# microsoft/hivedscheduler

Hardware: AMD Instinct MI355X
Metric: scheduling p50 latency + VC-safety violations; RCCL bus-bw at 1/2/4/8-GPU cells (lower is better)
Workload: dtype fp32; 1 GPU; model=hived-sched-config4-fragmentation-stress, cluster=simulated 4-node x 8-MI355X, global_batch=64, seq_len=0, parallelism=single

## Files before the change

hivedscheduler_amd/core/algorithm.cpp:

```cpp
#include <cstdio>
#include <cstdlib>

#include "core.hpp"

namespace hived {

bool mapDebugRelease() {
  static int v = -1;
  if (v < 0) v = getenv("HIVED_DEBUG_MAP") ? 1 : 0;
  return v == 1;
}

namespace {
constexpr size_t kWaitReasonReserve = 128;

struct Victims {
  std::map<std::string, std::set<std::string>> byNode;
  std::set<Group*> overlappingPreemptors;
};

Victims collectPreemptionVictims(const Placement<PhysicalCell>& placement) {
  Victims v;
  for (auto& [leafNum, pods] : placement) {
    (void)leafNum;
    for (auto& pod : pods) {
      for (PhysicalCell* c : pod) {
        if (c == nullptr) continue;
        if ((c->state == CState::Used || c->state == CState::Reserving) &&
            c->usingGroup != nullptr) {
          for (auto& [ln, victims] : c->usingGroup->allocatedPods) {
            (void)ln;
            for (auto& p : victims) {
              if (p.present) v.byNode[p.node].insert(p.key);
            }
          }
        }
        if (c->state == CState::Reserving || c->state == CState::Reserved) {
          v.overlappingPreemptors.insert(c->reservingGroup);
        }
      }
    }
  }
  return v;
}

std::set<std::string> collectBadOrNonSuggestedNodes(const Placement<PhysicalCell>& placement,
                                                    const std::set<std::string>& suggestedNodes,
                                                    bool ignoreSuggestedNodes) {
  std::set<std::string> bad;
  for (auto& [leafNum, pods] : placement) {
    (void)leafNum;
    for (auto& pod : pods) {
      for (PhysicalCell* c : pod) {
        if (c == nullptr) continue;
        if (!c->healthy || (!ignoreSuggestedNodes && !suggestedNodes.count(c->nodes[0]))) {
          bad.insert(c->nodes[0]);
        }
      }
    }
  }
  return bad;
}

std::pair<PodPlacementInfo, std::string> retrieveMissingPodPlacement(Group* g, int leafCellNum,
                                                                     int podIndex) {
  for (auto& [ln, pods] : g->allocatedPods) {
    (void)ln;
    for (auto& p : pods) {
      if (!p.present) continue;
      for (auto& mbi : p.bindInfo.memberBindInfo) {
        if (!mbi.empty() && static_cast<int>(mbi[0].leafIndices.size()) == leafCellNum &&
            podIndex < static_cast<int>(mbi.size())) {
          return {mbi[podIndex], p.bindInfo.chain};
        }
      }
    }
  }
  throw HivedError::Internal("no allocated pod found in group " + g->name +
                             " when retrieving missing placement");
}

VirtualCell* retrieveVirtualCell(const Placement<PhysicalCell>& phys,
                                 const Placement<VirtualCell>& virt, PhysicalCell* target) {
  for (auto& [leafNum, pods] : phys) {
    auto vIt = virt.find(leafNum);
    if (vIt == virt.end()) continue;
    for (size_t podIdx = 0; podIdx < pods.size(); podIdx++) {
      for (size_t i = 0; i < pods[podIdx].size(); i++) {
        if (pods[podIdx][i] == target) return vIt->second[podIdx][i];
      }
    }
  }
  return nullptr;
}

int getNewPodIndex(const std::vector<AllocatedPod>& pods) {
  for (size_t i = 0; i < pods.size(); i++) {
    if (!pods[i].present) return static_cast<int>(i);
  }
  return -1;
}

int getAllocatedPodIndex(const BindInfo& info, int leafCellNum) {
  for (auto& mbi : info.memberBindInfo) {
    if (mbi.empty() || static_cast<int>(mbi[0].leafIndices.size()) != leafCellNum) continue;
    for (size_t podIndex = 0; podIndex < mbi.size(); podIndex++) {
      auto& pl = mbi[podIndex];
      if (pl.node == info.node && !info.isolation.empty() &&
          std::find(pl.leafIndices.begin(), pl.leafIndices.end(), info.isolation[0]) !=
              pl.leafIndices.end()) {
        return static_cast<int>(podIndex);
      }
    }
  }
  return -1;
}

bool allPodsReleased(const std::map<int, std::vector<AllocatedPod>>& allocatedPods) {
  for (auto& [ln, pods] : allocatedPods) {
    (void)ln;
    for (auto& p : pods) {
      if (p.present) return false;
    }
  }
  return true;
}

bool anyBoundUnder(PhysicalCell* c) {
  if (c->virt != nullptr) return true;
  for (Cell* ch : c->children) {
    if (anyBoundUnder(static_cast<PhysicalCell*>(ch))) return true;
  }
  return false;
}

std::unique_ptr<Group> newGroup(const PodSpec& s, GState state) {
  auto g = std::make_unique<Group>();
  g->name = s.groupName;
  g->vc = s.vc;
  g->lazyPreemptionEnable = s.lazyPreemptionEnable;
  g->ignoreK8sSuggestedNodes = s.ignoreK8sSuggestedNodes;
  g->gangReleaseEnable = s.gangReleaseEnable;
  g->priority = s.priority;
  g->state = state;
  g->totalPodNums = s.groupPodNums;
  for (auto& [leafNum, podNum] : s.groupPodNums) {
    g->allocatedPods[leafNum].resize(podNum);
    auto& phys = g->physPlacement[leafNum];
    phys.resize(podNum);
    for (auto& pod : phys) pod.assign(leafNum, nullptr);
    auto& virt = g->virtPlacement[leafNum];
    virt.resize(podNum);
    for (auto& pod : virt) pod.assign(leafNum, nullptr);
  }
  return g;
}

}


ScheduleResult HivedCore::schedule(const PodSpec& s, const std::string& podKey,
                                   const std::set<std::string>& suggestedNodes, Phase phase) {
  OpGuard opGuard(this);
  scheduleCount_++;
  Placement<PhysicalCell> phys;
  Placement<VirtualCell> virt;
  bool hasVirtual = true;
  std::map<std::string, std::set<std::string>> victims;
  std::string waitReason;
  waitReason.reserve(kWaitReasonReserve);
  int podIndex = 0;
  bool havePlacement = false;

  auto it = groups_.find(s.groupName);
  bool groupExists = it != groups_.end();
  bool mayHaveGroup = groupExists || phase == Phase::Preempting;
  if (groupExists) {
    havePlacement = schedulePodFromExistingGroup(it->second.get(), s, suggestedNodes, phase,
                                                 podKey, &phys, &hasVirtual, &virt, &victims,
                                                 &podIndex);
    groupExists = groups_.find(s.groupName) != groups_.end();
  }
  if (!groupExists) {
    schedulePodFromNewGroup(s, suggestedNodes, phase, podKey, &phys, &hasVirtual, &virt, &victims,
                            &waitReason);
    havePlacement = !phys.empty();
  }
  (void)havePlacement;
  Group* g = nullptr;
  if (mayHaveGroup) {
    if (auto git = groups_.find(s.groupName); git != groups_.end()) g = git->second.get();
  }
  return generateResult(phys, hasVirtual, virt, victims, std::move(waitReason), s.leafCellNumber,
                        podIndex, g, s.groupName);
}

ScheduleResult HivedCore::generateResult(const Placement<PhysicalCell>& phys, bool hasVirtual,
                                         const Placement<VirtualCell>& virt,
                                         const std::map<std::string, std::set<std::string>>& victims,
                                         std::string&& waitReason, int currentLeafNum,
                                         int podIndex, Group* group,
                                         const std::string& groupName) {
  ScheduleResult r;
  if (phys.empty()) {
    r.kind = ScheduleResult::Kind::Wait;
    if (waitReason.empty()) {
      r.waitReason = "waiting for resources";
    } else {
      r.waitReason = std::move(waitReason);
    }
    return r;
  }
  if (!victims.empty()) {
    r.kind = ScheduleResult::Kind::Preempt;
    auto it = victims.begin();
    std::advance(it, static_cast<long>(victimRng_() % victims.size()));
    r.victimNode = it->first;
    r.victimPodKeys.assign(it->second.begin(), it->second.end());
    return r;
  }
  r.kind = ScheduleResult::Kind::Bind;
  BindInfo& info = r.bindInfo;
  for (auto& [leafNum, pods] : phys) {
    std::vector<PodPlacementInfo> placements(pods.size());
    for (size_t pi = 0; pi < pods.size(); pi++) {
      auto& pl = placements[pi];
      pl.leafIndices.assign(leafNum, 0);
      pl.preassignedTypes.assign(leafNum, "");
      for (int li = 0; li < leafNum; li++) {
        PhysicalCell* c = pods[pi][li];
        if (c == nullptr) {
          if (group == nullptr || group->state == GState::Preempting) {
            throw HivedError::Internal("first pod in group " + groupName +
                                       " was allocated invalid resource");
          }
          auto [retrieved, chain] = retrieveMissingPodPlacement(group, leafNum, static_cast<int>(pi));
          pl = retrieved;
          if (info.chain.empty()) info.chain = chain;
          break;
        }
        if (pl.node.empty()) pl.node = c->nodes[0];
        pl.leafIndices[li] = c->leafIndices[0];
        if (hasVirtual) {
          auto vIt = virt.find(leafNum);
          if (vIt != virt.end() && pi < vIt->second.size() &&
              li < static_cast<int>(vIt->second[pi].size()) && vIt->second[pi][li] != nullptr) {
            VirtualCell* v = vIt->second[pi][li];
            pl.preassignedTypes[li] = cellTypes_[v->chain][v->preassigned->level];
          }
        }
      }
    }
    if (leafNum == currentLeafNum) {
      if (podIndex >= static_cast<int>(placements.size())) {
        throw HivedError::BadRequest("pod index " + std::to_string(podIndex) +
                                     " out of range in group " + groupName);
      }
      info.node = placements[podIndex].node;
      info.isolation = placements[podIndex].leafIndices;
      PhysicalCell* first = pods[podIndex].empty() ? nullptr : pods[podIndex][0];
      if (first != nullptr) info.chain = first->chain;
    }
    info.memberBindInfo.push_back(std::move(placements));
  }
  return r;
}


bool HivedCore::schedulePodFromExistingGroup(
    Group* g, const PodSpec& s, const std::set<std::string>& suggestedNodes, Phase phase,
    const std::string& podKey, Placement<PhysicalCell>* phys, bool* hasVirtual,
    Placement<VirtualCell>* virt, std::map<std::string, std::set<std::string>>* victims,
    int* podIndex) {
  std::set<std::string> badNodes =
      collectBadOrNonSuggestedNodes(g->physPlacement, suggestedNodes, g->ignoreK8sSuggestedNodes);
  if (g->state == GState::Allocated) {
    *phys = g->physPlacement;
    *hasVirtual = g->hasVirtualPlacement;
    *virt = g->virtPlacement;
    auto it = g->allocatedPods.find(s.leafCellNumber);
    int idx = (it == g->allocatedPods.end()) ? -1 : getNewPodIndex(it->second);
    if (idx == -1) {
      throw HivedError::BadRequest("Requesting more pods than the configured number for " +
                                   std::to_string(s.leafCellNumber) + " leaf cells in group " +
                                   s.groupName);
    }
    *podIndex = idx;
    return true;
  }
  if (phase == Phase::Preempting && !badNodes.empty()) {
    deletePreemptingGroup(g, podKey);
    return false;
  }
  *phys = g->physPlacement;
  *hasVirtual = g->hasVirtualPlacement;
  *virt = g->virtPlacement;
  Victims v = collectPreemptionVictims(g->physPlacement);
  *victims = std::move(v.byNode);
  g->preemptingPods.insert(podKey);
  return true;
}

void HivedCore::schedulePodFromNewGroup(const PodSpec& s,
                                        const std::set<std::string>& suggestedNodes, Phase phase,
                                        const std::string& podKey, Placement<PhysicalCell>* phys,
                                        bool* hasVirtual, Placement<VirtualCell>* virt,
                                        std::map<std::string, std::set<std::string>>* victims,
                                        std::string* waitReason) {
  if (!scheduleNewAffinityGroup(s, suggestedNodes, podKey, phys, hasVirtual, virt, waitReason)) {
    phys->clear();
    return;
  }
  Victims v = collectPreemptionVictims(*phys);
  *victims = std::move(v.byNode);
  if (phase == Phase::Preempting) {
    for (Group* preemptor : v.overlappingPreemptors) {
      deletePreemptingGroup(preemptor, podKey);
    }
    if (!victims->empty()) {
      createPreemptingGroup(s, *phys, *virt, podKey);
    }
  }
}

bool HivedCore::scheduleNewAffinityGroup(const PodSpec& s,
                                         const std::set<std::string>& suggestedNodes,
                                         const std::string& podKey, Placement<PhysicalCell>* phys,
                                         bool* hasVirtual, Placement<VirtualCell>* virt,
                                         std::string* failedReason) {
  SchedulingRequest sr(s);
  sr.suggestedNodes = &suggestedNodes;
  sr.ignoreSuggestedNodes = s.ignoreK8sSuggestedNodes;
  sr.hbmBytes = s.hbmBytesPerCell;
  validateSchedulingRequest(sr, podKey);
  if (!sr.pinnedCellId.empty()) {
    sr.chain = &pinnedPhysical_[s.vc][s.pinnedCellId]->chain;
    auto it = sr.vcScheduler->pinnedSchedulers.find(sr.pinnedCellId);
    sr.topo = it == sr.vcScheduler->pinnedSchedulers.end() ? nullptr : &it->second;
    return handleSchedulingRequest(sr, phys, hasVirtual, virt, failedReason);
  }
  if (!s.leafCellType.empty()) {
    auto it = cellChains_.find(s.leafCellType);
    if (it == cellChains_.end()) {
      throw HivedError::BadRequest("[" + podKey + "]: Pod requesting leaf cell type " +
                                   s.leafCellType + " which the whole cluster does not have");
    }
    return scheduleForLeafCellType(sr, s.leafCellType, it->second, podKey, true, phys, hasVirtual,
                                   virt, failedReason);
  }
  for (auto& [leafType, chains] : cellChains_) {
    if (scheduleForLeafCellType(sr, leafType, chains, podKey, false, phys, hasVirtual, virt,
                                failedReason)) {
      return true;
    }
  }
  return false;
}

bool HivedCore::scheduleForLeafCellType(SchedulingRequest& sr, const std::string& leafCellType,
                                        const std::vector<std::string>& chains,
                                        const std::string& podKey, bool typeSpecified,
                                        Placement<PhysicalCell>* phys, bool* hasVirtual,
                                        Placement<VirtualCell>* virt, std::string* failedReason) {
  bool vcHasType = false;
  for (const std::string& chain : chains) {
    if (sr.priority < kMinGuaranteedPriority) {
      sr.topo = &opportunisticSchedulers_.at(chain);
    } else {
      auto it = sr.vcScheduler->nonPinnedSchedulers.find(chain);
      if (it == sr.vcScheduler->nonPinnedSchedulers.end()) continue;
      sr.topo = &it->second;
    }
    vcHasType = true;
    sr.chain = &chain;
    if (handleSchedulingRequest(sr, phys, hasVirtual, virt, failedReason)) return true;
  }
  if (typeSpecified && sr.priority >= kMinGuaranteedPriority && !vcHasType) {
    throw HivedError::BadRequest("[" + podKey + "]: Pod requesting leaf cell type " + leafCellType +
                                 " which VC " + sr.vc + " does not have");
  }
  return false;
}

void HivedCore::validateSchedulingRequest(SchedulingRequest& sr, const std::string& podKey) {
  std::string message;
  auto vcIt = vcSchedulers_.find(sr.vc);
  if (vcIt == vcSchedulers_.end()) {
    message = "VC " + sr.vc + " does not exist!";
  } else {
    sr.vcScheduler = &vcIt->second;
    if (!sr.pinnedCellId.empty()) {
      if (!sr.vcScheduler->pinned.count(sr.pinnedCellId)) {
        message = "VC " + sr.vc + " does not have pinned cell " + sr.pinnedCellId;
      } else if (sr.priority == kOpportunisticPriority) {
        message = "opportunistic pod not supported to use pinned cell " + sr.pinnedCellId;
      }
    }
  }
  if (!message.empty()) throw HivedError::BadRequest("[" + podKey + "]: " + message);
}

bool HivedCore::handleSchedulingRequest(SchedulingRequest& sr, Placement<PhysicalCell>* phys,
                                        bool* hasVirtual, Placement<VirtualCell>* virt,
                                        std::string* failedReason) {
  if (sr.priority >= kMinGuaranteedPriority) {
    *hasVirtual = true;
    return scheduleGuaranteedGroup(sr, phys, virt, failedReason);
  }
  *hasVirtual = false;
  virt->clear();
  return scheduleOpportunisticGroup(sr, phys, failedReason);
}

bool HivedCore::scheduleGuaranteedGroup(SchedulingRequest& sr, Placement<PhysicalCell>* phys,
                                        Placement<VirtualCell>* virt, std::string* failedReason) {
  struct RestoreSteering {
    SchedulingRequest& sr;
    bool honorLinksOnly;
    const CleanShapeWorld* cleanWorld;
    ~RestoreSteering() {
      sr.honorLinksOnly = honorLinksOnly;
      sr.cleanWorld = cleanWorld;
    }
  } restoreSteering{sr, sr.honorLinksOnly, sr.cleanWorld};

  const ChainCellList& fullCells = fullCellList_[*sr.chain];
  const bool badLinks = chainHasBadLinks(fullCells);

  auto attemptOnce = [&](bool honorOnly) -> bool {
    sr.honorLinksOnly = honorOnly;
    if (!sr.vcScheduler->schedule(sr, virt, failedReason)) return false;
    if (mapDebugRelease()) {
      for (auto& [ln, pods] : *virt) {
        for (auto& pod : pods) {
          fprintf(stderr, "[virt ln=%d honorOnly=%d]", ln, (int)honorOnly);
          for (auto* v : pod) fprintf(stderr, " %s", v->address.c_str());
          fprintf(stderr, "\n");
        }
      }
    }

    CellBindings bindings;
    auto lazyPreempted = tryLazyPreempt(*virt, sr.groupName);

    MapScratch& ms = mapScratch_;
    ms.reset();
    std::vector<BindingVertex*>& preassigned = ms.preassigned;
    SmallPtrMap<VirtualCell, BindingVertex*, 32> vertexMap;
    std::vector<VirtualCell*>& path = ms.path;
    for (auto& [leafNum, pods] : *virt) {
      (void)leafNum;
      for (auto& pod : pods) {
        for (VirtualCell* leaf : pod) {
          if (leaf->phys != nullptr) {
            bindings[leaf] = leaf->phys;
            continue;
          }
          path.clear();
          for (Cell* c = leaf; c != nullptr; c = c->parent) {
            auto* vc = static_cast<VirtualCell*>(c);
            if (vc->phys != nullptr || vertexMap.count(vc)) break;
            path.push_back(vc);
          }
          if (path.empty()) continue;
          VirtualCell* pathRoot = path.back();
          BindingVertex* rootPtr = ms.newVertex(pathRoot);
          vertexMap[pathRoot] = rootPtr;
          if (pathRoot->parent == nullptr) {
            preassigned.push_back(rootPtr);
          } else if (static_cast<VirtualCell*>(pathRoot->parent)->phys != nullptr) {
            bool buddyExists = false;
            for (size_t gi = 0; gi < ms.nonPreassignedUsed; gi++) {
              auto& grp = ms.nonPreassigned[gi];
              if (grp[0]->cell->parent == pathRoot->parent) {
                grp.push_back(rootPtr);
                buddyExists = true;
                break;
              }
            }
            if (!buddyExists) ms.newNonPreassignedGroup().push_back(rootPtr);
          } else {
            vertexMap.at(static_cast<VirtualCell*>(pathRoot->parent))->children.push_back(rootPtr);
          }
          for (int i = static_cast<int>(path.size()) - 2; i >= 0; i--) {
            BindingVertex* childVertex = ms.newVertex(path[i]);
            vertexMap[path[i]] = childVertex;
            vertexMap.at(static_cast<VirtualCell*>(path[i]->parent))->children.push_back(childVertex);
          }
        }
      }
    }

    const bool mayRetry = !honorOnly && (sr.cleanWorld != nullptr || badLinks);
    CellBindings seedBindings;
    if (mayRetry) seedBindings = bindings;
    bool firstTry = true;
    auto tryMap = [&](bool honorLinks) {
      if (!firstTry) bindings = seedBindings;
      firstTry = false;
      ms.freeList = freeCellList_[*sr.chain];
      ms.freeCellNum = allVCFreeCellNum_[*sr.chain];
      return mapVirtualPlacementToPhysical(preassigned, ms.nonPreassigned, ms.nonPreassignedUsed,
                                           ms.freeList, ms.freeCellNum, *sr.suggestedNodes,
                                           sr.ignoreSuggestedNodes, bindings, sr.hbmBytes,
                                           honorLinks, sr.cleanWorld);
    };
    bool mapped;
    if (honorOnly) {
      mapped = tryMap(true);
    } else if (sr.cleanWorld != nullptr || badLinks) {
      mapped = tryMap(true) || tryMap(false);
    } else {
      mapped = tryMap(false);
    }
    if (mapped) {
      phys->clear();
      for (auto& [leafNum, pods] : *virt) {
        for (auto& pod : pods) {
          std::vector<PhysicalCell*> cells;
          cells.reserve(pod.size());
          for (VirtualCell* v : pod) cells.push_back(bindings.at(v));
          (*phys)[leafNum].push_back(std::move(cells));
        }
      }
      return true;
    }
    for (auto& [groupName, placement] : lazyPreempted) {
      revertLazyPreempt(groups_.at(groupName).get(), placement);
    }
    return false;
  };

  int gangLeaves = 0;
  for (auto& [ln, pn] : sr.podLeafCellNums) gangLeaves += ln * pn;
  if (badLinks && gangLeaves >= 2) {
    const std::set<std::string>* filter =
        sr.ignoreSuggestedNodes ? nullptr : sr.suggestedNodes;
    auto tryWorlds = [&](int tier) {
      std::vector<CleanShapeWorld> computed;
      const std::vector<CleanShapeWorld>* worldsPtr;
      if (filter == nullptr) {
        WorldCacheEntry& entry = worldCache_[{*sr.chain, tier}];
        if (entry.epoch != gWorldEpochCounter) {
          entry.worlds = computeCleanShapeWorlds(fullCells, nullptr, 4, tier);
          entry.epoch = gWorldEpochCounter;
        }
        worldsPtr = &entry.worlds;
      } else {
        computed = computeCleanShapeWorlds(fullCells, filter, 4, tier);
        worldsPtr = &computed;
      }
      for (const auto& w : *worldsPtr) {
        sr.cleanWorld = &w;
        if (mapDebugRelease()) {
          fprintf(stderr, "[world] chain=%s tier=%d excl=%zu:", sr.chain->c_str(), tier,
                  w.excluded.size());
          for (auto& [l, v] : w.caps) fprintf(stderr, " L%d=%d", l, v);
          fprintf(stderr, "\n");
        }
        if (attemptOnce(true)) return true;
      }
      return false;
    };
    if (tryWorlds(kOpportunisticPriority)) return true;
    if (sr.priority > kOpportunisticPriority && tryWorlds(sr.priority)) return true;
    sr.cleanWorld = nullptr;
  }
  if (attemptOnce(false)) return true;
  failedReason->assign("Mapping the virtual placement would need to use at least one ")
      .append(sr.ignoreSuggestedNodes ? "bad" : "bad or non-suggested")
      .append(" node");
  return false;
}

bool HivedCore::chainHasBadLinks(const ChainCellList& ccl) {
  for (Cell* c : ccl.at(ccl.top())) {
    if (static_cast<PhysicalCell*>(c)->badLinksUnder > 0) return true;
  }
  return false;
}

std::map<std::string, Placement<VirtualCell>> HivedCore::tryLazyPreempt(
    const Placement<VirtualCell>& p, const std::string& groupName) {
  std::map<std::string, Placement<VirtualCell>> preempted;
  for (auto& [leafNum, pods] : p) {
    (void)leafNum;
    for (auto& pod : pods) {
      for (VirtualCell* leaf : pod) {
        if (PhysicalCell* pc = leaf->phys) {
          if (pc->state == CState::Used && pc->usingGroup->lazyPreemptionEnable &&
              !preempted.count(pc->usingGroup->name)) {
            preempted[pc->usingGroup->name] = lazyPreemptGroup(pc->usingGroup, groupName);
          }
        }
      }
    }
  }
  return preempted;
}

bool HivedCore::scheduleOpportunisticGroup(const SchedulingRequest& sr,
                                           Placement<PhysicalCell>* phys,
                                           std::string* failedReason) {
  Placement<Cell> generic;
  if (!sr.topo->Schedule(sr.podLeafCellNums, kOpportunisticPriority, *sr.suggestedNodes,
                         sr.ignoreSuggestedNodes, &generic, failedReason, sr.hbmBytes)) {
    failedReason->append(" when scheduling in physical cluster");
    return false;
  }
  phys->clear();
  for (auto& [leafNum, pods] : generic) {
    for (auto& pod : pods) {
      std::vector<PhysicalCell*> cells;
      cells.reserve(pod.size());
      for (Cell* c : pod) cells.push_back(static_cast<PhysicalCell*>(c));
      (*phys)[leafNum].push_back(std::move(cells));
    }
  }
  return true;
}


void HivedCore::deleteUnallocatedPod(const PodSpec& s, const std::string& podKey) {
  OpGuard opGuard(this);
  auto it = groups_.find(s.groupName);
  if (it == groups_.end() || it->second->state != GState::Preempting) return;
  Group* g = it->second.get();
  g->preemptingPods.erase(podKey);
  if (g->preemptingPods.empty()) {
    deletePreemptingGroup(g, podKey);
  }
}

void HivedCore::addAllocatedPod(const PodSpec& s, const BindInfo& info, const std::string& podKey) {
  OpGuard opGuard(this);
  int podIndex = 0;
  bool releasable = true;
  Group* g = nullptr;
  auto it = groups_.find(s.groupName);
  if (it != groups_.end()) {
    g = it->second.get();
    if (g->state == GState::Preempting) allocatePreemptingGroup(g, podKey);
    podIndex = getAllocatedPodIndex(info, s.leafCellNumber);
    if (podIndex == -1) return;
  } else {
    g = createAllocatedGroup(s, info, podKey);
    podIndex = getAllocatedPodIndex(info, s.leafCellNumber);
    if (podIndex == -1) {
      podIndex = 0;
      releasable = false;
    }
  }
  setPodSlot(g, s.leafCellNumber, podIndex, releasable, podKey, info);
}

void HivedCore::deleteAllocatedPod(const PodSpec& s, const BindInfo& info,
                                   const std::string& podKey) {
  OpGuard opGuard(this);
  auto it = groups_.find(s.groupName);
  if (it == groups_.end()) return;
  Group* g = it->second.get();
  int podIndex = getAllocatedPodIndex(info, s.leafCellNumber);
  if (podIndex == -1) return;
  clearPodSlot(g, s.leafCellNumber, podIndex);
  if (allPodsReleased(g->allocatedPods)) {
    deleteAllocatedGroup(g, podKey);
  }
}

bool HivedCore::deleteAllocatedPodByKey(const std::string& podKey) {
  auto it = podIndex_.find(podKey);
  if (it == podIndex_.end()) return false;
  const PodSlotRef ref = it->second;
  OpGuard opGuard(this);
  if (!ref.releasable) return true;
  podIndex_.erase(it);
  ref.group->allocatedPods[ref.leafCellNum][ref.podIndex] = AllocatedPod{};
  if (allPodsReleased(ref.group->allocatedPods)) {
    deleteAllocatedGroup(ref.group, podKey);
  }
  return true;
}

void HivedCore::setPodSlot(Group* g, int leafCellNum, int podIndex, bool releasable,
                           const std::string& podKey, const BindInfo& info) {
  auto& slots = g->allocatedPods[leafCellNum];
  if (podIndex >= static_cast<int>(slots.size())) slots.resize(podIndex + 1);
  AllocatedPod& slot = slots[podIndex];
  if (slot.present && slot.key != podKey) clearPodSlot(g, leafCellNum, podIndex);
  slot.present = true;
  slot.key = podKey;
  slot.node = info.node;
  slot.bindInfo = info;
  podIndex_[podKey] = PodSlotRef{g, leafCellNum, podIndex, releasable};
}

void HivedCore::clearPodSlot(Group* g, int leafCellNum, int podIndex) {
  auto& slots = g->allocatedPods[leafCellNum];
  if (podIndex >= static_cast<int>(slots.size())) return;
  AllocatedPod& slot = slots[podIndex];
  if (slot.present) {
    auto it = podIndex_.find(slot.key);
    if (it != podIndex_.end() && it->second.group == g &&
        it->second.leafCellNum == leafCellNum && it->second.podIndex == podIndex) {
      podIndex_.erase(it);
    }
  }
  slot = AllocatedPod{};
}

void HivedCore::eraseGroup(Group* g) {
  for (auto& [leafNum, pods] : g->allocatedPods) {
    for (size_t i = 0; i < pods.size(); i++) {
      if (pods[i].present) clearPodSlot(g, leafNum, static_cast<int>(i));
    }
  }
  groups_.erase(g->name);
}


Group* HivedCore::createAllocatedGroup(const PodSpec& s, const BindInfo& info,
                                       const std::string& podKey) {
  auto group = newGroup(s, GState::Allocated);
  Group* g = group.get();
  groups_[s.groupName] = std::move(group);
  bool shouldLazyPreempt = false;
  for (auto& mbi : info.memberBindInfo) {
    if (mbi.empty()) continue;
    int leafCellNumber = static_cast<int>(mbi[0].leafIndices.size());
    if (!g->physPlacement.count(leafCellNumber)) {
      g->physPlacement[leafCellNumber].assign(mbi.size(),
                                              std::vector<PhysicalCell*>(leafCellNumber, nullptr));
      g->virtPlacement[leafCellNumber].assign(mbi.size(),
                                              std::vector<VirtualCell*>(leafCellNumber, nullptr));
      g->allocatedPods[leafCellNumber].resize(mbi.size());
    }
    for (size_t podIndex = 0; podIndex < mbi.size(); podIndex++) {
      for (size_t li = 0; li < mbi[podIndex].leafIndices.size(); li++) {
        bool lazyPreempt = false;
        bool isOpportunistic = false;
        auto [p, v] = findAllocatedLeafCell(static_cast<int>(li), mbi[podIndex], info.chain, s, g,
                                            podKey, &lazyPreempt, &isOpportunistic);
        if (p == nullptr) {
          continue;
        }
        g->physPlacement[leafCellNumber][podIndex][li] = p;
        if (isOpportunistic) {
          g->hasVirtualPlacement = false;
        } else if (v != nullptr) {
          g->virtPlacement[leafCellNumber][podIndex][li] = v;
          if (inFreeCellList(p) && v->preassigned->priority > kFreePriority) {
            lazyPreemptCell(v->preassigned, g->name);
          }
        } else {
          shouldLazyPreempt = shouldLazyPreempt || lazyPreempt;
        }
        if (p->reservingGroup != nullptr && p->reservingGroup != g) {
          deletePreemptingGroup(p->reservingGroup, podKey);
        }
        auto [safetyOk, reason] =
            allocateLeafCell(p, g->virtPlacement[leafCellNumber][podIndex][li], s.priority, g->vc);
        p->usingGroup = g;
        setCellState(p, CState::Used);
        if (!safetyOk) {
          shouldLazyPreempt = true;
        }
        (void)reason;
      }
    }
  }
  if (shouldLazyPreempt) {
    lazyPreemptGroup(g, g->name);
  }
  return g;
}

void HivedCore::deleteAllocatedGroup(Group* g, const std::string& podKey) {
  (void)podKey;
  for (auto& [leafNum, pods] : g->physPlacement) {
    (void)leafNum;
    for (auto& pod : pods) {
      for (PhysicalCell* c : pod) {
        if (c == nullptr) continue;
        c->usingGroup = nullptr;
        if (c->state == CState::Used) {
          releaseLeafCell(c, g->vc);
          setCellState(c, CState::Free);
        } else {
          setCellState(c, CState::Reserved);
        }
      }
    }
  }
  eraseGroup(g);
}

void HivedCore::createPreemptingGroup(const PodSpec& s, const Placement<PhysicalCell>& phys,
                                      const Placement<VirtualCell>& virt,
                                      const std::string& podKey) {
  auto group = newGroup(s, GState::Preempting);
  Group* g = group.get();
  g->physPlacement = phys;
  g->virtPlacement = virt;
  for (auto& [leafNum, pods] : phys) {
    auto vIt = virt.find(leafNum);
    for (size_t pi = 0; pi < pods.size(); pi++) {
      for (size_t li = 0; li < pods[pi].size(); li++) {
        PhysicalCell* pc = pods[pi][li];
        VirtualCell* vc = vIt->second[pi][li];
        if (pc->state == CState::Used) {
          Group* usingGroup = pc->usingGroup;
          releaseLeafCell(pc, usingGroup->vc);
          usingGroup->state = GState::BeingPreempted;
        }
        allocateLeafCell(pc, vc, s.priority, g->vc);
        pc->reservingGroup = g;
        if (pc->state == CState::Used) {
          setCellState(pc, CState::Reserving);
        } else {
          setCellState(pc, CState::Reserved);
        }
      }
    }
  }
  g->preemptingPods.insert(podKey);
  groups_[s.groupName] = std::move(group);
}

void HivedCore::deletePreemptingGroup(Group* g, const std::string& podKey) {
  (void)podKey;
  for (auto& [leafNum, pods] : g->physPlacement) {
    (void)leafNum;
    for (auto& pod : pods) {
      for (PhysicalCell* pc : pod) {
        releaseLeafCell(pc, g->vc);
        pc->reservingGroup = nullptr;
        if (pc->state == CState::Reserving) {
          setCellState(pc, CState::Used);
          Group* beingPreempted = pc->usingGroup;
          VirtualCell* vc = nullptr;
          if (beingPreempted->hasVirtualPlacement) {
            vc = retrieveVirtualCell(beingPreempted->physPlacement, beingPreempted->virtPlacement,
                                     pc);
          }
          allocateLeafCell(pc, vc, beingPreempted->priority, beingPreempted->vc);
        } else {
          setCellState(pc, CState::Free);
        }
      }
    }
  }
  for (auto& [name, other] : groups_) {
    (void)name;
    if (other->state == GState::BeingPreempted) {
      bool stillPreempted = false;
      for (auto& [ln, pods] : other->physPlacement) {
        (void)ln;
        for (auto& pod : pods) {
          for (PhysicalCell* c : pod) {
            if (c != nullptr && (c->state == CState::Reserving || c->state == CState::Reserved)) {
              stillPreempted = true;
            }
          }
        }
      }
      if (!stillPreempted) other->state = GState::Allocated;
    }
  }
  eraseGroup(g);
}

void HivedCore::allocatePreemptingGroup(Group* g, const std::string& podKey) {
  (void)podKey;
  for (auto& [leafNum, pods] : g->physPlacement) {
    (void)leafNum;
    for (auto& pod : pods) {
      for (PhysicalCell* pc : pod) {
        pc->reservingGroup = nullptr;
        pc->usingGroup = g;
        setCellState(pc, CState::Used);
      }
    }
  }
  g->state = GState::Allocated;
  g->preemptingPods.clear();
}

Placement<VirtualCell> HivedCore::lazyPreemptGroup(Group* victim, const std::string& preemptor) {
  if (victim->hasVirtualPlacement) {
    for (auto& [leafNum, pods] : victim->virtPlacement) {
      (void)leafNum;
      for (auto& pod : pods) {
        for (VirtualCell* v : pod) {
          if (v != nullptr && v->phys != nullptr) {
            PhysicalCell* p = v->phys;
            releaseLeafCell(p, victim->vc);
            allocateLeafCell(p, nullptr, kOpportunisticPriority, victim->vc);
          }
        }
      }
    }
  }
  Placement<VirtualCell> original = victim->virtPlacement;
  victim->virtPlacement.clear();
  victim->hasVirtualPlacement = false;
  victim->lazyStatus = LazyPreemptionStatus{preemptor, ""};
  return original;
}

void HivedCore::lazyPreemptCell(VirtualCell* c, const std::string& preemptor) {
  if (c->level == kLowestLevel && c->phys != nullptr && c->phys->state == CState::Used &&
      c->phys->usingGroup != nullptr) {
    lazyPreemptGroup(c->phys->usingGroup, preemptor);
  }
  for (Cell* child : c->children) {
    lazyPreemptCell(static_cast<VirtualCell*>(child), preemptor);
  }
}

void HivedCore::revertLazyPreempt(Group* g, const Placement<VirtualCell>& virt) {
  for (auto& [leafNum, pods] : g->physPlacement) {
    auto vIt = virt.find(leafNum);
    if (vIt == virt.end()) continue;
    for (size_t pi = 0; pi < pods.size(); pi++) {
      for (size_t li = 0; li < pods[pi].size(); li++) {
        PhysicalCell* p = pods[pi][li];
        if (p == nullptr) continue;
        VirtualCell* v = vIt->second[pi][li];
        releaseLeafCell(p, g->vc);
        allocateLeafCell(p, v, g->priority, g->vc);
      }
    }
  }
  g->virtPlacement = virt;
  g->hasVirtualPlacement = true;
  g->lazyStatus.reset();
}


std::pair<PhysicalCell*, VirtualCell*> HivedCore::findAllocatedLeafCell(
    int index, const PodPlacementInfo& placement, const std::string& chain, const PodSpec& s,
    Group* group, const std::string& podKey, bool* lazyPreempt, bool* isOpportunistic) {
  (void)podKey;
  *lazyPreempt = false;
  *isOpportunistic = false;
  int leafIndex = placement.leafIndices[index];
  PhysicalCell* p = nullptr;
  int matches = 0;
  if (auto nodeIt = nodeLeafCellsStorage_.find(placement.node);
      nodeIt != nodeLeafCellsStorage_.end()) {
    for (PhysicalCell* leaf : nodeIt->second) {
      if (leaf->leafIndices[0] == leafIndex) {
        p = leaf;
        matches++;
      }
    }
  }
  if (matches > 1) p = findPhysicalLeafCell(fullCellList_, chain, placement.node, leafIndex);
  if (p == nullptr) return {nullptr, nullptr};
  if (placement.preassignedTypes.empty()) {
    *lazyPreempt = true;
    return {p, nullptr};
  }
  if (!group->hasVirtualPlacement) {
    return {p, nullptr};
  }
  const std::string& preassignedType =
      index < static_cast<int>(placement.preassignedTypes.size()) ? placement.preassignedTypes[index]
                                                                  : std::string();
  if (preassignedType.empty()) {
    *isOpportunistic = true;
    return {p, nullptr};
  }
  int preassignedLevel = -1;
  auto typesIt = cellTypes_.find(p->chain);
  if (typesIt != cellTypes_.end()) {
    for (auto& [l, t] : typesIt->second) {
      if (t == preassignedType) preassignedLevel = l;
    }
  }
  if (preassignedLevel > 0) {
    PhysicalCell* pre = p;
    while (pre->parent != nullptr && pre->level < preassignedLevel) {
      pre = static_cast<PhysicalCell*>(pre->parent);
    }
    for (PhysicalCell* a = static_cast<PhysicalCell*>(pre->parent); a != nullptr;
         a = static_cast<PhysicalCell*>(a->parent)) {
      if (a->virt != nullptr) {
        *lazyPreempt = true;
        return {p, nullptr};
      }
    }
    if (pre->virt == nullptr) {
      for (Cell* ch : pre->children) {
        if (anyBoundUnder(static_cast<PhysicalCell*>(ch))) {
          *lazyPreempt = true;
          return {p, nullptr};
        }
      }
    }
  }
  VirtualCell* v = nullptr;
  std::string message;
  if (preassignedLevel < 0) {
    message = "preassigned cell type " + preassignedType + " not found in chain " + p->chain;
  } else if (!vcSchedulers_.count(s.vc)) {
    message = "VC " + s.vc + " not found";
  } else {
    IntraVCScheduler& vcs = vcSchedulers_[s.vc];
    const ChainCellList* vccl = nullptr;
    if (!s.pinnedCellId.empty()) {
      auto it = vcs.pinned.find(s.pinnedCellId);
      if (it != vcs.pinned.end()) vccl = &it->second;
    } else {
      auto it = vcs.nonPinnedPreassigned.find(p->chain);
      if (it != vcs.nonPinnedPreassigned.end()) vccl = &it->second;
    }
    if (vccl == nullptr) {
      message = "VC " + s.vc + " has no cell for chain " + p->chain;
    } else {
      v = mapPhysicalCellToVirtual(p, *vccl, preassignedLevel, s.priority, &message);
    }
  }
  if (v == nullptr) {
    *lazyPreempt = true;
    return {p, nullptr};
  }
  if (v->vc != s.vc) {
    *lazyPreempt = true;
    return {p, nullptr};
  }
  return {p, v};
}

std::pair<bool, std::string> HivedCore::allocateLeafCell(PhysicalCell* p, VirtualCell* v,
                                                         int priority, const std::string& vc) {
  bool safetyOk = true;
  std::string reason;
  if (v != nullptr) {
    setCellPriority(v, priority);
    updateUsedLeafCellNumAtPriority(v, priority, true);
    setCellPriority(p, priority);
    updateUsedLeafCellNumAtPriority(p, priority, true);
    VirtualCell* pac = v->preassigned;
    if (pac->phys != nullptr && pac->phys->virt == pac &&
        pac->phys->priority < kMinGuaranteedPriority &&
        vcDoomedBadCells_[vc][p->chain].contains(pac->phys, pac->phys->level)) {
      PhysicalCell* anc = p;
      while (anc->parent != nullptr && anc != pac->phys && anc->level < pac->phys->level) {
        anc = static_cast<PhysicalCell*>(anc->parent);
      }
      if (anc != pac->phys) {
        PhysicalCell* doomed = pac->phys;
        pac->phys = nullptr;
        doomed->virt = nullptr;
        vcDoomedBadCells_[vc][p->chain].remove(doomed, doomed->level);
        allVCDoomedBadCellNum_[p->chain][doomed->level]--;
        releasePreassignedCell(doomed, vc, true);
      }
    }
    bool preassignedNewlyBound = pac->phys == nullptr;
    bool preassignedProducible = false;
    if (preassignedNewlyBound) {
      PhysicalCell* anc = p;
      while (anc->parent != nullptr && anc->level < pac->level) {
        anc = static_cast<PhysicalCell*>(anc->parent);
      }
      auto& fl = freeCellList_[p->chain];
      for (PhysicalCell* a = anc; a != nullptr && a->virt == nullptr;
           a = static_cast<PhysicalCell*>(a->parent)) {
        if (a->level <= fl.top() && fl.contains(a, a->level)) {
          preassignedProducible = true;
          break;
        }
      }
    }
    if (p->virt == nullptr) {
      bindCell(p, v);
    }
    if (preassignedNewlyBound && preassignedProducible) {
      std::tie(safetyOk, reason) = allocatePreassignedCell(pac->phys, vc, false);
    }
  } else {
    setCellPriority(p, kOpportunisticPriority);
    updateUsedLeafCellNumAtPriority(p, kOpportunisticPriority, true);
    p->otVC = vc;
  }
  return {safetyOk, reason};
}

void HivedCore::releaseLeafCell(PhysicalCell* p, const std::string& vc) {
  (void)vc;
  if (!p->otVC.empty() || p->virt == nullptr) {
    p->otVC.clear();
  } else {
    VirtualCell* v = p->virt;
    const std::string& owner = v->vc;
    updateUsedLeafCellNumAtPriority(v, v->priority, false);
    setCellPriority(v, kFreePriority);
    PhysicalCell* preassignedPhysical = v->preassigned->phys;
    if (p->healthy) {
      unbindCell(p);
    }
    if (preassignedPhysical != nullptr && !preassignedPhysical->pinned &&
        v->preassigned->priority < kMinGuaranteedPriority &&
        !vcDoomedBadCells_[owner][preassignedPhysical->chain].contains(
            preassignedPhysical, preassignedPhysical->level)) {
      releasePreassignedCell(preassignedPhysical, owner, false);
    } else if (mapDebugRelease()) {
      fprintf(stderr, "[rel] keep preassigned %s: phys=%d pinned=%d prio=%d doomed=%d (leaf %s)\n",
              v->preassigned->address.c_str(), preassignedPhysical != nullptr,
              preassignedPhysical != nullptr && preassignedPhysical->pinned,
              v->preassigned->priority,
              preassignedPhysical != nullptr &&
                  vcDoomedBadCells_[owner][preassignedPhysical->chain].contains(
                      preassignedPhysical, preassignedPhysical->level),
              p->address.c_str());
    }
  }
  updateUsedLeafCellNumAtPriority(p, p->priority, false);
  setCellPriority(p, kFreePriority);
}

}
```

hivedscheduler_amd/core/bindings.cpp:

```cpp
#include <pybind11/pybind11.h>
#include <pybind11/stl.h>

#include <climits>
#include <cstring>
#include <functional>
#include <mutex>

#include "core.hpp"

namespace py = pybind11;
using namespace hived;

namespace {

std::string dstr(const py::dict& d, const char* key, const std::string& def = "") {
  if (!d.contains(key)) return def;
  py::object v = d[key];
  if (v.is_none()) return def;
  return py::cast<std::string>(py::str(v));
}
long long dint(const py::dict& d, const char* key, long long def = 0) {
  if (!d.contains(key)) return def;
  py::object v = d[key];
  if (v.is_none()) return def;
// ... 130 lines not shown
  HIVED_NAME(leafCellNumber);
  HIVED_NAME(gangReleaseEnable);
  HIVED_NAME(lazyPreemptionEnable);
  HIVED_NAME(ignoreK8sSuggestedNodes);
  HIVED_NAME(hbmBytesPerCell);
  HIVED_NAME(affinityGroup);
  HIVED_NAME(name);
  HIVED_NAME(members);
  HIVED_NAME(podNumber);
  HIVED_NAME(node);
  HIVED_NAME(cellChain);
  HIVED_NAME(leafCellIsolation);
  HIVED_NAME(affinityGroupBindInfo);
  HIVED_NAME(podPlacements);
  HIVED_NAME(physicalNode);
  HIVED_NAME(physicalLeafCellIndices);
  HIVED_NAME(preassignedCellTypes);
  HIVED_NAME(kind);
  HIVED_NAME(bind);
  HIVED_NAME(preempt);
  HIVED_NAME(wait);
  HIVED_NAME(bindInfo);
  HIVED_NAME(victimNode);
  HIVED_NAME(victimPodKeys);
  HIVED_NAME(reason);
  HIVED_NAME(pod_spec);
  HIVED_NAME(spec);
  HIVED_NAME(pod_key);
  HIVED_NAME(suggested_nodes);
  HIVED_NAME(phase);
  HIVED_NAME(commit);
  HIVED_NAME(validate);
  HIVED_NAME(Filtering);
  HIVED_NAME(Preempting);
  HIVED_NAME(code);
#undef HIVED_NAME
}

struct ApiTypes {
  PyObject* PodSchedulingSpec;
  PyObject* AffinityGroupSpec;
  PyObject* AffinityGroupMemberSpec;
  PyObject* PodBindInfo;
  PyObject* AffinityGroupMemberBindInfo;
  PyObject* PodPlacementInfo;
  PyObject* WebServerError;
  PyObject* emptyTuple;
  PyObject* one;
};
ApiTypes T{};

void initApiTypes() {
  py::module_ types = py::module_::import("hivedscheduler_amd.api.types");
#define HIVED_TYPE(x) T.x = py::object(types.attr(#x)).release().ptr()
  HIVED_TYPE(PodSchedulingSpec);
  HIVED_TYPE(AffinityGroupSpec);
  HIVED_TYPE(AffinityGroupMemberSpec);
  HIVED_TYPE(PodBindInfo);
  HIVED_TYPE(AffinityGroupMemberBindInfo);
  HIVED_TYPE(PodPlacementInfo);
  HIVED_TYPE(WebServerError);
#undef HIVED_TYPE
  T.emptyTuple = PyTuple_New(0);
  T.one = PyLong_FromLong(1);
  if (T.emptyTuple == nullptr || T.one == nullptr) throw py::error_already_set();
}

class Record {
 public:
  explicit Record(py::handle rec) : rec_(rec.ptr()) {
    if (PyDict_Check(rec_)) {
      dict_ = rec_;
      wire_ = true;
      return;
    }
    PyObject* tp = reinterpret_cast<PyObject*>(Py_TYPE(rec_));
    if (tp == T.PodSchedulingSpec || tp == T.AffinityGroupMemberSpec ||
        tp == T.AffinityGroupSpec) {
      dict_ = ownedDict_ = PyObject_GenericGetDict(rec_, nullptr);
      if (dict_ == nullptr) PyErr_Clear();
    }
  }
  Record(const Record&) = delete;
  Record& operator=(const Record&) = delete;
  ~Record() { Py_XDECREF(ownedDict_); }
  py::handle object() const { return rec_; }

 private:
  friend class Field;
  PyObject* rec_;
  PyObject* dict_ = nullptr;
  PyObject* ownedDict_ = nullptr;
  bool wire_ = false;
};

class Field {
 public:
  Field(py::handle rec, PyObject* name) {
    if (PyDict_Check(rec.ptr())) {
      p_ = PyDict_GetItemWithError(rec.ptr(), name);
      if (p_ == nullptr && PyErr_Occurred()) throw py::error_already_set();
    } else {
      p_ = PyObject_GetAttr(rec.ptr(), name);
      if (p_ == nullptr) throw py::error_already_set();
      owned_ = true;
    }
  }
  Field(const Record& rec, PyObject* name) {
    if (rec.dict_ != nullptr) {
      p_ = PyDict_GetItemWithError(rec.dict_, name);
      if (p_ == nullptr && PyErr_Occurred()) throw py::error_already_set();
      if (rec.wire_) return;
      if (p_ != nullptr) {
        Py_INCREF(p_);
        owned_ = true;
        return;
      }
    }
    p_ = PyObject_GetAttr(rec.rec_, name);
    if (p_ == nullptr) throw py::error_already_set();
    owned_ = true;
  }
  Field(const Field&) = delete;
  Field& operator=(const Field&) = delete;
  ~Field() {
    if (owned_) Py_DECREF(p_);
  }
  explicit operator bool() const { return p_ != nullptr && p_ != Py_None; }
  py::handle get() const { return p_; }

 private:
  PyObject* p_ = nullptr;
  bool owned_ = false;
};

std::string toStdString(py::handle v) {
  if (PyUnicode_Check(v.ptr())) {
    Py_ssize_t n = 0;
    const char* s = PyUnicode_AsUTF8AndSize(v.ptr(), &n);
    if (s == nullptr) throw py::error_already_set();
    return std::string(s, static_cast<size_t>(n));
  }
  return py::cast<std::string>(py::str(v));
}
long long toLongLong(py::handle v) {
  if (PyLong_CheckExact(v.ptr())) {
    int overflow = 0;
    long long x = PyLong_AsLongLongAndOverflow(v.ptr(), &overflow);
    if (overflow == 0) {
      if (x == -1 && PyErr_Occurred()) throw py::error_already_set();
      return x;
    }
  }
  return py::cast<long long>(v);
}
int toInt(py::handle v) {
  if (PyLong_CheckExact(v.ptr())) {
    int overflow = 0;
    long x = PyLong_AsLongAndOverflow(v.ptr(), &overflow);
    if (overflow == 0 && x >= INT_MIN && x <= INT_MAX) {
      if (x == -1 && PyErr_Occurred()) throw py::error_already_set();
      return static_cast<int>(x);
    }
  }
  return py::cast<int>(v);
}
bool toBool(py::handle v) {
  if (v.ptr() == Py_True) return true;
  if (v.ptr() == Py_False) return false;
  return py::cast<bool>(v);
}

template <class Rec>
std::string fstr(const Rec& rec, PyObject* name) {
  Field f(rec, name);
  return f ? toStdString(f.get()) : std::string();
}
template <class Rec>
long long fint(const Rec& rec, PyObject* name) {
  Field f(rec, name);
  return f ? toLongLong(f.get()) : 0;
}
template <class Rec>
bool fbool(const Rec& rec, PyObject* name, bool def) {
  Field f(rec, name);
  return f ? toBool(f.get()) : def;
}

class Items {
 public:
  explicit Items(py::handle v) : seq_(PySequence_Fast(v.ptr(), "expected a list")) {
    if (seq_ == nullptr) throw py::error_already_set();
  }
  Items(const Items&) = delete;
  Items& operator=(const Items&) = delete;
  ~Items() { Py_DECREF(seq_); }
  Py_ssize_t size() const { return PySequence_Fast_GET_SIZE(seq_); }
  py::handle operator[](Py_ssize_t i) const { return PySequence_Fast_GET_ITEM(seq_, i); }

 private:
  PyObject* seq_;
};

PodSpec parsePodSpec(py::handle spec) {
  Record d(spec);
  PodSpec s;
  s.vc = fstr(d, N.virtualCluster);
  s.priority = static_cast<int>(fint(d, N.priority));
  s.pinnedCellId = fstr(d, N.pinnedCellId);
  s.leafCellType = fstr(d, N.leafCellType);
  s.leafCellNumber = static_cast<int>(fint(d, N.leafCellNumber));
  s.gangReleaseEnable = fbool(d, N.gangReleaseEnable, false);
  s.lazyPreemptionEnable = fbool(d, N.lazyPreemptionEnable, false);
  s.ignoreK8sSuggestedNodes = fbool(d, N.ignoreK8sSuggestedNodes, true);
  s.hbmBytesPerCell = fint(d, N.hbmBytesPerCell);
  if (s.hbmBytesPerCell < 0) {
    throw HivedError::BadRequest("hbmBytesPerCell must be non-negative");
  }
  if (Field ag{d, N.affinityGroup}) {
    Record group(ag.get());
    s.groupName = fstr(group, N.name);
    if (Field members{group, N.members}) {
      Items ms(members.get());
      for (Py_ssize_t i = 0; i < ms.size(); i++) {
        Record member(ms[i]);
        s.groupPodNums[static_cast<int>(fint(member, N.leafCellNumber))] +=
            static_cast<int>(fint(member, N.podNumber));
      }
    }
  }
  if (s.groupPodNums.empty() && s.leafCellNumber > 0) {
    s.groupPodNums[s.leafCellNumber] = 1;
  }
  return s;
}

void parseIntList(py::handle rec, PyObject* name, std::vector<int>* out) {
  if (Field f{rec, name}) {
    Items items(f.get());
    out->reserve(static_cast<size_t>(items.size()));
    for (Py_ssize_t i = 0; i < items.size(); i++) out->push_back(toInt(items[i]));
  }
}

BindInfo parseBindInfo(py::handle d) {
  BindInfo info;
  info.node = fstr(d, N.node);
  info.chain = fstr(d, N.cellChain);
  parseIntList(d, N.leafCellIsolation, &info.isolation);
  if (Field mbis{d, N.affinityGroupBindInfo}) {
    Items mbiItems(mbis.get());
    info.memberBindInfo.reserve(static_cast<size_t>(mbiItems.size()));
    for (Py_ssize_t m = 0; m < mbiItems.size(); m++) {
      std::vector<PodPlacementInfo> placements;
      if (Field pls{mbiItems[m], N.podPlacements}) {
        Items plItems(pls.get());
        placements.reserve(static_cast<size_t>(plItems.size()));
        for (Py_ssize_t p = 0; p < plItems.size(); p++) {
          py::handle plD = plItems[p];
          PodPlacementInfo pl;
          pl.node = fstr(plD, N.physicalNode);
          parseIntList(plD, N.physicalLeafCellIndices, &pl.leafIndices);
          if (Field types{plD, N.preassignedCellTypes}) {
            Items ts(types.get());
            pl.preassignedTypes.reserve(static_cast<size_t>(ts.size()));
            for (Py_ssize_t t = 0; t < ts.size(); t++) {
              pl.preassignedTypes.push_back(ts[t].is_none() ? std::string() : toStdString(ts[t]));
            }
          }
          placements.push_back(std::move(pl));
        }
      }
      info.memberBindInfo.push_back(std::move(placements));
    }
  }
  return info;
}

py::object pyStr(const std::string& s) {
  PyObject* o = PyUnicode_FromStringAndSize(s.data(), static_cast<Py_ssize_t>(s.size()));
  if (o == nullptr) throw py::error_already_set();
  return py::reinterpret_steal<py::object>(o);
}
py::object pyIntList(const std::vector<int>& v) {
  py::list l(v.size());
  for (size_t i = 0; i < v.size(); i++) {
    PyObject* o = PyLong_FromLong(v[i]);
    if (o == nullptr) throw py::error_already_set();
    PyList_SET_ITEM(l.ptr(), static_cast<Py_ssize_t>(i), o);
  }
  return std::move(l);
}
py::object pyStrList(const std::vector<std::string>& v) {
  py::list l(v.size());
  for (size_t i = 0; i < v.size(); i++) {
    PyList_SET_ITEM(l.ptr(), static_cast<Py_ssize_t>(i), pyStr(v[i]).release().ptr());
  }
  return std::move(l);
}
void setItem(py::dict& d, PyObject* key, py::handle value) {
  if (PyDict_SetItem(d.ptr(), key, value.ptr()) != 0) throw py::error_already_set();
}

py::dict bindInfoToDict(const BindInfo& info) {
  py::dict d;
  setItem(d, N.node, pyStr(info.node));
  setItem(d, N.leafCellIsolation, pyIntList(info.isolation));
  setItem(d, N.cellChain, pyStr(info.chain));
  py::list mbis(info.memberBindInfo.size());
  for (size_t m = 0; m < info.memberBindInfo.size(); m++) {
    auto& mbi = info.memberBindInfo[m];
    py::list placements(mbi.size());
    for (size_t p = 0; p < mbi.size(); p++) {
      auto& pl = mbi[p];
      py::dict pd;
      setItem(pd, N.physicalNode, pyStr(pl.node));
      setItem(pd, N.physicalLeafCellIndices, pyIntList(pl.leafIndices));
      setItem(pd, N.preassignedCellTypes, pyStrList(pl.preassignedTypes));
      PyList_SET_ITEM(placements.ptr(), static_cast<Py_ssize_t>(p), pd.release().ptr());
    }
    py::dict md;
    setItem(md, N.podPlacements, placements);
    PyList_SET_ITEM(mbis.ptr(), static_cast<Py_ssize_t>(m), md.release().ptr());
  }
  setItem(d, N.affinityGroupBindInfo, mbis);
  return d;
}

bool isNodeNameCollection(py::handle v) {
  PyObject* o = v.ptr();
  if (PySequence_Check(o) != 0) return !PyUnicode_Check(o) && !PyBytes_Check(o);
  if (PyGen_Check(o) != 0 || PyAnySet_Check(o) != 0) return true;
  if (PyType_Check(o)) return false;
  const char* tp = Py_TYPE(o)->tp_name;
  for (const char* ok : {"dict_keys", "dict_values", "dict_items", "map", "zip"}) {
    if (std::strcmp(tp, ok) == 0) return true;
  }
  return false;
}

std::set<std::string> toNodeNameSet(py::handle v) {
  std::set<std::string> out;
  Items items(v);
  for (Py_ssize_t i = 0; i < items.size(); i++) {
    py::handle item = items[i];
    if (!PyUnicode_Check(item.ptr()) && !PyBytes_Check(item.ptr())) {
      throw py::type_error("suggested_nodes must contain node names (str)");
    }
    out.insert(py::cast<std::string>(item));
  }
  return out;
}


py::object newInstance(PyObject* cls) {
  PyTypeObject* tp = reinterpret_cast<PyTypeObject*>(cls);
  PyObject* o = tp->tp_new(tp, T.emptyTuple, nullptr);
  if (o == nullptr) throw py::error_already_set();
  return py::reinterpret_steal<py::object>(o);
}
void setAttr(py::handle o, PyObject* name, py::handle value) {
  if (PyObject_SetAttr(o.ptr(), name, value.ptr()) != 0) throw py::error_already_set();
}

py::object defaultAffinityGroup(py::handle podKey, py::handle leafCellNumber) {
  py::object member = newInstance(T.AffinityGroupMemberSpec);
  setAttr(member, N.podNumber, T.one);
  setAttr(member, N.leafCellNumber, leafCellNumber);
  py::list members(1);
  PyList_SET_ITEM(members.ptr(), 0, member.release().ptr());
  py::object group = newInstance(T.AffinityGroupSpec);
  setAttr(group, N.name, podKey);
  setAttr(group, N.members, members);
  return group;
}

PodSpec parseValidatedPodSpec(py::handle spec, py::handle podKey, const std::string& key) {
  if (PyDict_Check(spec.ptr())) {
    throw py::type_error("schedule_pod validates a PodSchedulingSpec object, not a dict");
  }
  Record d(spec);
  PodSpec s;
  Field leaf(d, N.leafCellNumber);
  bool defaulted = false;
  {
    Field ag(d, N.affinityGroup);
    if (!ag) {
      setAttr(spec, N.affinityGroup, defaultAffinityGroup(podKey, leaf.get()));
      defaulted = true;
    }
  }
  s.vc = fstr(d, N.virtualCluster);
  if (s.vc.empty()) throw HivedError::BadRequest("VirtualCluster is empty");
  long long priority = fint(d, N.priority);
  if (priority < kOpportunisticPriority) {
    throw HivedError::BadRequest("Priority is less than " + std::to_string(kOpportunisticPriority));
  }
  if (priority > kMaxGuaranteedPriority) {
    throw HivedError::BadRequest("Priority is greater than " +
                                 std::to_string(kMaxGuaranteedPriority));
  }
  s.priority = static_cast<int>(priority);
  long long leafNum = leaf ? toLongLong(leaf.get()) : 0;
  if (leafNum <= 0) throw HivedError::BadRequest("LeafCellNumber is non-positive");
  s.leafCellNumber = static_cast<int>(leafNum);
  if (defaulted) {
    s.groupName = key;
    s.groupPodNums[s.leafCellNumber] = 1;
  } else {
    Field ag(d, N.affinityGroup);
    Record group(ag.get());
    s.groupName = fstr(group, N.name);
    if (s.groupName.empty()) throw HivedError::BadRequest("AffinityGroup.Name is empty");
    bool podInGroup = false;
    if (Field members{group, N.members}) {
      Items ms(members.get());
      for (Py_ssize_t i = 0; i < ms.size(); i++) {
        Record member(ms[i]);
        long long podNumber = fint(member, N.podNumber);
        if (podNumber <= 0) {
          throw HivedError::BadRequest("AffinityGroup.Members has non-positive PodNumber");
        }
        long long memberLeafNum = fint(member, N.leafCellNumber);
        if (memberLeafNum <= 0) {
          throw HivedError::BadRequest("AffinityGroup.Members has non-positive LeafCellNumber");
        }
        if (memberLeafNum == leafNum) podInGroup = true;
        s.groupPodNums[static_cast<int>(memberLeafNum)] += static_cast<int>(podNumber);
      }
    }
    if (!podInGroup) {
      throw HivedError::BadRequest("AffinityGroup.Members does not contain current Pod");
    }
  }
  s.pinnedCellId = fstr(d, N.pinnedCellId);
  s.leafCellType = fstr(d, N.leafCellType);
  s.gangReleaseEnable = fbool(d, N.gangReleaseEnable, false);
  s.lazyPreemptionEnable = fbool(d, N.lazyPreemptionEnable, false);
  s.ignoreK8sSuggestedNodes = fbool(d, N.ignoreK8sSuggestedNodes, true);
  s.hbmBytesPerCell = fint(d, N.hbmBytesPerCell);
  if (s.hbmBytesPerCell < 0) {
    throw HivedError::BadRequest("hbmBytesPerCell must be non-negative");
  }
  return s;
}

py::object bindInfoToObject(const BindInfo& info) {
  py::list mbis(info.memberBindInfo.size());
  for (size_t m = 0; m < info.memberBindInfo.size(); m++) {
    auto& mbi = info.memberBindInfo[m];
    py::list placements(mbi.size());
    for (size_t p = 0; p < mbi.size(); p++) {
      auto& pl = mbi[p];
      py::object po = newInstance(T.PodPlacementInfo);
      setAttr(po, N.physicalNode, pyStr(pl.node));
      setAttr(po, N.physicalLeafCellIndices, pyIntList(pl.leafIndices));
      setAttr(po, N.preassignedCellTypes, pyStrList(pl.preassignedTypes));
      PyList_SET_ITEM(placements.ptr(), static_cast<Py_ssize_t>(p), po.release().ptr());
    }
    py::object mo = newInstance(T.AffinityGroupMemberBindInfo);
    setAttr(mo, N.podPlacements, placements);
    PyList_SET_ITEM(mbis.ptr(), static_cast<Py_ssize_t>(m), mo.release().ptr());
  }
  py::object o = newInstance(T.PodBindInfo);
  setAttr(o, N.node, pyStr(info.node));
  setAttr(o, N.leafCellIsolation, pyIntList(info.isolation));
  setAttr(o, N.cellChain, pyStr(info.chain));
  setAttr(o, N.affinityGroupBindInfo, mbis);
  return o;
}

struct PyScheduleResult {
  PyObject_HEAD
  PyObject* bindInfo;
  PyObject* victimNode;
  PyObject* victimPodKeys;
  PyObject* waitReason;
  hived::ScheduleResult r;
};

void resultDealloc(PyObject* self) {
  auto* o = reinterpret_cast<PyScheduleResult*>(self);
  Py_XDECREF(o->bindInfo);
  Py_XDECREF(o->victimNode);
  Py_XDECREF(o->victimPodKeys);
  Py_XDECREF(o->waitReason);
  o->r.~ScheduleResult();
  Py_TYPE(self)->tp_free(self);
}

template <class Make>
PyObject* cachedAttr(PyObject** slot, Make make) {
  if (*slot == nullptr) {
    try {
      *slot = make().release().ptr();
    } catch (py::error_already_set& e) {
      e.restore();
      return nullptr;
    } catch (const std::exception& e) {
      PyErr_SetString(PyExc_RuntimeError, e.what());
      return nullptr;
    }
  }
  Py_INCREF(*slot);
  return *slot;
}

PyObject* resultKind(PyObject* self, void*) {
  PyObject* k = nullptr;
  switch (reinterpret_cast<PyScheduleResult*>(self)->r.kind) {
    case hived::ScheduleResult::Kind::Bind: k = N.bind; break;
    case hived::ScheduleResult::Kind::Preempt: k = N.preempt; break;
    case hived::ScheduleResult::Kind::Wait: k = N.wait; break;
  }
  Py_INCREF(k);
  return k;
}
PyObject* resultBindInfo(PyObject* self, void*) {
  auto* o = reinterpret_cast<PyScheduleResult*>(self);
  if (o->r.kind != hived::ScheduleResult::Kind::Bind) Py_RETURN_NONE;
  return cachedAttr(&o->bindInfo, [o] { return bindInfoToObject(o->r.bindInfo); });
}
PyObject* resultVictimNode(PyObject* self, void*) {
  auto* o = reinterpret_cast<PyScheduleResult*>(self);
  return cachedAttr(&o->victimNode, [o] { return pyStr(o->r.victimNode); });
}
PyObject* resultVictimPodKeys(PyObject* self, void*) {
  auto* o = reinterpret_cast<PyScheduleResult*>(self);
  return cachedAttr(&o->victimPodKeys, [o] { return pyStrList(o->r.victimPodKeys); });
}
PyObject* resultWaitReason(PyObject* self, void*) {
  auto* o = reinterpret_cast<PyScheduleResult*>(self);
  return cachedAttr(&o->waitReason, [o] { return pyStr(o->r.waitReason); });
}

PyObject* resultRepr(PyObject* self) {
  auto* o = reinterpret_cast<PyScheduleResult*>(self);
  switch (o->r.kind) {
    case hived::ScheduleResult::Kind::Bind: {
      PyObject* info = resultBindInfo(self, nullptr);
      if (info == nullptr) return nullptr;
      PyObject* node = PyObject_GetAttr(info, N.node);
      PyObject* cells = PyObject_GetAttr(info, N.leafCellIsolation);
      PyObject* out = (node != nullptr && cells != nullptr)
                          ? PyUnicode_FromFormat("ScheduleResult(bind node=%S cells=%S)", node, cells)
                          : nullptr;
      Py_XDECREF(node);
      Py_XDECREF(cells);
      Py_DECREF(info);
      return out;
    }
    case hived::ScheduleResult::Kind::Preempt: {
      PyObject* keys = resultVictimPodKeys(self, nullptr);
      if (keys == nullptr) return nullptr;
      PyObject* out = PyUnicode_FromFormat("ScheduleResult(preempt victims=%S)", keys);
      Py_DECREF(keys);
      return out;
    }
    case hived::ScheduleResult::Kind::Wait:
      break;
  }
  PyObject* reason = resultWaitReason(self, nullptr);
  if (reason == nullptr) return nullptr;
  PyObject* out = PyUnicode_FromFormat("ScheduleResult(wait reason=%R)", reason);
  Py_DECREF(reason);
  return out;
}

PyGetSetDef resultGetSet[] = {
    {"kind", resultKind, nullptr, "\"bind\", \"preempt\" or \"wait\"", nullptr},
    {"bind_info", resultBindInfo, nullptr, "PodBindInfo of a bind decision, else None", nullptr},
    {"victim_node", resultVictimNode, nullptr, "node whose pods a preempt decision evicts", nullptr},
    {"victim_pod_keys", resultVictimPodKeys, nullptr, "pod keys a preempt decision evicts", nullptr},
    {"wait_reason", resultWaitReason, nullptr, "why a wait decision waits", nullptr},
    {nullptr, nullptr, nullptr, nullptr, nullptr},
};

PyTypeObject ResultType = {PyVarObject_HEAD_INIT(nullptr, 0)};

void initResultType(py::module_& m) {
  ResultType.tp_name = "hivedscheduler_amd.hivedcore.ScheduleResult";
  ResultType.tp_doc = "One of bind / preempt / wait.";
  ResultType.tp_basicsize = sizeof(PyScheduleResult);
  ResultType.tp_flags = Py_TPFLAGS_DEFAULT;
  ResultType.tp_dealloc = resultDealloc;
  ResultType.tp_repr = resultRepr;
  ResultType.tp_getset = resultGetSet;
  if (PyType_Ready(&ResultType) != 0) throw py::error_already_set();
  m.add_object("ScheduleResult", reinterpret_cast<PyObject*>(&ResultType));
}

py::object makeResult(hived::ScheduleResult&& r) {
  PyScheduleResult* o = PyObject_New(PyScheduleResult, &ResultType);
  if (o == nullptr) throw py::error_already_set();
  o->bindInfo = o->victimNode = o->victimPodKeys = o->waitReason = nullptr;
  new (&o->r) hived::ScheduleResult(std::move(r));
  return py::reinterpret_steal<py::object>(reinterpret_cast<PyObject*>(o));
}

py::dict physicalCellStatus(PhysicalCell* c, bool withChildren = true) {
  py::dict d;
  d["cellType"] = c->typeName;
  d["cellAddress"] = c->address;
  d["isNodeLevel"] = c->isNodeLevel;
  d["cellState"] = to_string(c->state);
  d["cellHealthiness"] = c->healthy ? "Healthy" : "Bad";
  d["cellPriority"] = c->priority;
  if (!c->otVC.empty()) d["vc"] = c->otVC;
  if (c->virt != nullptr) {
    d["vc"] = c->virt->vc;
    d["virtualCell"] = c->virt->address;
  }
  if (c->level == kLowestLevel) {
    d["physicalNode"] = c->nodes.empty() ? "" : c->nodes[0];
    d["leafCellIndex"] = c->leafIndices.empty() ? -1 : c->leafIndices[0];
    d["hbmBytes"] = c->hbmBytes;
  } else if (c->badLinksUnder > 0) {
    d["badXgmiLinksUnder"] = c->badLinksUnder;
  }
  if (withChildren && !c->children.empty()) {
    py::list children;
    for (Cell* child : c->children) {
      children.append(physicalCellStatus(static_cast<PhysicalCell*>(child)));
    }
    d["cellChildren"] = children;
  }
  return d;
}

py::dict virtualCellStatus(VirtualCell* c, bool withChildren = true) {
  py::dict d;
  d["cellType"] = c->typeName;
  d["cellAddress"] = c->address;
  CState state = c->phys != nullptr ? c->phys->state
                                    : (c->priority > kFreePriority ? CState::Used : CState::Free);
  d["cellState"] = to_string(state);
  d["cellHealthiness"] = (c->phys == nullptr || c->phys->healthy) ? "Healthy" : "Bad";
  d["cellPriority"] = c->priority;
  if (c->phys != nullptr) d["physicalCell"] = c->phys->address;
  if (withChildren && !c->children.empty()) {
    py::list children;
    for (Cell* child : c->children) {
      children.append(virtualCellStatus(static_cast<VirtualCell*>(child)));
    }
    d["cellChildren"] = children;
  }
  return d;
}

py::dict groupToDict(const Group* g) {
  py::dict d;
  d["name"] = g->name;
  d["vc"] = g->vc;
  d["priority"] = g->priority;
  d["state"] = to_string(g->state);
  if (g->lazyStatus.has_value()) {
    py::dict lp;
    lp["preemptor"] = g->lazyStatus->preemptor;
    lp["preemptionTime"] = g->lazyStatus->preemptionTime;
    d["lazyPreemptionStatus"] = lp;
  } else {
    d["lazyPreemptionStatus"] = py::none();
  }
  py::dict physD;
  for (auto& [leafNum, pods] : g->physPlacement) {
    (void)leafNum;
    for (auto& pod : pods) {
      for (PhysicalCell* c : pod) {
        if (c == nullptr) continue;
        std::string node = c->nodes.empty() ? "" : c->nodes[0];
        if (!physD.contains(py::str(node))) physD[py::str(node)] = py::list();
        py::cast<py::list>(physD[py::str(node)]).append(c->leafIndices[0]);
      }
    }
  }
  d["physicalPlacement"] = physD;
  py::dict virtD;
  if (g->hasVirtualPlacement) {
    for (auto& [leafNum, pods] : g->virtPlacement) {
      (void)leafNum;
      for (auto& pod : pods) {
        for (VirtualCell* v : pod) {
          if (v == nullptr) continue;
          std::string pre = v->preassigned->address;
          if (!virtD.contains(py::str(pre))) virtD[py::str(pre)] = py::list();
          py::cast<py::list>(virtD[py::str(pre)]).append(v->address);
        }
      }
    }
  }
  d["virtualPlacement"] = virtD;
  py::list allocated;
  for (auto& [ln, pods] : g->allocatedPods) {
    (void)ln;
    for (auto& p : pods) {
      if (p.present) allocated.append(p.key);
    }
  }
  d["allocatedPods"] = allocated;
  py::list preempting;
  for (auto& k : g->preemptingPods) preempting.append(k);
  d["preemptingPods"] = preempting;
  return d;
}

#if defined(Py_GIL_DISABLED) || defined(HIVED_CORE_MUTEX)
using CoreMutex = std::mutex;
using CoreSection = std::lock_guard<std::mutex>;
#else
struct CoreMutex {};
struct CoreSection {
  explicit CoreSection(CoreMutex&) {}
};
#endif

class PyHivedCore {
 public:
  explicit PyHivedCore(const py::dict& spec) : core_(parseClusterSpec(spec)) {
    for (auto& node : core_.allNodes()) {
      nodeNames_.push_back(pyStr(node));
      allNodeSet_.insert(node);
    }
  }

  void setNodeHealthy(const std::string& node, bool healthy) {
    CoreSection section(coreMutex_);
    core_.setNodeHealthy(node, healthy);
  }
  void setLeafCellHealthy(const std::string& node, int leafIndex, bool healthy) {
    CoreSection section(coreMutex_);
    core_.setLeafCellHealthy(node, leafIndex, healthy);
  }
  void setXgmiLinkHealthy(const std::string& node, int a, int b, bool healthy, double gbps) {
    CoreSection section(coreMutex_);
    core_.setXgmiLinkHealthy(node, a, b, healthy, gbps);
  }
  py::list xgmiLinks(const std::string& node) const {
    py::list out;
    for (auto& [a, b, gbps, healthy] : core_.xgmiLinks(node)) {
      py::dict d;
      d["a"] = a;
      d["b"] = b;
      d["gbps"] = gbps;
      d["healthy"] = healthy;
      out.append(d);
    }
    return out;
  }
  py::list allNodes() const {
    py::list out(nodeNames_.size());
    for (size_t i = 0; i < nodeNames_.size(); i++) {
      PyList_SET_ITEM(out.ptr(), static_cast<Py_ssize_t>(i), py::object(nodeNames_[i]).release().ptr());
    }
    return out;
  }
  std::vector<std::string> badNodes() const {
    auto s = core_.badNodes();
    return {s.begin(), s.end()};
  }

  py::dict schedule(py::handle spec, const std::string& podKey, py::handle suggestedNodes,
                    const std::string& phase) {
    if (!isNodeNameCollection(suggestedNodes)) {
      throw py::type_error("suggested_nodes must be a sequence of node names, not " +
                           std::string(Py_TYPE(suggestedNodes.ptr())->tp_name));
    }
    PodSpec s = parsePodSpec(spec);
    bool needSuggested = !s.ignoreK8sSuggestedNodes;
    if (!needSuggested) {
      CoreSection section(coreMutex_);
      auto it = core_.groups().find(s.groupName);
      needSuggested = it != core_.groups().end() && !it->second->ignoreK8sSuggestedNodes;
    }
    std::set<std::string> suggested;
    if (needSuggested) suggested = toNodeNameSet(suggestedNodes);
    Phase ph = (phase == "Preempting") ? Phase::Preempting : Phase::Filtering;
    ScheduleResult r = [&] {
      CoreSection section(coreMutex_);
      return core_.schedule(s, podKey, suggested, ph);
    }();
    py::dict d;
    switch (r.kind) {
      case ScheduleResult::Kind::Bind:
        setItem(d, N.kind, N.bind);
        setItem(d, N.bindInfo, bindInfoToDict(r.bindInfo));
        break;
      case ScheduleResult::Kind::Preempt:
        setItem(d, N.kind, N.preempt);
        setItem(d, N.victimNode, pyStr(r.victimNode));
        setItem(d, N.victimPodKeys, pyStrList(r.victimPodKeys));
        break;
      case ScheduleResult::Kind::Wait:
        setItem(d, N.kind, N.wait);
        setItem(d, N.reason, pyStr(r.waitReason));
        break;
    }
    return d;
  }

  py::object schedulePod(py::handle spec, py::handle podKey, py::handle suggestedNodes,
                         py::handle phase, bool commit, bool validate) {
    if (!PyUnicode_Check(podKey.ptr())) throw py::type_error("pod_key must be a str");
    Phase ph = Phase::Filtering;
    if (phase.ptr() != nullptr && phase.ptr() != N.Filtering) {
      if (!PyUnicode_Check(phase.ptr())) throw py::type_error("phase must be a str");
      if (phase.ptr() == N.Preempting ||
          PyUnicode_CompareWithASCIIString(phase.ptr(), "Preempting") == 0) {
        ph = Phase::Preempting;
      }
    }
    if (!suggestedNodes.is_none() && !isNodeNameCollection(suggestedNodes)) {
      throw py::type_error("suggested_nodes must be a sequence of node names, not " +
                           std::string(Py_TYPE(suggestedNodes.ptr())->tp_name));
    }
    std::string key = toStdString(podKey);
    PodSpec s = validate ? parseValidatedPodSpec(spec, podKey, key) : parsePodSpec(spec);
    bool needSuggested = !s.ignoreK8sSuggestedNodes;
    if (!needSuggested) {
      CoreSection section(coreMutex_);
      auto it = core_.groups().find(s.groupName);
      needSuggested = it != core_.groups().end() && !it->second->ignoreK8sSuggestedNodes;
    }
    std::set<std::string> given;
    const std::set<std::string>* suggested = &given;
    if (needSuggested) {
      if (suggestedNodes.is_none()) {
        suggested = &allNodeSet_;
      } else {
        given = toNodeNameSet(suggestedNodes);
      }
    }
    hived::ScheduleResult r = [&] {
      CoreSection section(coreMutex_);
      hived::ScheduleResult decided = core_.schedule(s, key, *suggested, ph);
      if (commit && decided.kind == hived::ScheduleResult::Kind::Bind) {
        core_.addAllocatedPod(s, decided.bindInfo, key);
      }
      return decided;
    }();
    return makeResult(std::move(r));
  }

  void deleteUnallocatedPod(py::handle spec, const std::string& podKey) {
    PodSpec s = parsePodSpec(spec);
    CoreSection section(coreMutex_);
    core_.deleteUnallocatedPod(s, podKey);
  }
  void addAllocatedPod(py::handle spec, py::handle bindInfo, const std::string& podKey) {
    PodSpec s = parsePodSpec(spec);
    BindInfo info = parseBindInfo(bindInfo);
    CoreSection section(coreMutex_);
    core_.addAllocatedPod(s, info, podKey);
  }
  void deleteAllocatedPod(py::handle spec, py::handle bindInfo, const std::string& podKey) {
    PodSpec s = parsePodSpec(spec);
    BindInfo info = parseBindInfo(bindInfo);
    CoreSection section(coreMutex_);
    core_.deleteAllocatedPod(s, info, podKey);
  }

  bool deleteAllocatedPodByKey(py::handle podKey) {
    if (!PyUnicode_Check(podKey.ptr())) throw py::type_error("pod_key must be a str");
    Py_ssize_t n = 0;
    const char* utf8 = PyUnicode_AsUTF8AndSize(podKey.ptr(), &n);
    if (utf8 == nullptr) throw py::error_already_set();
    CoreSection section(coreMutex_);
    releaseKey_.assign(utf8, static_cast<size_t>(n));
    return core_.deleteAllocatedPodByKey(releaseKey_);
  }

  py::list getAllAffinityGroups() const {
    py::list out;
    for (auto& [name, g] : core_.groups()) {
      (void)name;
      out.append(groupToDict(g.get()));
    }
    return out;
  }

  py::dict getAffinityGroup(const std::string& name) const {
    auto it = core_.groups().find(name);
    if (it == core_.groups().end()) {
      throw HivedError::BadRequest("Affinity group " + name +
                                   " does not exist since it is not allocated or preempting");
    }
    return groupToDict(it->second.get());
  }

  py::dict getClusterStatus() {
    py::dict d;
    d["physicalCluster"] = getPhysicalClusterStatus();
    d["virtualClusters"] = getAllVirtualClustersStatus();
    return d;
  }

  py::list getPhysicalClusterStatus() {
    py::list out;
    for (auto& [chain, ccl] : core_.fullCellList_) {
      (void)chain;
      int top = ccl.top();
      for (Cell* c : ccl.at(top)) {
        out.append(physicalCellStatus(static_cast<PhysicalCell*>(c)));
      }
    }
    return out;
  }

  py::dict getAllVirtualClustersStatus() {
    py::dict out;
    for (auto& [vcName, vcs] : core_.vcSchedulers_) {
      out[py::str(vcName)] = getVirtualClusterStatus(vcName);
    }
    return out;
  }

  py::list getVirtualClusterStatus(const std::string& vcName) {
    auto it = core_.vcSchedulers_.find(vcName);
    if (it == core_.vcSchedulers_.end()) {
      throw HivedError::NotFound("VC " + vcName + " not found");
    }
    py::list out;
    for (auto& [chain, ccl] : it->second.nonPinnedPreassigned) {
      (void)chain;
      for (int l = 1; l <= ccl.top(); l++) {
        for (Cell* c : ccl.at(l)) {
          out.append(virtualCellStatus(static_cast<VirtualCell*>(c)));
        }
      }
    }
    for (auto& [pid, ccl] : it->second.pinned) {
      (void)pid;
      int top = ccl.top();
      for (Cell* c : ccl.at(top)) {
        out.append(virtualCellStatus(static_cast<VirtualCell*>(c)));
      }
    }
    for (auto& [chain, ccl] : core_.fullCellList_) {
      (void)chain;
      for (Cell* c : ccl.at(kLowestLevel)) {
        auto* pc = static_cast<PhysicalCell*>(c);
        if (pc->otVC == vcName) {
          py::dict d;
          d["cellType"] = pc->typeName;
          d["cellAddress"] = pc->address + "-opp";
          d["cellState"] = to_string(CState::Used);
          d["cellHealthiness"] = pc->healthy ? "Healthy" : "Bad";
          d["cellPriority"] = kOpportunisticPriority;
          d["physicalCell"] = pc->address;
          out.append(d);
        }
      }
    }
    return out;
  }

  long long scheduleCount() const { return core_.scheduleCount_; }
  void checkInvariants() const { hived::checkInvariants(core_); }

  py::dict debugCounters() const {
    py::dict d;
    for (auto& [chain, perLevel] : core_.totalLeftCellNum_) {
      py::dict cd;
      for (auto& [level, left] : perLevel) {
        py::dict ld;
        ld["totalLeft"] = left;
        int avf = 0;
        auto ai = core_.allVCFreeCellNum_.find(chain);
        if (ai != core_.allVCFreeCellNum_.end()) {
          auto li = ai->second.find(level);
          if (li != ai->second.end()) avf = li->second;
        }
        ld["allVCFree"] = avf;
        py::dict vd;
        for (auto& [vcn, perChain] : core_.vcFreeCellNum_) {
          auto ci = perChain.find(chain);
          if (ci == perChain.end()) continue;
          auto li = ci->second.find(level);
          if (li != ci->second.end() && li->second != 0) vd[py::str(vcn)] = li->second;
        }
        ld["vcFree"] = vd;
        auto fi = core_.freeCellList_.find(chain);
        if (fi != core_.freeCellList_.end() && level <= fi->second.top()) {
          py::list fl;
          for (auto* fc : fi->second.at(level)) fl.append(fc->address);
          ld["freeList"] = fl;
        }
        auto di = core_.allVCDoomedBadCellNum_.find(chain);
        if (di != core_.allVCDoomedBadCellNum_.end()) {
          auto li2 = di->second.find(level);
          if (li2 != di->second.end() && li2->second != 0) ld["doomed"] = li2->second;
        }
        auto bi = core_.badFreeCells_.find(chain);
        if (bi != core_.badFreeCells_.end() && level <= bi->second.top()) {
          ld["badFree"] = static_cast<int>(bi->second.at(level).size());
        }
        cd[py::int_(level)] = ld;
      }
      d[py::str(chain)] = cd;
    }
    return d;
  }

 private:
  HivedCore core_;
  std::vector<py::object> nodeNames_;
  std::set<std::string> allNodeSet_;
  CoreMutex coreMutex_;
  std::string releaseKey_;
};


PyObject* gCoreError = nullptr;
PyTypeObject* gCoreType = nullptr;

PyObject* newCoreError(const HivedError& e) {
  PyObject* text = PyUnicode_FromString(e.what());
  if (text == nullptr) return nullptr;
  PyObject* inst = PyObject_CallFunctionObjArgs(gCoreError, text, nullptr);
  Py_DECREF(text);
  if (inst == nullptr) return nullptr;
  PyObject* code = PyLong_FromLong(e.code);
  if (code == nullptr || PyObject_SetAttr(inst, N.code, code) != 0) {
    Py_XDECREF(code);
    Py_DECREF(inst);
    return nullptr;
  }
  Py_DECREF(code);
  return inst;
}

void setCoreError(const HivedError& e, bool asWebServerError) {
  PyObject* inst = newCoreError(e);
  if (inst == nullptr) return;
  if (!asWebServerError) {
    PyErr_SetObject(gCoreError, inst);
    Py_DECREF(inst);
    return;
  }
  PyObject* web = PyObject_CallFunction(T.WebServerError, "is", e.code, e.what());
  if (web == nullptr) {
    Py_DECREF(inst);
    return;
  }
  Py_INCREF(inst);
  PyException_SetCause(web, inst);
  PyException_SetContext(web, inst);
  PyErr_SetObject(T.WebServerError, web);
  Py_DECREF(web);
}

bool toFlag(PyObject* o, const char* name) {
  if (o == Py_True) return true;
  if (o == Py_False || o == Py_None) return false;
  PyNumberMethods* num = Py_TYPE(o)->tp_as_number;
  if (num != nullptr && num->nb_bool != nullptr) {
    int r = num->nb_bool(o);
    if (r < 0) throw py::error_already_set();
    return r != 0;
  }
  throw py::type_error(std::string(name) + " must be a bool");
}

PyHivedCore* coreOf(PyObject* self) {
  if (Py_TYPE(self) == gCoreType) {
    auto* inst = reinterpret_cast<py::detail::instance*>(self);
    if (inst->simple_layout && inst->simple_value_holder[0] != nullptr) {
      return static_cast<PyHivedCore*>(inst->simple_value_holder[0]);
    }
  }
  return py::cast<PyHivedCore*>(py::handle(self));
}

void setErrorFromCurrentException(bool facade) {
  try {
    throw;
  } catch (py::error_already_set& e) {
    e.restore();
  } catch (const py::builtin_exception& e) {
    e.set_error();
  } catch (const HivedError& e) {
    setCoreError(e, facade);
  } catch (const std::bad_alloc&) {
    PyErr_NoMemory();
  } catch (const std::out_of_range& e) {
    PyErr_SetString(PyExc_IndexError, e.what());
  } catch (const std::exception& e) {
    PyErr_SetString(PyExc_RuntimeError, e.what());
  }
}

constexpr int kSchedulePodArgs = 6;

PyObject* schedulePodCall(PyObject* self, PyObject* const* args, Py_ssize_t nargs,
                          PyObject* kwnames, bool facade) {
  const char* fn = facade ? "schedule_validated_pod" : "schedule_pod";
  const int maxArgs = facade ? kSchedulePodArgs - 1 : kSchedulePodArgs;
  PyObject* const names[kSchedulePodArgs] = {facade ? N.spec : N.pod_spec, N.pod_key,
                                             N.suggested_nodes,            N.phase,
                                             N.commit,                     N.validate};
  PyObject* a[kSchedulePodArgs] = {nullptr, nullptr, nullptr, nullptr, nullptr, nullptr};
  Py_ssize_t nkw = kwnames == nullptr ? 0 : PyTuple_GET_SIZE(kwnames);
  if (nargs + nkw > maxArgs) {
    PyErr_Format(PyExc_TypeError, "%s() takes at most %d arguments (%zd given)", fn, maxArgs,
                 nargs + nkw);
    return nullptr;
  }
  for (Py_ssize_t i = 0; i < nargs; i++) a[i] = args[i];
  for (Py_ssize_t k = 0; k < nkw; k++) {
    PyObject* name = PyTuple_GET_ITEM(kwnames, k);
    int idx = -1;
    for (int j = 0; j < maxArgs; j++) {
      if (name == names[j]) {
        idx = j;
        break;
      }
    }
    for (int j = 0; idx < 0 && j < maxArgs; j++) {
      int eq = PyObject_RichCompareBool(name, names[j], Py_EQ);
      if (eq < 0) return nullptr;
      if (eq) idx = j;
    }
    if (idx < 0) {
      PyErr_Format(PyExc_TypeError, "%s() got an unexpected keyword argument '%U'", fn, name);
      return nullptr;
    }
    if (a[idx] != nullptr) {
      PyErr_Format(PyExc_TypeError, "%s() got multiple values for argument '%U'", fn, name);
      return nullptr;
    }
    a[idx] = args[nargs + k];
  }
  for (int j = 0; j < 2; j++) {
    if (a[j] == nullptr) {
      PyErr_Format(PyExc_TypeError, "%s() missing required argument '%U' (pos %d)", fn, names[j],
                   j + 1);
      return nullptr;
    }
  }
  try {
    bool commit = a[4] != nullptr && toFlag(a[4], "commit");
    bool validate = a[5] == nullptr || toFlag(a[5], "validate");
    return coreOf(self)
        ->schedulePod(a[0], a[1], a[2] != nullptr ? a[2] : Py_None, a[3], commit, validate)
        .release()
        .ptr();
  } catch (...) {
    setErrorFromCurrentException(facade);
  }
  return nullptr;
}

PyObject* deleteByKeyCall(PyObject* self, PyObject* const* args, Py_ssize_t nargs,
                          PyObject* kwnames, bool facade) {
  const char* fn = facade ? "delete_validated_pod_by_key" : "delete_allocated_pod_by_key";
  Py_ssize_t nkw = kwnames == nullptr ? 0 : PyTuple_GET_SIZE(kwnames);
  if (nargs + nkw != 1) {
    PyErr_Format(PyExc_TypeError, "%s() takes exactly one argument 'pod_key' (%zd given)", fn,
                 nargs + nkw);
    return nullptr;
  }
  if (nkw == 1) {
    PyObject* name = PyTuple_GET_ITEM(kwnames, 0);
    int eq = name == N.pod_key ? 1 : PyObject_RichCompareBool(name, N.pod_key, Py_EQ);
    if (eq < 0) return nullptr;
    if (eq == 0) {
      PyErr_Format(PyExc_TypeError, "%s() got an unexpected keyword argument '%U'", fn, name);
      return nullptr;
    }
  }
  try {
    if (coreOf(self)->deleteAllocatedPodByKey(args[0])) Py_RETURN_TRUE;
    Py_RETURN_FALSE;
  } catch (...) {
    setErrorFromCurrentException(facade);
  }
  return nullptr;
}

PyObject* schedulePodEntry(PyObject* self, PyObject* const* args, Py_ssize_t nargs,
                           PyObject* kwnames) {
  return schedulePodCall(self, args, nargs, kwnames, false);
}
PyObject* scheduleValidatedPodEntry(PyObject* self, PyObject* const* args, Py_ssize_t nargs,
                                    PyObject* kwnames) {
  return schedulePodCall(self, args, nargs, kwnames, true);
}

PyObject* deleteByKeyEntry(PyObject* self, PyObject* const* args, Py_ssize_t nargs,
                           PyObject* kwnames) {
  return deleteByKeyCall(self, args, nargs, kwnames, false);
}
PyObject* deleteValidatedByKeyEntry(PyObject* self, PyObject* const* args, Py_ssize_t nargs,
                                    PyObject* kwnames) {
  return deleteByKeyCall(self, args, nargs, kwnames, true);
}

using FastCallWithKeywords = PyObject* (*)(PyObject*, PyObject* const*, Py_ssize_t, PyObject*);
PyCFunction asCFunction(FastCallWithKeywords f) {
  return reinterpret_cast<PyCFunction>(reinterpret_cast<void (*)()>(f));
}

PyMethodDef directMethods[] = {
    {"schedule_pod", asCFunction(schedulePodEntry), METH_FASTCALL | METH_KEYWORDS,
     "schedule_pod($self, /, pod_spec, pod_key, suggested_nodes=None, phase='Filtering', "
     "commit=False, validate=True)\n--\n\n"
     "One filter decision in one call: validate and default the request, decide,\n"
     "commit a bind decision, return the native ScheduleResult. Raises CoreError."},
    {"schedule_validated_pod", asCFunction(scheduleValidatedPodEntry),
     METH_FASTCALL | METH_KEYWORDS,
     "schedule_validated_pod($self, /, spec, pod_key, suggested_nodes=None, "
     "phase='Filtering', commit=False)\n--\n\n"
     "schedule_pod with validate=True whose core errors leave as\n"
     "WebServerError(code, text) with the CoreError as __cause__."},
    {"delete_allocated_pod_by_key", asCFunction(deleteByKeyEntry), METH_FASTCALL | METH_KEYWORDS,
     "delete_allocated_pod_by_key($self, /, pod_key)\n--\n\n"
     "Release the allocated pod the core holds under pod_key, as\n"
     "delete_allocated_pod does for the spec and bind info it was added with.\n"
     "False, and nothing changed, if the core holds no such pod. Raises CoreError."},
    {"delete_validated_pod_by_key", asCFunction(deleteValidatedByKeyEntry),
     METH_FASTCALL | METH_KEYWORDS,
     "delete_validated_pod_by_key($self, /, pod_key)\n--\n\n"
     "delete_allocated_pod_by_key whose core errors leave as\n"
     "WebServerError(code, text) with the CoreError as __cause__."},
};

void addDirectMethods(py::handle cls) {
  gCoreType = reinterpret_cast<PyTypeObject*>(cls.ptr());
  for (PyMethodDef& def : directMethods) {
    PyObject* descr = PyDescr_NewMethod(gCoreType, &def);
    if (descr == nullptr) throw py::error_already_set();
    int rc = PyObject_SetAttrString(cls.ptr(), def.ml_name, descr);
    Py_DECREF(descr);
    if (rc != 0) throw py::error_already_set();
  }
}

}

PYBIND11_MODULE(hivedcore, m) {
  m.doc() = "MI355X-native gang scheduler core (C++)";
  initNames();
  initApiTypes();
  initResultType(m);

  static py::exception<HivedError> exc(m, "CoreError");
  gCoreError = exc.ptr();
  py::register_exception_translator([](std::exception_ptr p) {
    try {
      if (p) std::rethrow_exception(p);
    } catch (const HivedError& e) {
      py::object pyExc = exc;
      py::object inst = pyExc(e.what());
      inst.attr("code") = e.code;
      PyErr_SetObject(pyExc.ptr(), inst.ptr());
    }
  });

  py::class_<PyHivedCore> coreClass(m, "HivedCore");
  coreClass
      .def(py::init<const py::dict&>(), py::arg("spec"))
      .def("set_node_healthy", &PyHivedCore::setNodeHealthy, py::arg("node"), py::arg("healthy"))
      .def("set_xgmi_link_healthy", &PyHivedCore::setXgmiLinkHealthy, py::arg("node"),
           py::arg("a"), py::arg("b"), py::arg("healthy"), py::arg("gbps") = 0.0)
      .def("xgmi_links", &PyHivedCore::xgmiLinks, py::arg("node"))
      .def("set_leaf_cell_healthy", &PyHivedCore::setLeafCellHealthy, py::arg("node"),
           py::arg("leaf_index"), py::arg("healthy"))
      .def("all_nodes", &PyHivedCore::allNodes)
      .def("bad_nodes", &PyHivedCore::badNodes)
      .def("schedule", &PyHivedCore::schedule, py::arg("pod_spec"), py::arg("pod_key"),
           py::arg("suggested_nodes"), py::arg("phase"))
      .def("delete_unallocated_pod", &PyHivedCore::deleteUnallocatedPod, py::arg("pod_spec"),
           py::arg("pod_key"))
      .def("add_allocated_pod", &PyHivedCore::addAllocatedPod, py::arg("pod_spec"),
           py::arg("bind_info"), py::arg("pod_key"))
      .def("delete_allocated_pod", &PyHivedCore::deleteAllocatedPod, py::arg("pod_spec"),
           py::arg("bind_info"), py::arg("pod_key"))
      .def("get_all_affinity_groups", &PyHivedCore::getAllAffinityGroups)
      .def("get_affinity_group", &PyHivedCore::getAffinityGroup, py::arg("name"))
      .def("get_cluster_status", &PyHivedCore::getClusterStatus)
      .def("get_physical_cluster_status", &PyHivedCore::getPhysicalClusterStatus)
      .def("get_all_virtual_clusters_status", &PyHivedCore::getAllVirtualClustersStatus)
      .def("get_virtual_cluster_status", &PyHivedCore::getVirtualClusterStatus, py::arg("vc"))
      .def("schedule_count", &PyHivedCore::scheduleCount)
      .def("check_invariants", &PyHivedCore::checkInvariants)
      .def("debug_counters", &PyHivedCore::debugCounters);
  addDirectMethods(coreClass);
}
```

hivedscheduler_amd/core/config4_alloc_main.cpp:

```cpp
#include <cstdio>
#include <cstdlib>
#include <map>
#include <new>
#include <string>
#include <vector>

#include "config4_stream.hpp"
#include "core.hpp"

namespace {
long gAllocations = 0;
}

void* operator new(std::size_t n) {
  gAllocations++;
  if (void* p = std::malloc(n ? n : 1)) return p;
  throw std::bad_alloc();
}
void* operator new[](std::size_t n) { return operator new(n); }
void* operator new(std::size_t n, const std::nothrow_t&) noexcept {
  gAllocations++;
  return std::malloc(n ? n : 1);
}
void* operator new[](std::size_t n, const std::nothrow_t& t) noexcept { return operator new(n, t); }
void operator delete(void* p) noexcept { std::free(p); }
void operator delete[](void* p) noexcept { std::free(p); }
void operator delete(void* p, std::size_t) noexcept { std::free(p); }
void operator delete[](void* p, std::size_t) noexcept { std::free(p); }

using namespace hived;
using namespace config4;

namespace {

struct Tally {
  long n = 0, total = 0, lo = -1, hi = 0;
  void add(long a) {
    n++;
    total += a;
    if (lo < 0 || a < lo) lo = a;
    if (a > hi) hi = a;
  }
};

bool endsWith(const std::string& s, const char* tail) {
  std::string t(tail);
  return s.size() >= t.size() && s.compare(s.size() - t.size(), t.size(), t) == 0;
}

}

int main(int argc, char** argv) {
  int steps = argc > 1 ? atoi(argv[1]) : 20;
  int warmup = argc > 2 ? atoi(argv[2]) : 5;

  HivedCore core(makeSpec());
  for (auto& n : core.allNodes()) core.setNodeHealthy(n, true);

  std::vector<PodSpec> specs(kNumRequests);
  std::vector<std::string> keys(kNumRequests);
  for (int i = 0; i < kNumRequests; i++) {
    keys[i] = "bench/p" + std::to_string(i);
    PodSpec& s = specs[i];
    s.vc = kRequests[i].vc;
    s.priority = kRequests[i].priority;
    s.leafCellNumber = kRequests[i].cells;
    s.groupName = keys[i];
    s.groupPodNums[s.leafCellNumber] = 1;
  }
  const std::set<std::string> suggested;

  std::map<std::string, Tally> tallies;
  for (int step = 0; step < warmup + steps; step++) {
    std::vector<std::pair<int, BindInfo>> bound;
    for (int i = 0; i < kNumRequests; i++) {
      long before = gAllocations;
      ScheduleResult r = core.schedule(specs[i], keys[i], suggested, Phase::Filtering);
      long during = gAllocations - before;
      std::string what;
      switch (r.kind) {
        case ScheduleResult::Kind::Bind:
          what = "bind";
          {
            long beforeAdd = gAllocations;
            core.addAllocatedPod(specs[i], r.bindInfo, keys[i]);
            long add = gAllocations - beforeAdd;
            if (step >= warmup) {
              tallies["commit (addAllocatedPod)"].add(add);
              tallies["bind + commit"].add(during + add);
            }
          }
          bound.emplace_back(i, std::move(r.bindInfo));
          break;
        case ScheduleResult::Kind::Preempt:
          what = "preempt";
          break;
        case ScheduleResult::Kind::Wait:
          what = "wait: " + r.waitReason;
          if (!endsWith(r.waitReason, "physical cluster")) {
            what += kRequests[i].priority >= 0 ? " [guaranteed]" : " [opportunistic]";
          }
          break;
      }
      if (step >= warmup) tallies[what].add(during);
    }
#ifdef CONFIG4_NO_RELEASE_BY_KEY
    const bool byKey = false;
#else
    const bool byKey = step % 2 == 1;
#endif
    for (auto& [i, info] : bound) {
      long before = gAllocations;
#ifndef CONFIG4_NO_RELEASE_BY_KEY
      if (byKey) {
        if (!core.deleteAllocatedPodByKey(keys[i])) {
          fprintf(stderr, "unknown key %s\n", keys[i].c_str());
          return 1;
        }
      } else
#endif
        core.deleteAllocatedPod(specs[i], info, keys[i]);
      if (step >= warmup) {
        tallies[byKey ? "release (deleteAllocatedPodByKey)" : "release (deleteAllocatedPod)"].add(
            gAllocations - before);
      }
    }
#ifndef CONFIG4_NO_RELEASE_BY_KEY
    for (auto& [i, info] : bound) {
      (void)info;
      if (core.deleteAllocatedPodByKey(keys[i])) {
        fprintf(stderr, "key %s known after its release\n", keys[i].c_str());
        return 1;
      }
    }
#endif
  }
  checkInvariants(core);

  printf("config4 heap allocations per core call: steps=%d warmup=%d\n", steps, warmup);
  for (auto& [what, t] : tallies) {
    printf("  n=%-5ld min=%-3ld max=%-3ld mean=%6.2f  %s\n", t.n, t.lo, t.hi,
           static_cast<double>(t.total) / static_cast<double>(t.n), what.c_str());
  }
  return 0;
}
```

hivedscheduler_amd/core/config4_bench_main.cpp:

```cpp
#include <algorithm>
#include <chrono>
#include <cstdio>
#include <cstdlib>
#include <string>
#include <vector>

#include "config4_stream.hpp"
#include "core.hpp"

using namespace hived;
using namespace config4;

namespace {

using Clock = std::chrono::steady_clock;
double usSince(Clock::time_point t0) {
  return std::chrono::duration<double, std::micro>(Clock::now() - t0).count();
}

struct Samples {
  std::vector<double> us;
  void report(const char* what) {
    if (us.empty()) {
      printf("  %-22s n=0\n", what);
      return;
    }
    std::sort(us.begin(), us.end());
    printf("  %-22s n=%-6zu p50=%7.2fus p99=%7.2fus\n", what, us.size(), us[us.size() / 2],
           us[std::min(us.size() - 1, static_cast<size_t>(us.size() * 0.99))]);
  }
};

}

int main(int argc, char** argv) {
  int steps = argc > 1 ? atoi(argv[1]) : 200;
  int warmup = argc > 2 ? atoi(argv[2]) : 5;

  HivedCore core(makeSpec());
  for (auto& n : core.allNodes()) core.setNodeHealthy(n, true);

  std::vector<PodSpec> specs(kNumRequests);
  std::vector<std::string> keys(kNumRequests);
  for (int i = 0; i < kNumRequests; i++) {
    keys[i] = "bench/p" + std::to_string(i);
    PodSpec& s = specs[i];
    s.vc = kRequests[i].vc;
    s.priority = kRequests[i].priority;
    s.leafCellNumber = kRequests[i].cells;
    s.groupName = keys[i];
    s.groupPodNums[s.leafCellNumber] = 1;
  }
  const std::set<std::string> suggested;

  Samples all, waitS, preemptS, bindS, addS, delS, delKeyS;
  std::vector<double> stepMs;
  long binds = 0, waits = 0, preempts = 0;
  for (int step = 0; step < warmup + steps; step++) {
    bool timed = step >= warmup;
    std::vector<std::pair<int, BindInfo>> bound;
    auto ts = Clock::now();
    for (int i = 0; i < kNumRequests; i++) {
      auto t0 = Clock::now();
      ScheduleResult r = core.schedule(specs[i], keys[i], suggested, Phase::Filtering);
      double us = usSince(t0);
      double addUs = 0;
      if (r.kind == ScheduleResult::Kind::Bind) {
        auto t1 = Clock::now();
        core.addAllocatedPod(specs[i], r.bindInfo, keys[i]);
        addUs = usSince(t1);
        bound.emplace_back(i, std::move(r.bindInfo));
      }
      if (!timed) continue;
      all.us.push_back(us + addUs);
      switch (r.kind) {
        case ScheduleResult::Kind::Bind:
          bindS.us.push_back(us);
          addS.us.push_back(addUs);
          binds++;
          break;
        case ScheduleResult::Kind::Preempt:
          preemptS.us.push_back(us);
          preempts++;
          break;
        case ScheduleResult::Kind::Wait:
          waitS.us.push_back(us);
          waits++;
          break;
      }
    }
#ifdef CONFIG4_NO_RELEASE_BY_KEY
    const bool byKey = false;
#else
    const bool byKey = step % 2 == 1;
#endif
    for (auto& [i, info] : bound) {
      auto t0 = Clock::now();
#ifndef CONFIG4_NO_RELEASE_BY_KEY
      if (byKey) {
        if (!core.deleteAllocatedPodByKey(keys[i])) {
          fprintf(stderr, "unknown key %s\n", keys[i].c_str());
          return 1;
        }
      } else
#endif
        core.deleteAllocatedPod(specs[i], info, keys[i]);
      double us = usSince(t0);
      if (timed) (byKey ? delKeyS : delS).us.push_back(us);
    }
    if (timed) stepMs.push_back(usSince(ts) / 1e3);
  }
  checkInvariants(core);

  int n = std::max(1, steps);
  printf("config4 core-only: steps=%d warmup=%d per step: binds=%ld waits=%ld preempts=%ld\n", steps,
         warmup, binds / n, waits / n, preempts / n);
  all.report("decision (+commit)");
  waitS.report("schedule -> wait");
  preemptS.report("schedule -> preempt");
  bindS.report("schedule -> bind");
  addS.report("addAllocatedPod");
  delS.report("deleteAllocatedPod");
  delKeyS.report("deleteAllocatedPodByKey");
  std::sort(stepMs.begin(), stepMs.end());
  if (!stepMs.empty()) printf("  ms_per_step p50=%.4f\n", stepMs[stepMs.size() / 2]);
  return 0;
}
```

hivedscheduler_amd/core/core.hpp:

```cpp
#pragma once

#include <algorithm>
#include <cstddef>
#include <map>
#include <memory>
#include <optional>
#include <random>
#include <set>
#include <stdexcept>
#include <string>
#include <unordered_map>
#include <unordered_set>
#include <vector>

namespace hived {

constexpr int kMaxGuaranteedPriority = 1000;
constexpr int kMinGuaranteedPriority = 0;
constexpr int kOpportunisticPriority = -1;
constexpr int kFreePriority = -2;
constexpr int kLowestLevel = 1;
constexpr int kHighestLevel = 100;

enum class CState { Free, Used, Reserving, Reserved };
enum class GState { Allocated, Preempting, BeingPreempted };

const char* to_string(CState s);
const char* to_string(GState s);

struct HivedError : std::runtime_error {
  int code;
  HivedError(int code_, const std::string& msg) : std::runtime_error(msg), code(code_) {}
  static HivedError BadRequest(const std::string& msg) { return HivedError(400, msg); }
  static HivedError NotFound(const std::string& msg) { return HivedError(404, msg); }
  static HivedError Internal(const std::string& msg) { return HivedError(500, msg); }
};

template <class K, size_t N = 16>
class SmallPtrSet {
 public:
  bool empty() const { return n_ == 0 && big_.empty(); }
  size_t count(K* k) const {
    if (!big_.empty()) return big_.count(k);
    for (size_t i = 0; i < n_; i++) {
      if (inl_[i] == k) return 1;
    }
    return 0;
  }
  void insert(K* k) {
    if (count(k)) return;
    if (big_.empty() && n_ < N) {
      inl_[n_++] = k;
      return;
    }
    for (size_t i = 0; i < n_; i++) big_.insert(inl_[i]);
    n_ = 0;
    big_.insert(k);
  }
  void erase(K* k) {
    if (!big_.empty()) {
      big_.erase(k);
      return;
    }
    for (size_t i = 0; i < n_; i++) {
      if (inl_[i] == k) {
        inl_[i] = inl_[--n_];
        return;
      }
    }
  }

 private:
  K* inl_[N];
  size_t n_ = 0;
  std::unordered_set<K*> big_;
};

template <class K, class V, size_t N = 32>
class SmallPtrMap {
 public:
  bool empty() const { return n_ == 0 && big_.empty(); }
  V* find(K* k) {
    if (!big_.empty()) {
      auto it = big_.find(k);
      return it == big_.end() ? nullptr : &it->second;
    }
    for (size_t i = 0; i < n_; i++) {
      if (inl_[i].first == k) return &inl_[i].second;
    }
    return nullptr;
  }
  const V* find(K* k) const { return const_cast<SmallPtrMap*>(this)->find(k); }
  size_t count(K* k) const { return find(k) != nullptr ? 1 : 0; }
  V& at(K* k) {
    V* v = find(k);
    if (v == nullptr) throw std::out_of_range("SmallPtrMap::at");
    return *v;
  }
  V& operator[](K* k) {
    if (V* v = find(k)) return *v;
    if (big_.empty() && n_ < N) {
      inl_[n_] = {k, V{}};
      return inl_[n_++].second;
    }
    for (size_t i = 0; i < n_; i++) big_.emplace(inl_[i].first, inl_[i].second);
    n_ = 0;
    return big_[k];
  }
  void erase(K* k) {
    if (!big_.empty()) {
      big_.erase(k);
      return;
    }
    for (size_t i = 0; i < n_; i++) {
      if (inl_[i].first == k) {
        inl_[i] = inl_[--n_];
        return;
      }
    }
  }
  void clear() {
    n_ = 0;
    big_.clear();
  }
  template <class F>
  void forEach(F f) const {
    for (size_t i = 0; i < n_; i++) f(inl_[i].first, inl_[i].second);
    for (auto& [k, v] : big_) f(k, v);
  }

 private:
  std::pair<K*, V> inl_[N];
  size_t n_ = 0;
  std::unordered_map<K*, V> big_;
};

template <class T, size_t N = 16>
class SmallBuf {
 public:
  explicit SmallBuf(size_t n, const T& init = T{}) : n_(n) {
    if (n > N) {
      heap_.assign(n, init);
      p_ = heap_.data();
    } else {
      p_ = inl_;
      for (size_t i = 0; i < n; i++) inl_[i] = init;
    }
  }
  SmallBuf(const SmallBuf&) = delete;
  SmallBuf& operator=(const SmallBuf&) = delete;
  T& operator[](size_t i) { return p_[i]; }
  const T& operator[](size_t i) const { return p_[i]; }
  T* begin() { return p_; }
  T* end() { return p_ + n_; }
  size_t size() const { return n_; }

 private:
  T inl_[N];
  std::vector<T> heap_;
  T* p_;
  size_t n_;
};

template <class It, class Less>
void stableSortSmall(It first, It last, Less less) {
  if (last - first > 16) {
    std::stable_sort(first, last, less);
    return;
  }
  for (It i = first == last ? last : first + 1; i != last; ++i) {
    auto moving = *i;
    It j = i;
    for (; j != first && less(moving, *(j - 1)); --j) *j = *(j - 1);
    *j = moving;
  }
}

struct Group;
struct PhysicalCell;
struct VirtualCell;

struct Cell {
  std::string chain;
  int level = 0;
  int totalLeaf = 0;
  std::string address;
  std::string typeName;
  bool atOrAboveNode = false;
  bool isNodeLevel = false;
  Cell* parent = nullptr;
  std::vector<Cell*> children;
  int priority = kFreePriority;
  bool healthy = true;
  std::map<int, int> usedLeafAtPriority;
  int freeLeavesUnder = 0;

  virtual ~Cell() = default;
  virtual bool isPhysical() const = 0;
  int usedAt(int p) const {
    auto it = usedLeafAtPriority.find(p);
    return it == usedLeafAtPriority.end() ? 0 : it->second;
  }
};

struct PhysicalCell : Cell {
  std::vector<std::string> nodes;
  std::vector<int> leafIndices;
  CState state = CState::Free;
  bool split = false;
  bool pinned = false;
  std::string pinnedId;
  VirtualCell* virt = nullptr;
  Group* usingGroup = nullptr;
  Group* reservingGroup = nullptr;
  std::string otVC;
  long long hbmBytes = 0;
  int badLinksUnder = 0;
  std::vector<PhysicalCell*> badLinkPeers;
  bool isPhysical() const override { return true; }
};

struct XgmiLink {
  PhysicalCell* a = nullptr;
  PhysicalCell* b = nullptr;
  double gbps = 0.0;
  bool healthy = true;
};

struct VirtualCell : Cell {
  std::string vc;
  VirtualCell* preassigned = nullptr;
  PhysicalCell* phys = nullptr;
  std::string pinnedId;
  bool isPhysical() const override { return false; }
};

struct ChainCellList {
  std::vector<std::vector<Cell*>> byLevel;
  int top() const { return static_cast<int>(byLevel.size()) - 1; }
  void init(int topLevel) { byLevel.assign(topLevel + 1, {}); }
  std::vector<Cell*>& at(int l) { return byLevel[l]; }
  const std::vector<Cell*>& at(int l) const { return byLevel[l]; }
  bool contains(Cell* c, int l) const {
    if (l < 0 || l >= static_cast<int>(byLevel.size())) return false;
    auto& v = byLevel[l];
    return std::find(v.begin(), v.end(), c) != v.end();
  }
  void remove(Cell* c, int l) {
    auto& v = byLevel[l];
    auto it = std::find(v.begin(), v.end(), c);
    if (it == v.end()) throw HivedError::Internal("cell not found in list when removing: " + c->address);
    *it = v.back();
    v.pop_back();
  }
  void add(Cell* c, int l) { byLevel[l].push_back(c); }
  ChainCellList shallowCopy() const { return *this; }
};

struct PodPlacementInfo {
  std::string node;
  std::vector<int> leafIndices;
  std::vector<std::string> preassignedTypes;
};
struct BindInfo {
  std::string node;
  std::vector<int> isolation;
  std::string chain;
  std::vector<std::vector<PodPlacementInfo>> memberBindInfo;
};

struct AllocatedPod {
  bool present = false;
  std::string key;
  std::string node;
  BindInfo bindInfo;
};

struct LazyPreemptionStatus {
  std::string preemptor;
  std::string preemptionTime;
};

struct Group {
  std::string name;
  std::string vc;
  bool lazyPreemptionEnable = false;
  bool ignoreK8sSuggestedNodes = true;
  bool gangReleaseEnable = false;
  int priority = 0;
  GState state = GState::Allocated;
  std::map<int, int> totalPodNums;
  std::map<int, std::vector<AllocatedPod>> allocatedPods;
  std::map<int, std::vector<std::vector<PhysicalCell*>>> physPlacement;
  bool hasVirtualPlacement = true;
  std::map<int, std::vector<std::vector<VirtualCell*>>> virtPlacement;
  std::set<std::string> preemptingPods;
  std::optional<LazyPreemptionStatus> lazyStatus;
};

struct CellTypeSpec {
  std::string child;
  int childCount = 0;
  bool isNode = false;
};
struct PhysCellSpec {
  std::string type;
  std::string address;
  std::string pinnedId;
  std::vector<PhysCellSpec> children;
  long long hbmBytes = 0;
  std::vector<std::tuple<int, int, double, bool>> xgmiLinks;
};
struct VirtCellSpec {
  std::string typePath;
  int number = 0;
};
struct VCSpec {
  std::vector<VirtCellSpec> virtualCells;
  std::vector<std::string> pinnedIds;
};
struct ClusterSpec {
  std::map<std::string, CellTypeSpec> cellTypes;
  std::vector<PhysCellSpec> physicalCells;
  std::map<std::string, VCSpec> virtualClusters;
};

struct PodSpec {
  std::string vc;
  int priority = 0;
  std::string pinnedCellId;
  std::string leafCellType;
  int leafCellNumber = 0;
  bool gangReleaseEnable = false;
  bool lazyPreemptionEnable = false;
  bool ignoreK8sSuggestedNodes = true;
  std::string groupName;
  std::map<int, int> groupPodNums;
  long long hbmBytesPerCell = 0;
};

enum class Phase { Filtering, Preempting };

struct ScheduleResult {
  enum class Kind { Bind, Preempt, Wait } kind = Kind::Wait;
  BindInfo bindInfo;
  std::string victimNode;
  std::vector<std::string> victimPodKeys;
  std::string waitReason;
};

template <class CellT>
using Placement = std::map<int, std::vector<std::vector<CellT*>>>;

struct CleanShapeWorld {
  int priority = kOpportunisticPriority;
  std::map<int, int> caps;
  std::unordered_set<PhysicalCell*> excluded;
  std::map<int, std::vector<PhysicalCell*>> physByLevel;
};

class TopoScheduler;
struct IntraVCScheduler;

struct SchedulingRequest {
  explicit SchedulingRequest(const PodSpec& s)
      : vc(s.vc),
        pinnedCellId(s.pinnedCellId),
        groupName(s.groupName),
        podLeafCellNums(s.groupPodNums),
        priority(s.priority) {}
  const std::string& vc;
  const std::string& pinnedCellId;
  const std::string& groupName;
  const std::map<int, int>& podLeafCellNums;
  const std::string* chain = nullptr;
  IntraVCScheduler* vcScheduler = nullptr;
  const TopoScheduler* topo = nullptr;
  int priority = 0;
  const std::set<std::string>* suggestedNodes = nullptr;
  bool ignoreSuggestedNodes = true;
  long long hbmBytes = 0;
  const CleanShapeWorld* cleanWorld = nullptr;
  bool honorLinksOnly = false;
};

class TopoScheduler {
 public:
  TopoScheduler() = default;
  TopoScheduler(const ChainCellList& ccl, std::map<int, int> levelLeafNum, bool crossPriorityPack);

  bool Schedule(const std::map<int, int>& podLeafCellNums, int priority,
                const std::set<std::string>& suggestedNodes, bool ignoreSuggestedNodes,
                Placement<Cell>* out, std::string* failedReason,
                long long minHbmBytes = 0,
                const CleanShapeWorld* cleanWorld = nullptr, bool honorOnly = false) const;

 private:
  struct NodeView {
    Cell* c = nullptr;
    int freeAtPriority = 0;
    int usedSamePriority = 0;
    int usedHigherPriority = 0;
    bool healthy = true;
    bool suggested = true;
  };
  bool tryScheduleAtPriority(const std::vector<int>& sortedLeafNums, int priority,
                             const std::set<std::string>& suggestedNodes, bool ignoreSuggestedNodes,
                             long long minHbmBytes, bool honorLinks,
                             const CleanShapeWorld* cleanWorld, Placement<Cell>* out,
                             std::string* failedReason) const;

  std::vector<Cell*> viewCells_;
  std::map<int, int> levelLeafNum_;
  bool crossPriorityPack_ = false;
  struct Scratch {
    std::vector<NodeView> view;
    std::vector<int> sortedLeafNums;
    std::vector<int> pickedNodeIndices;
  };
  mutable Scratch scratch_;
};

struct IntraVCScheduler {
  std::map<std::string, ChainCellList> nonPinnedFull;
  std::map<std::string, ChainCellList> nonPinnedPreassigned;
  std::map<std::string, ChainCellList> pinned;
  std::map<std::string, TopoScheduler> nonPinnedSchedulers;
  std::map<std::string, TopoScheduler> pinnedSchedulers;

  bool schedule(const SchedulingRequest& sr, Placement<VirtualCell>* out, std::string* failedReason) const;
};

struct BindingVertex {
  VirtualCell* cell = nullptr;
  std::vector<BindingVertex*> children;
};

using CellBindings = SmallPtrMap<VirtualCell, PhysicalCell*, 32>;

class HivedCore {
 public:
  explicit HivedCore(const ClusterSpec& spec);
  ~HivedCore();

  void setNodeHealthy(const std::string& node, bool healthy);
  void setLeafCellHealthy(const std::string& node, int leafIndex, bool healthy);
  void setXgmiLinkHealthy(const std::string& node, int a, int b, bool healthy,
                          double gbps = 0.0);
  std::vector<std::tuple<int, int, double, bool>> xgmiLinks(const std::string& node) const;
  std::vector<std::string> allNodes() const;
  std::set<std::string> badNodes() const { return badNodes_; }

  ScheduleResult schedule(const PodSpec& s, const std::string& podKey,
                          const std::set<std::string>& suggestedNodes, Phase phase);
  void deleteUnallocatedPod(const PodSpec& s, const std::string& podKey);
  void addAllocatedPod(const PodSpec& s, const BindInfo& info, const std::string& podKey);
  void deleteAllocatedPod(const PodSpec& s, const BindInfo& info, const std::string& podKey);
  bool deleteAllocatedPodByKey(const std::string& podKey);

  const std::map<std::string, std::unique_ptr<Group>>& groups() const { return groups_; }
  const std::map<std::string, ChainCellList>& fullCellList() const { return fullCellList_; }
  const std::map<std::string, ChainCellList>& freeCellList() const { return freeCellList_; }
  const std::map<std::string, IntraVCScheduler>& vcSchedulers() const { return vcSchedulers_; }
  std::vector<std::string> chains() const;
  std::map<int, std::string> chainLevelTypes(const std::string& chain) const;

 private:
  friend struct BuildContext;

  void buildFromSpec(const ClusterSpec& spec);
  void initCellNums();
  void initPinnedCells();
  void initBadNodes();

  void setBadCell(PhysicalCell* c);
  void setHealthyCell(PhysicalCell* c);
  void addBadFreeCell(PhysicalCell* c);
  void removeBadFreeCell(PhysicalCell* c);
  bool doomAllocationIsSafe(PhysicalCell* pc);
  void tryBindDoomedBadCell(const std::string& chain, int level);
  void tryUnbindDoomedBadCell(const std::string& chain, int level);
  void doBindDoomedBadCell(const std::string& chain, int level);
  void doUnbindDoomedBadCell(const std::string& chain, int level);
  void drainDoomChecks();

  class OpGuard {
   public:
    explicit OpGuard(HivedCore* c)
        : c_(c), outer_(!c->inOperation_), exceptionsAtEntry_(std::uncaught_exceptions()) {
      c_->inOperation_ = true;
    }
    ~OpGuard() noexcept(false) {
      if (!outer_) return;
      c_->inOperation_ = false;
      if (std::uncaught_exceptions() == exceptionsAtEntry_) c_->drainDoomChecks();
    }

   private:
    HivedCore* c_;
    bool outer_;
    int exceptionsAtEntry_;
  };

  ScheduleResult generateResult(const Placement<PhysicalCell>& phys, bool hasVirtual,
                                const Placement<VirtualCell>& virt,
                                const std::map<std::string, std::set<std::string>>& victims,
                                std::string&& waitReason, int currentLeafNum, int podIndex,
                                Group* group, const std::string& groupName);
  bool schedulePodFromExistingGroup(Group* g, const PodSpec& s,
                                    const std::set<std::string>& suggestedNodes, Phase phase,
                                    const std::string& podKey, Placement<PhysicalCell>* phys,
                                    bool* hasVirtual, Placement<VirtualCell>* virt,
                                    std::map<std::string, std::set<std::string>>* victims,
                                    int* podIndex);
  void schedulePodFromNewGroup(const PodSpec& s, const std::set<std::string>& suggestedNodes,
                               Phase phase, const std::string& podKey,
                               Placement<PhysicalCell>* phys, bool* hasVirtual,
                               Placement<VirtualCell>* virt,
                               std::map<std::string, std::set<std::string>>* victims,
                               std::string* waitReason);
  bool scheduleNewAffinityGroup(const PodSpec& s, const std::set<std::string>& suggestedNodes,
                                const std::string& podKey, Placement<PhysicalCell>* phys,
                                bool* hasVirtual, Placement<VirtualCell>* virt,
                                std::string* failedReason);
  bool scheduleForLeafCellType(SchedulingRequest& sr, const std::string& leafCellType,
                               const std::vector<std::string>& chains,
                               const std::string& podKey, bool typeSpecified,
                               Placement<PhysicalCell>* phys, bool* hasVirtual,
                               Placement<VirtualCell>* virt, std::string* failedReason);
  bool handleSchedulingRequest(SchedulingRequest& sr, Placement<PhysicalCell>* phys,
                               bool* hasVirtual, Placement<VirtualCell>* virt,
                               std::string* failedReason);
  bool scheduleGuaranteedGroup(SchedulingRequest& sr, Placement<PhysicalCell>* phys,
                               Placement<VirtualCell>* virt, std::string* failedReason);
  static bool chainHasBadLinks(const ChainCellList& fullCells);
  bool scheduleOpportunisticGroup(const SchedulingRequest& sr, Placement<PhysicalCell>* phys,
                                  std::string* failedReason);
  void validateSchedulingRequest(SchedulingRequest& sr, const std::string& podKey);

  std::map<std::string, Placement<VirtualCell>> tryLazyPreempt(const Placement<VirtualCell>& p,
                                                               const std::string& groupName);

  void setPodSlot(Group* g, int leafCellNum, int podIndex, bool releasable,
                  const std::string& podKey, const BindInfo& info);
  void clearPodSlot(Group* g, int leafCellNum, int podIndex);
  void eraseGroup(Group* g);

  Group* createAllocatedGroup(const PodSpec& s, const BindInfo& info, const std::string& podKey);
  void deleteAllocatedGroup(Group* g, const std::string& podKey);
  void createPreemptingGroup(const PodSpec& s, const Placement<PhysicalCell>& phys,
                             const Placement<VirtualCell>& virt, const std::string& podKey);
  void deletePreemptingGroup(Group* g, const std::string& podKey);
  void allocatePreemptingGroup(Group* g, const std::string& podKey);
  Placement<VirtualCell> lazyPreemptGroup(Group* victim, const std::string& preemptor);
  void lazyPreemptCell(VirtualCell* c, const std::string& preemptor);
  void revertLazyPreempt(Group* g, const Placement<VirtualCell>& virt);

  std::pair<PhysicalCell*, VirtualCell*> findAllocatedLeafCell(
      int index, const PodPlacementInfo& placement, const std::string& chain, const PodSpec& s,
      Group* group, const std::string& podKey, bool* lazyPreempt, bool* isOpportunistic);
  std::pair<bool, std::string> allocateLeafCell(PhysicalCell* p, VirtualCell* v, int priority,
                                                const std::string& vc);
  void releaseLeafCell(PhysicalCell* p, const std::string& vc);
  std::pair<bool, std::string> allocatePreassignedCell(PhysicalCell* c, const std::string& vc,
                                                       bool doomedBad);
  void releasePreassignedCell(PhysicalCell* c, const std::string& vc, bool doomedBad);
  void allocateBadCell(PhysicalCell* c);
  void releaseBadCell(PhysicalCell* c);
  int removeCellFromFreeList(PhysicalCell* c);
  int addCellToFreeList(PhysicalCell* c);

  bool mapVirtualPlacementToPhysical(const std::vector<BindingVertex*>& preassigned,
                                     const std::vector<std::vector<BindingVertex*>>& nonPreassigned,
                                     size_t nonPreassignedCount, ChainCellList& freeList,
                                     std::map<int, int>& freeCellNum,
                                     const std::set<std::string>& suggestedNodes,
                                     bool ignoreSuggestedNodes, CellBindings& bindings,
                                     long long minHbmBytes = 0, bool honorLinks = false,
                                     const CleanShapeWorld* world = nullptr);

  struct MapScratch {
    std::vector<std::unique_ptr<BindingVertex>> vertexPool;
    size_t verticesUsed = 0;
    std::vector<BindingVertex*> preassigned;
    std::vector<std::vector<BindingVertex*>> nonPreassigned;
    size_t nonPreassignedUsed = 0;
    std::vector<VirtualCell*> path;
    ChainCellList freeList;
    std::map<int, int> freeCellNum;
    void reset() {
      verticesUsed = 0;
      preassigned.clear();
      nonPreassignedUsed = 0;
    }
    BindingVertex* newVertex(VirtualCell* cell) {
      if (verticesUsed == vertexPool.size()) vertexPool.push_back(std::make_unique<BindingVertex>());
      BindingVertex* v = vertexPool[verticesUsed++].get();
      v->cell = cell;
      v->children.clear();
      return v;
    }
    std::vector<BindingVertex*>& newNonPreassignedGroup() {
      if (nonPreassignedUsed == nonPreassigned.size()) nonPreassigned.emplace_back();
      std::vector<BindingVertex*>& g = nonPreassigned[nonPreassignedUsed++];
      g.clear();
      return g;
    }
  };
  MapScratch mapScratch_;

 public:
  std::map<std::string, ChainCellList> fullCellList_;
  std::map<std::string, ChainCellList> freeCellList_;
  bool inOperation_ = false;
  std::vector<std::pair<std::string, int>> pendingDoomChecks_;
  std::map<std::string, IntraVCScheduler> vcSchedulers_;
  std::map<std::string, TopoScheduler> opportunisticSchedulers_;
  std::map<std::string, std::unique_ptr<Group>> groups_;
  struct PodSlotRef {
    Group* group = nullptr;
    int leafCellNum = 0;
    int podIndex = 0;
    bool releasable = true;
  };
  std::unordered_map<std::string, PodSlotRef> podIndex_;

  std::map<std::string, std::map<std::string, std::map<int, int>>> vcFreeCellNum_;
  std::map<std::string, std::map<int, int>> allVCFreeCellNum_;
  std::map<std::string, std::map<int, int>> totalLeftCellNum_;

  std::map<std::string, ChainCellList> badFreeCells_;
  std::map<std::string, std::map<std::string, ChainCellList>> vcDoomedBadCells_;
  std::map<std::string, std::map<int, int>> allVCDoomedBadCellNum_;

  std::set<std::string> badNodes_;
  std::set<PhysicalCell*> badLeafMarks_;
  std::map<std::string, std::map<std::pair<int, int>, XgmiLink>> xgmiLinks_;
  std::map<std::string, std::vector<std::string>> cellChains_;
  std::map<std::string, std::map<int, std::string>> cellTypes_;
  std::map<std::string, std::map<int, int>> leafCellNums_;
  std::map<std::string, std::map<std::string, PhysicalCell*>> pinnedPhysical_;

  std::minstd_rand victimRng_{12345};
  std::vector<std::unique_ptr<Cell>> cellStore_;
  std::map<std::string, std::vector<PhysicalCell*>> nodeLeafCellsStorage_;
  long long scheduleCount_ = 0;
  struct WorldCacheEntry {
    unsigned long long epoch = 0;
    std::vector<CleanShapeWorld> worlds;
  };
  std::map<std::pair<std::string, int>, WorldCacheEntry> worldCache_;
};

extern unsigned long long gWorldEpochCounter;
void setCellPriority(Cell* c, int p);
void updateUsedLeafCellNumAtPriority(Cell* c, int p, bool increase);
void bindCell(PhysicalCell* pc, VirtualCell* vc);
void unbindCell(PhysicalCell* c);
VirtualCell* getUnboundVirtualCell(const std::vector<Cell*>& cl);
VirtualCell* getLowestPriorityVirtualCell(const std::vector<Cell*>& cl, int p);
VirtualCell* mapPhysicalCellToVirtual(PhysicalCell* c, const ChainCellList& vccl,
                                      int preassignedLevel, int p, std::string* message);
bool inFreeCellList(PhysicalCell* c);
void setCellState(PhysicalCell* c, CState s);
PhysicalCell* findPhysicalLeafCell(std::map<std::string, ChainCellList>& fullCellList,
                                   const std::string& chain, const std::string& node,
                                   int leafIndex);
Cell* ancestorNoHigherThanNode(Cell* c);
std::vector<CleanShapeWorld> computeCleanShapeWorlds(
    const ChainCellList& ccl, const std::set<std::string>* suggestedNodes,
    size_t maxWorlds = 4, int priority = kOpportunisticPriority);
void checkInvariants(const HivedCore& core);

}
```

hivedscheduler_amd/core/debug.cpp:

```cpp
#include <sstream>

#include "core.hpp"

namespace hived {

namespace {

void fail(const std::string& what) { throw HivedError::Internal("invariant violated: " + what); }

int countFreeListSubtree(const ChainCellList& freeList, int level) {
  int count = 0;
  for (int l = level; l <= freeList.top(); l++) {
    int mult = 1;
    bool ok = true;
    for (Cell* c : freeList.at(l)) {
      Cell* probe = c;
      mult = 1;
      while (probe->level > level) {
        mult *= static_cast<int>(probe->children.size());
        probe = probe->children[0];
      }
      if (ok) count += mult;
    }
  }
  return count;
}

}

void checkInvariants(const HivedCore& core) {
  for (auto& [chain, ccl] : core.fullCellList_) {
    for (int l = ccl.top(); l >= kLowestLevel; l--) {
      for (Cell* cc : ccl.at(l)) {
        auto* c = static_cast<PhysicalCell*>(cc);
        if (!c->children.empty()) {
          int maxPrio = kFreePriority;
          bool allHealthy = true;
          bool anyUsed = false;
          std::map<int, int> usedSum;
          for (Cell* childC : c->children) {
            auto* child = static_cast<PhysicalCell*>(childC);
            maxPrio = std::max(maxPrio, child->priority);
            allHealthy = allHealthy && child->healthy;
            anyUsed = anyUsed || (child->state == CState::Used);
            for (auto& [p, n] : child->usedLeafAtPriority) usedSum[p] += n;
          }
          if (c->priority != maxPrio) {
            fail("priority roll-up at " + c->address + ": " + std::to_string(c->priority) +
                 " != max(children) " + std::to_string(maxPrio));
          }
          int freeSum = 0;
          for (Cell* childC : c->children) freeSum += childC->freeLeavesUnder;
          if (c->freeLeavesUnder != freeSum) {
            fail("freeLeavesUnder roll-up at " + c->address + ": " +
                 std::to_string(c->freeLeavesUnder) + " != sum(children) " +
                 std::to_string(freeSum));
          }
          if (c->healthy != allHealthy) fail("healthiness roll-up at " + c->address);
          if (anyUsed && c->state != CState::Used) fail("state roll-up (Used) at " + c->address);
          if (usedSum != c->usedLeafAtPriority) fail("usedLeafAtPriority roll-up at " + c->address);
        } else if (c->freeLeavesUnder != (c->priority == kFreePriority ? 1 : 0)) {
          fail("leaf freeLeavesUnder at " + c->address);
        }
        if (c->virt != nullptr && c->virt->phys != c) fail("asymmetric binding at " + c->address);
      }
    }
  }
  {
    std::unordered_map<const Cell*, int> expect;
    for (auto& [node, links] : core.xgmiLinks_) {
      (void)node;
      for (auto& [key, l] : links) {
        (void)key;
        if (l.healthy) continue;
        auto hasPeer = [](PhysicalCell* from, PhysicalCell* to) {
          return std::find(from->badLinkPeers.begin(), from->badLinkPeers.end(), to) !=
                 from->badLinkPeers.end();
        };
        if (!hasPeer(l.a, l.b) || !hasPeer(l.b, l.a)) {
          fail("bad xGMI link " + l.a->address + "<->" + l.b->address +
               " not mirrored in badLinkPeers");
        }
        Cell* x = l.a;
        Cell* y = l.b;
        while (x != y && x != nullptr && y != nullptr) {
          x = x->parent;
          y = y->parent;
        }
        for (Cell* c = x; c != nullptr; c = c->parent) expect[c]++;
      }
    }
    for (auto& [chain, ccl] : core.fullCellList_) {
      (void)chain;
      for (int l = ccl.top(); l >= kLowestLevel; l--) {
        for (Cell* cc : ccl.at(l)) {
          auto* c = static_cast<PhysicalCell*>(cc);
          int want = expect.count(c) ? expect[c] : 0;
          if (c->badLinksUnder != want) {
            fail("badLinksUnder roll-up at " + c->address + ": " +
                 std::to_string(c->badLinksUnder) + " != " + std::to_string(want));
          }
        }
      }
    }
  }
  for (auto& [chain, freeList] : core.freeCellList_) {
    for (int l = freeList.top(); l >= kLowestLevel; l--) {
      for (Cell* cc : freeList.at(l)) {
        auto* c = static_cast<PhysicalCell*>(cc);
        if (c->virt != nullptr) fail("free cell " + c->address + " is bound");
        if (c->split) fail("free cell " + c->address + " is split");
        if (c->parent != nullptr && !static_cast<PhysicalCell*>(c->parent)->split) {
          fail("free cell " + c->address + " has unsplit parent (should be merged)");
        }
        if (c->priority >= kMinGuaranteedPriority) {
          fail("free cell " + c->address + " has guaranteed priority " +
               std::to_string(c->priority));
        }
      }
    }
    auto tlIt = core.totalLeftCellNum_.find(chain);
    if (tlIt != core.totalLeftCellNum_.end()) {
      for (auto& [level, left] : tlIt->second) {
        int actual = countFreeListSubtree(freeList, level);
        if (actual != left) {
          std::ostringstream os;
          os << "totalLeftCellNum mismatch at chain " << chain << " level " << level
             << ": accounted " << left << ", free list yields " << actual;
          fail(os.str());
        }
      }
    }
  }
  for (auto& [chain, perLevel] : core.allVCFreeCellNum_) {
    auto tlIt = core.totalLeftCellNum_.find(chain);
    if (tlIt == core.totalLeftCellNum_.end()) continue;
    for (auto& [level, vcFree] : perLevel) {
      auto it = tlIt->second.find(level);
      int left = it == tlIt->second.end() ? 0 : it->second;
      if (left < vcFree) {
        std::ostringstream os;
        os << "VC safety broken at chain " << chain << " level " << level << ": " << left
           << " left < " << vcFree << " free in all VCs";
        fail(os.str());
      }
    }
  }
  std::map<std::string, std::map<int, int>> sum;
  for (auto& [vc, perChain] : core.vcFreeCellNum_) {
    (void)vc;
    for (auto& [chain, perLevel] : perChain) {
      for (auto& [level, n] : perLevel) sum[chain][level] += n;
    }
  }
  for (auto& [chain, perLevel] : core.allVCFreeCellNum_) {
    for (auto& [level, n] : perLevel) {
      int s = sum.count(chain) && sum[chain].count(level) ? sum[chain][level] : 0;
      if (s != n) {
        fail("allVCFreeCellNum mismatch at " + chain + " level " + std::to_string(level));
      }
    }
  }
  for (auto& [vcName, perChain] : core.vcDoomedBadCells_) {
    for (auto& [chain, ccl] : perChain) {
      for (int l = 1; l <= ccl.top(); l++) {
        for (Cell* cc : ccl.at(l)) {
          auto* pc = static_cast<PhysicalCell*>(cc);
          if (pc->virt == nullptr) {
            fail("doomed bad cell " + pc->address + " (VC " + vcName + ", chain " + chain +
                 ") has no binding");
          }
          if (pc->virt->phys != pc) fail("doomed bad cell " + pc->address + " binding asymmetric");
        }
      }
    }
  }
  for (auto& [vcName, vcs] : core.vcSchedulers_) {
    (void)vcName;
    for (auto& [chain, ccl] : vcs.nonPinnedFull) {
      (void)chain;
      for (int l = ccl.top(); l >= kLowestLevel; l--) {
        for (Cell* cc : ccl.at(l)) {
          auto* v = static_cast<VirtualCell*>(cc);
          if (v->phys != nullptr && v->phys->virt != v) {
            fail("asymmetric virtual binding at " + v->address);
          }
          if (!v->children.empty()) {
            int maxPrio = kFreePriority;
            int freeSum = 0;
            for (Cell* child : v->children) {
              maxPrio = std::max(maxPrio, child->priority);
              freeSum += child->freeLeavesUnder;
            }
            if (v->priority != maxPrio) fail("virtual priority roll-up at " + v->address);
            if (v->freeLeavesUnder != freeSum) {
              fail("virtual freeLeavesUnder roll-up at " + v->address);
            }
          } else if (v->freeLeavesUnder != (v->priority == kFreePriority ? 1 : 0)) {
            fail("virtual leaf freeLeavesUnder at " + v->address);
          }
        }
      }
    }
  }
  for (auto& [name, g] : core.groups_) {
    (void)name;
    for (auto& [leafNum, pods] : g->physPlacement) {
      (void)leafNum;
      for (auto& pod : pods) {
        for (PhysicalCell* c : pod) {
          if (c == nullptr) continue;
          if (g->state == GState::Allocated && c->state == CState::Used &&
              c->usingGroup != g.get() && c->usingGroup != nullptr) {
          }
          if (g->state == GState::Preempting &&
              (c->state == CState::Reserving || c->state == CState::Reserved) &&
              c->reservingGroup != g.get()) {
            fail("reserved cell " + c->address + " does not reference its preemptor");
          }
        }
      }
    }
  }
}

}
```

hivedscheduler_amd/core/sched_bench_main.cpp:

```cpp
#include <algorithm>
#include <chrono>
#include <cstdio>
#include <cstdlib>
#include <random>
#include <vector>

#include "core.hpp"

using namespace hived;

static ClusterSpec makeSpec(int nodes) {
  ClusterSpec spec;
  spec.cellTypes["MI355X"] = {"", 0, false};
  spec.cellTypes["MI355X-PAIR"] = {"MI355X", 2, false};
  spec.cellTypes["MI355X-QUAD"] = {"MI355X-PAIR", 2, false};
  CellTypeSpec node;
  node.child = "MI355X-QUAD";
  node.childCount = 2;
  node.isNode = true;
  spec.cellTypes["MI355X-NODE"] = node;
  for (int i = 0; i < nodes; i++) {
    PhysCellSpec n;
    n.type = "MI355X-NODE";
    n.address = "node" + std::to_string(i + 1);
    int g = 0;
    for (int q = 0; q < 2; q++) {
      PhysCellSpec quad;
      for (int p = 0; p < 2; p++) {
        PhysCellSpec pair;
        for (int l = 0; l < 2; l++) {
          PhysCellSpec leaf;
          leaf.address = std::to_string(g++);
          pair.children.push_back(leaf);
        }
        quad.children.push_back(pair);
      }
      n.children.push_back(quad);
    }
    spec.physicalCells.push_back(n);
  }
  VCSpec vc1, vc2;
  VirtCellSpec v;
  v.typePath = "MI355X-NODE";
  v.number = nodes / 2;
  vc1.virtualCells.push_back(v);
  v.number = nodes - nodes / 2;
  vc2.virtualCells.push_back(v);
  spec.virtualClusters["VC1"] = vc1;
  spec.virtualClusters["VC2"] = vc2;
  return spec;
}

int main(int argc, char** argv) {
  int nodes = argc > 1 ? atoi(argv[1]) : 128;
  int nreq = argc > 2 ? atoi(argv[2]) : 2000;
  int badLinks = argc > 3 ? atoi(argv[3]) : 0;
  auto tb0 = std::chrono::steady_clock::now();
  HivedCore core(makeSpec(nodes));
  for (int i = 0; i < nodes; i++) core.setNodeHealthy("node" + std::to_string(i + 1), true);
  {
    std::mt19937 lrng(7);
    for (int i = 0; i < badLinks; i++) {
      int n = (int)(lrng() % nodes) + 1;
      int a = (int)(lrng() % 8), b = (int)(lrng() % 8);
      if (a == b) b = (a + 1) % 8;
      core.setXgmiLinkHealthy("node" + std::to_string(n), a, b, false, 12.0);
    }
  }
  auto tb1 = std::chrono::steady_clock::now();

  std::mt19937 rng(0);
  std::set<std::string> suggested;
  std::vector<double> lat;
  lat.reserve(nreq);
  struct LivePod {
    PodSpec spec;
    BindInfo info;
    std::string key;
  };
  std::vector<LivePod> live;
  int cells[] = {1, 2, 4};
  for (int i = 0; i < nreq; i++) {
    PodSpec s;
    s.vc = (rng() % 2) ? "VC1" : "VC2";
    s.priority = (int)(rng() % 2);
    s.leafCellNumber = cells[rng() % 3];
    s.groupName = "g" + std::to_string(i);
    s.groupPodNums[s.leafCellNumber] = 1;
    std::string key = "ns/p" + std::to_string(i);
    auto t0 = std::chrono::steady_clock::now();
    ScheduleResult r = core.schedule(s, key, suggested, Phase::Filtering);
    if (r.kind == ScheduleResult::Kind::Bind) {
      core.addAllocatedPod(s, r.bindInfo, key);
    }
    auto t1 = std::chrono::steady_clock::now();
    lat.push_back(std::chrono::duration<double, std::micro>(t1 - t0).count());
    if (r.kind == ScheduleResult::Kind::Bind) {
      live.push_back({s, r.bindInfo, key});
    }
    if ((int)live.size() > nodes * 4) {
      core.deleteAllocatedPod(live.front().spec, live.front().info, live.front().key);
      live.erase(live.begin());
    }
  }
  std::sort(lat.begin(), lat.end());
  printf("nodes=%d reqs=%d badLinks=%d build=%.1fms p50=%.1fus p90=%.1fus p99=%.1fus\n", nodes, nreq,
         badLinks,
         std::chrono::duration<double, std::milli>(tb1 - tb0).count(), lat[lat.size() / 2],
         lat[(size_t)(lat.size() * 0.90)], lat[(size_t)(lat.size() * 0.99)]);
  return 0;
}
```

hivedscheduler_amd/core/topo_sched.cpp:

```cpp
#include <climits>
#include <functional>

#include "core.hpp"

namespace hived {

TopoScheduler::TopoScheduler(const ChainCellList& ccl, std::map<int, int> levelLeafNum,
                             bool crossPriorityPack)
    : levelLeafNum_(std::move(levelLeafNum)), crossPriorityPack_(crossPriorityPack) {
  int top = ccl.top();
  int nodeLevel = top;
  for (int l = 1; l <= top; l++) {
    if (!ccl.at(l).empty() && ccl.at(l)[0]->atOrAboveNode) {
      nodeLevel = l;
      break;
    }
  }
  std::unordered_set<Cell*> seen;
  for (int l = std::min(nodeLevel, top); l >= 1; l--) {
    for (Cell* c : ccl.at(l)) {
      Cell* v = ancestorNoHigherThanNode(c);
      if (seen.insert(v).second) viewCells_.push_back(v);
    }
  }
// ... 261 lines not shown
  for (Cell* c : toExclude) s.excluded.insert(c);
}

int bestLCALevel(Cell* c, int q, int p, const PickSession& s) {
  auto [t, f] = availLeaves(c, p, s);
  (void)f;
  if (t < q) return INT_MAX;
  int best = c->level;
  for (Cell* child : c->children) {
    int b = bestLCALevel(child, q, p, s);
    if (b < best) best = b;
  }
  return best;
}

void pickLeaves(Cell* cell, int q, int p, PickSession& s, std::vector<Cell*>& out) {
  if (cell->level == kLowestLevel) {
    s.taken.insert(cell);
    out.push_back(cell);
    return;
  }
  int n = static_cast<int>(cell->children.size());
  SmallBuf<std::pair<int, int>, 8> av(n);
  for (int i = 0; i < n; i++) av[i] = availLeaves(cell->children[i], p, s);

  int best = -1, bestLca = INT_MAX;
  for (int i = 0; i < n; i++) {
    if (av[i].first >= q) {
      int lca = bestLCALevel(cell->children[i], q, p, s);
      if (best < 0) {
        best = i;
        bestLca = lca;
        continue;
      }
      int needPreempt = std::max(0, q - av[i].second);
      int bestPreempt = std::max(0, q - av[best].second);
      int linkKey = badLinksUnderOf(cell->children[i]);
      int bestLinkKey = badLinksUnderOf(cell->children[best]);
      if (q == 1) {
        linkKey = -linkKey;
        bestLinkKey = -bestLinkKey;
      }
      if (lca < bestLca ||
          (lca == bestLca &&
           (needPreempt < bestPreempt ||
            (needPreempt == bestPreempt &&
             (linkKey < bestLinkKey ||
              (linkKey == bestLinkKey && av[i].first < av[best].first)))))) {
        best = i;
        bestLca = lca;
      }
    }
  }
  if (best >= 0) {
    pickLeaves(cell->children[best], q, p, s, out);
    return;
  }
  SmallBuf<int, 8> order(n);
  for (int i = 0; i < n; i++) order[i] = i;
  stableSortSmall(order.begin(), order.end(),
                  [&](int a, int b) { return av[a].first > av[b].first; });
  int remaining = q;
  for (int idx : order) {
    if (remaining == 0) break;
    int t = std::min(remaining, av[idx].first);
    if (t > 0) {
      pickLeaves(cell->children[idx], t, p, s, out);
      remaining -= t;
    }
  }
  if (remaining != 0) throw HivedError::Internal("pickLeaves underflow in " + cell->address);
}

struct WorldPair {
  Cell* child;
  PhysicalCell* hint;
  int avail;
};

bool matchWorldChildren(Cell* cell, PhysicalCell* hint, int p, const PickSession& s,
                        std::vector<WorldPair>& pairs) {
  std::vector<Cell*> unboundChildren;
  std::vector<PhysicalCell*> freeHints;
  for (Cell* childC : cell->children) {
    auto* vc = static_cast<VirtualCell*>(childC);
    if (vc->phys != nullptr) {
      pairs.push_back({vc, vc->phys, 0});
    } else {
      unboundChildren.push_back(vc);
    }
  }
  for (Cell* hc : hint->children) {
    auto* ph = static_cast<PhysicalCell*>(hc);
    if (ph->virt == nullptr) freeHints.push_back(ph);
  }
  if (freeHints.size() < unboundChildren.size()) return false;
  std::stable_sort(freeHints.begin(), freeHints.end(), [&](PhysicalCell* a, PhysicalCell* b) {
    return physFreeInWorld(a, s) > physFreeInWorld(b, s);
  });
  std::stable_sort(unboundChildren.begin(), unboundChildren.end(), [&](Cell* a, Cell* b) {
    return availLeaves(a, p, s).first > availLeaves(b, p, s).first;
  });
  for (size_t i = 0; i < unboundChildren.size(); i++) {
    pairs.push_back({unboundChildren[i], freeHints[i], 0});
  }
  return true;
}

int availWorld(Cell* cell, PhysicalCell* hint, int p, const PickSession& s) {
  if (cell->level == kLowestLevel) {
    auto [t, f] = availLeaves(cell, p, s);
    (void)f;
    return std::min(t, physFreeInWorld(hint, s));
  }
  std::vector<WorldPair> pairs;
  if (!matchWorldChildren(cell, hint, p, s, pairs)) return 0;
  int total = 0;
  for (auto& pr : pairs) total += availWorld(pr.child, pr.hint, p, s);
  return total;
}

bool pickLeavesWorld(Cell* cell, PhysicalCell* hint, int q, int p, PickSession& s,
                     std::vector<Cell*>& out) {
  if (cell->level == kLowestLevel) {
    if (availWorld(cell, hint, p, s) < 1) return false;
    s.taken.insert(cell);
    s.physTaken.insert(hint);
    s.hintTaken[cell] = hint;
    out.push_back(cell);
    return true;
  }
  std::vector<WorldPair> pairs;
  if (!matchWorldChildren(cell, hint, p, s, pairs)) return false;
  int total = 0;
  for (auto& pr : pairs) {
    pr.avail = availWorld(pr.child, pr.hint, p, s);
    total += pr.avail;
  }
  if (total < q) return false;
  int best = -1;
  for (size_t i = 0; i < pairs.size(); i++) {
    if (pairs[i].avail >= q && (best < 0 || pairs[i].avail < pairs[best].avail)) {
      best = static_cast<int>(i);
    }
  }
  if (best >= 0) {
    return pickLeavesWorld(pairs[best].child, pairs[best].hint, q, p, s, out);
  }
  std::stable_sort(pairs.begin(), pairs.end(), [](const WorldPair& a, const WorldPair& b) {
    return a.avail > b.avail;
  });
  int remaining = q;
  size_t outStart = out.size();
  for (auto& pr : pairs) {
    if (remaining == 0) break;
    int t = std::min(remaining, pr.avail);
    if (t > 0) {
      if (!pickLeavesWorld(pr.child, pr.hint, t, p, s, out)) {
        for (size_t i = outStart; i < out.size(); i++) {
          s.taken.erase(out[i]);
          auto it = s.hintTaken.find(out[i]);
          if (it != s.hintTaken.end()) {
            s.physTaken.erase(it->second);
            s.hintTaken.erase(it);
          }
        }
        out.resize(outStart);
        return false;
      }
      remaining -= t;
    }
  }
  if (remaining != 0) {
    for (size_t i = outStart; i < out.size(); i++) {
      s.taken.erase(out[i]);
      auto it = s.hintTaken.find(out[i]);
      if (it != s.hintTaken.end()) {
        s.physTaken.erase(it->second);
        s.hintTaken.erase(it);
      }
    }
    out.resize(outStart);
    return false;
  }
  return true;
}

std::vector<PhysicalCell*> resolveWorldHints(Cell* cell, int q, const PickSession& s) {
  auto* vc = static_cast<VirtualCell*>(cell);
  if (vc->phys != nullptr) return {vc->phys};
  PhysicalCell* region = nullptr;
  for (Cell* a = cell->parent; a != nullptr; a = a->parent) {
    PhysicalCell* ap = static_cast<VirtualCell*>(a)->phys;
    if (ap != nullptr) {
      region = ap;
      break;
    }
  }
  std::vector<PhysicalCell*> candidates;
  auto consider = [&](PhysicalCell* ph) {
    if (ph->virt != nullptr) return;
    if (physFreeInWorld(ph, s) >= q) candidates.push_back(ph);
  };
  if (region != nullptr) {
    std::function<void(PhysicalCell*)> walk = [&](PhysicalCell* ph) {
      if (ph->level == cell->level) {
        consider(ph);
        return;
      }
      for (Cell* c : ph->children) walk(static_cast<PhysicalCell*>(c));
    };
    walk(region);
  } else {
    auto it = s.world->physByLevel.find(cell->level);
    if (it != s.world->physByLevel.end()) {
      for (PhysicalCell* ph : it->second) consider(ph);
    }
  }
  std::stable_sort(candidates.begin(), candidates.end(),
                   [&](PhysicalCell* a, PhysicalCell* b) {
                     return physFreeInWorld(a, s) < physFreeInWorld(b, s);
                   });
  return candidates;
}

std::tuple<bool, bool> healthyAndSuggested(Cell* c, const std::set<std::string>& suggestedNodes,
                                           bool ignoreSuggestedNodes) {
  PhysicalCell* pc = physOf(c);
  if (pc == nullptr) return {true, true};
  bool suggested =
      ignoreSuggestedNodes || (!pc->nodes.empty() && suggestedNodes.count(pc->nodes[0]) > 0);
  return {pc->healthy, suggested};
}

}

std::vector<CleanShapeWorld> computeCleanShapeWorlds(
    const ChainCellList& ccl, const std::set<std::string>* suggestedNodes, size_t maxWorlds,
    int priority) {
  PickSession base;
  base.suggestedFilter = suggestedNodes;
  int top = ccl.top();
  std::vector<std::vector<std::vector<Cell*>>> perCell;
  for (Cell* c : ccl.at(top)) {
    auto variants = enumerateCleanExclusionVariants(c, base, maxWorlds, priority);
    if (!variants.empty()) perCell.push_back(std::move(variants));
  }
  std::vector<CleanShapeWorld> worlds;
  std::map<int, std::vector<PhysicalCell*>> physByLevel;
  std::map<int, int> cleanCellBest;
  PickSession noExcl = base;
  for (int l = kLowestLevel; l <= top; l++) {
    int best = 0;
    for (Cell* c : ccl.at(l)) {
      auto* ph = static_cast<PhysicalCell*>(c);
      if (ph->virt == nullptr) physByLevel[l].push_back(ph);
      if (ph->badLinksUnder == 0) {
        best = std::max(best, availLeaves(c, priority, noExcl).first);
      }
    }
    cleanCellBest[l] = best;
  }
  std::vector<size_t> idx(perCell.size(), 0);
  for (;;) {
    CleanShapeWorld w;
    PickSession session = base;
    for (size_t i = 0; i < perCell.size(); i++) {
      for (Cell* e : perCell[i][idx[i]]) {
        session.excluded.insert(e);
        w.excluded.insert(static_cast<PhysicalCell*>(e));
      }
    }
    w.priority = priority;
    for (int l = kLowestLevel; l <= top; l++) {
      int best = cleanCellBest[l];
      for (Cell* c : ccl.at(l)) {
        auto* ph = static_cast<PhysicalCell*>(c);
        if (ph->badLinksUnder > 0) {
          best = std::max(best, availLeaves(c, priority, session).first);
        }
      }
      w.caps[l] = best;
    }
    w.physByLevel = physByLevel;
    worlds.push_back(std::move(w));
    if (worlds.size() >= maxWorlds || perCell.empty()) break;
    size_t d = 0;
    while (d < perCell.size()) {
      if (++idx[d] < perCell[d].size()) break;
      idx[d] = 0;
      d++;
    }
    if (d == perCell.size()) break;
  }
  if (worlds.empty()) worlds.push_back(CleanShapeWorld{});
  return worlds;
}


bool TopoScheduler::tryScheduleAtPriority(const std::vector<int>& sortedLeafNums, int priority,
                                          const std::set<std::string>& suggestedNodes,
                                          bool ignoreSuggestedNodes, long long minHbmBytes,
                                          bool honorLinks, const CleanShapeWorld* cleanWorld,
                                          Placement<Cell>* out,
                                          std::string* failedReason) const {
  std::vector<NodeView>& cv = scratch_.view;
  cv.clear();
  cv.reserve(viewCells_.size());
  PickSession probe;
  probe.minHbm = minHbmBytes;
  if (honorLinks) probe.world = cleanWorld;
  int totalLeafNum = 0;
  for (int q : sortedLeafNums) totalLeafNum += q;
  long long freeSum = 0;
  int freeMax = 0;
  bool allSuggested = true;
  for (Cell* c : viewCells_) {
    NodeView n;
    n.c = c;
    n.usedSamePriority = c->usedAt(priority);
    n.usedHigherPriority = 0;
    for (auto& [p, num] : c->usedLeafAtPriority) {
      if (crossPriorityPack_) {
        if (p != priority) n.usedSamePriority += num;
      } else if (p > priority) {
        n.usedHigherPriority += num;
      }
    }
    if (honorLinks && probe.world == nullptr && badLinksUnderOf(c) > 0) {
      n.freeAtPriority = cleanAvailAnalysis(c, priority, probe, INT_MAX, nullptr);
    } else {
      n.freeAtPriority = availLeaves(c, priority, probe).first;
    }
    auto [healthy, suggested] = healthyAndSuggested(c, suggestedNodes, ignoreSuggestedNodes);
    n.healthy = healthy;
    n.suggested = suggested;
    freeSum += n.freeAtPriority;
    freeMax = std::max(freeMax, n.freeAtPriority);
    allSuggested = allSuggested && suggested;
    cv.push_back(n);
  }
  if (allSuggested && (totalLeafNum > freeSum ||
                       (sortedLeafNums.size() == 1 && sortedLeafNums[0] > freeMax))) {
    *failedReason = "insufficient capacity";
    return false;
  }
  auto before = [](const NodeView& a, const NodeView& b) {
    if (a.healthy != b.healthy) return a.healthy;
    if (a.suggested != b.suggested) return a.suggested;
    if (a.usedSamePriority != b.usedSamePriority) return a.usedSamePriority > b.usedSamePriority;
    return a.usedHigherPriority < b.usedHigherPriority;
  };
  for (size_t i = 1; i < cv.size(); i++) {
    if (!before(cv[i], cv[i - 1])) continue;
    NodeView moving = cv[i];
    size_t j = i;
    for (; j > 0 && before(moving, cv[j - 1]); j--) cv[j] = cv[j - 1];
    cv[j] = moving;
  }

  std::vector<int>& pickedNodeIndices = scratch_.pickedNodeIndices;
  pickedNodeIndices.assign(sortedLeafNums.size(), -1);
  size_t podIndex = 0;
  int pickedLeafCellNum = 0;
  for (size_t nodeIndex = 0; nodeIndex < cv.size(); nodeIndex++) {
    const NodeView& n = cv[nodeIndex];
    if (n.freeAtPriority >= totalLeafNum) {
      if (!n.suggested) continue;
      for (size_t i = 0; i < sortedLeafNums.size(); i++) {
        pickedNodeIndices[i] = static_cast<int>(nodeIndex);
      }
      podIndex = sortedLeafNums.size();
      break;
    }
  }
  for (size_t nodeIndex = 0; nodeIndex < cv.size() && podIndex < sortedLeafNums.size();) {
    const NodeView& n = cv[nodeIndex];
    if (n.freeAtPriority - pickedLeafCellNum >= sortedLeafNums[podIndex]) {
      if (!n.suggested) {
        *failedReason = "have to use at least one non-suggested node " + n.c->address;
        return false;
      }
      pickedNodeIndices[podIndex] = static_cast<int>(nodeIndex);
      pickedLeafCellNum += sortedLeafNums[podIndex];
      podIndex++;
    } else {
      pickedLeafCellNum = 0;
      nodeIndex++;
    }
  }
  if (podIndex < sortedLeafNums.size()) {
    *failedReason = "insufficient capacity";
    return false;
  }

  PickSession session;
  session.minHbm = minHbmBytes;
  if (honorLinks) {
    session.world = cleanWorld;
    if (cleanWorld == nullptr) {
      for (size_t i = 0; i < sortedLeafNums.size();) {
        const int nodeIndex = pickedNodeIndices[i];
        int demand = 0;
        for (; i < sortedLeafNums.size() && pickedNodeIndices[i] == nodeIndex; i++) {
          demand += sortedLeafNums[i];
        }
        if (demand >= 2) applyLinkExclusions(cv[nodeIndex].c, demand, priority, session);
      }
    }
  }
  out->clear();
  for (size_t i = 0; i < sortedLeafNums.size(); i++) {
    int q = sortedLeafNums[i];
    Cell* node = cv[pickedNodeIndices[i]].c;
    std::vector<Cell*> leaves;
    leaves.reserve(q);
    if (session.world != nullptr && !node->isPhysical()) {
      bool placed = false;
      for (PhysicalCell* hint : resolveWorldHints(node, q, session)) {
        if (pickLeavesWorld(node, hint, q, priority, session, leaves)) {
          placed = true;
          break;
        }
      }
      if (!placed) {
        *failedReason = "no link-clean shape in this world";
        return false;
      }
    } else {
      pickLeaves(node, q, priority, session, leaves);
    }
    (*out)[q].push_back(std::move(leaves));
  }
  return true;
}

bool TopoScheduler::Schedule(const std::map<int, int>& podLeafCellNums, int priority,
                             const std::set<std::string>& suggestedNodes,
                             bool ignoreSuggestedNodes, Placement<Cell>* out,
                             std::string* failedReason, long long minHbmBytes,
                             const CleanShapeWorld* cleanWorld, bool honorOnly) const {
  std::vector<int>& sortedLeafNums = scratch_.sortedLeafNums;
  sortedLeafNums.clear();
  for (auto& [leafNum, podNum] : podLeafCellNums) {
    for (int i = 0; i < podNum; i++) sortedLeafNums.push_back(leafNum);
  }
  bool anyBadLinks = cleanWorld != nullptr;
  for (Cell* c : viewCells_) {
    if (anyBadLinks || badLinksUnderOf(c) > 0) {
      anyBadLinks = true;
      break;
    }
  }
  auto attempt = [&](int p, bool honorLinks) {
    return tryScheduleAtPriority(sortedLeafNums, p, suggestedNodes, ignoreSuggestedNodes,
                                 minHbmBytes, honorLinks, cleanWorld, out, failedReason);
  };
  if (honorOnly) return attempt(cleanWorld != nullptr ? cleanWorld->priority : priority, true);
  if (attempt(kOpportunisticPriority, true)) return true;
  if (anyBadLinks && attempt(kOpportunisticPriority, false)) return true;
  if (priority > kOpportunisticPriority) {
    if (attempt(priority, true)) return true;
    if (anyBadLinks && attempt(priority, false)) return true;
  }
  return false;
}

bool IntraVCScheduler::schedule(const SchedulingRequest& sr, Placement<VirtualCell>* out,
                                std::string* failedReason) const {
  const TopoScheduler* scheduler = sr.topo;
  Placement<Cell> generic;
  if (scheduler == nullptr ||
      !scheduler->Schedule(sr.podLeafCellNums, sr.priority, *sr.suggestedNodes,
                           sr.ignoreSuggestedNodes, &generic, failedReason, sr.hbmBytes,
                           sr.cleanWorld, sr.honorLinksOnly)) {
    if (failedReason->empty()) *failedReason = "no scheduler for request";
    failedReason->append(" when scheduling in VC ").append(sr.vc);
    return false;
  }
  out->clear();
  for (auto& [leafNum, pods] : generic) {
    for (auto& pod : pods) {
      std::vector<VirtualCell*> cells;
      cells.reserve(pod.size());
      for (Cell* c : pod) cells.push_back(static_cast<VirtualCell*>(c));
      (*out)[leafNum].push_back(std::move(cells));
    }
  }
  return true;
}

}
```

Before: 791.0 ns.

## Replace map/set/vector scheduler containers with flat pooled structures and shared bind info

Swaps the std::map/set victim and placement containers for flat leaf maps, a contiguous PodCells block, a reusable VictimList scratch and a pooled Group node cache. Placements now go straight into the typed output through a sink, with no intermediate generic copy. BindInfo is shared by pointer instead of copied, the bad-node check exits early, and the Python bindings cache interned name strings. The aim is to cut heap allocations and copies on each schedule call, at the cost of much more custom container code and API changes across callers.

```diff
diff --git a/hivedscheduler_amd/core/algorithm.cpp b/hivedscheduler_amd/core/algorithm.cpp
--- a/hivedscheduler_amd/core/algorithm.cpp
+++ b/hivedscheduler_amd/core/algorithm.cpp
@@ -14,13 +14,12 @@
 namespace {
 constexpr size_t kWaitReasonReserve = 128;
 
-struct Victims {
-  std::map<std::string, std::set<std::string>> byNode;
-  std::set<Group*> overlappingPreemptors;
-};
-
-Victims collectPreemptionVictims(const Placement<PhysicalCell>& placement) {
-  Victims v;
+using OverlappingPreemptors = std::vector<Group*>;
+
+OverlappingPreemptors collectPreemptionVictims(const Placement<PhysicalCell>& placement,
+                                               VictimList* victims) {
+  OverlappingPreemptors overlapping;
+  victims->clear();
   for (auto& [leafNum, pods] : placement) {
     (void)leafNum;
     for (auto& pod : pods) {
@@ -28,38 +27,41 @@
         if (c == nullptr) continue;
         if ((c->state == CState::Used || c->state == CState::Reserving) &&
             c->usingGroup != nullptr) {
-          for (auto& [ln, victims] : c->usingGroup->allocatedPods) {
+          for (auto& [ln, slots] : c->usingGroup->allocatedPods) {
             (void)ln;
-            for (auto& p : victims) {
-              if (p.present) v.byNode[p.node].insert(p.key);
+            for (auto& p : slots) {
+              if (p.present) victims->add(p.node, p.key);
             }
           }
         }
         if (c->state == CState::Reserving || c->state == CState::Reserved) {
-          v.overlappingPreemptors.insert(c->reservingGroup);
-        }
-      }
-    }
-  }
-  return v;
-}
-
-std::set<std::string> collectBadOrNonSuggestedNodes(const Placement<PhysicalCell>& placement,
-                                                    const std::set<std::string>& suggestedNodes,
-                                                    bool ignoreSuggestedNodes) {
-  std::set<std::string> bad;
+          if (std::find(overlapping.begin(), overlapping.end(), c->reservingGroup) ==
+              overlapping.end()) {
+            overlapping.push_back(c->reservingGroup);
+          }
+        }
+      }
+    }
+  }
+  if (!victims->empty()) victims->seal();
+  return overlapping;
+}
+
+bool usesBadOrNonSuggestedNode(const Placement<PhysicalCell>& placement,
+                               const std::set<std::string>& suggestedNodes,
+                               bool ignoreSuggestedNodes) {
   for (auto& [leafNum, pods] : placement) {
     (void)leafNum;
     for (auto& pod : pods) {
       for (PhysicalCell* c : pod) {
         if (c == nullptr) continue;
         if (!c->healthy || (!ignoreSuggestedNodes && !suggestedNodes.count(c->nodes[0]))) {
-          bad.insert(c->nodes[0]);
-        }
-      }
-    }
-  }
-  return bad;
+          return true;
+        }
+      }
+    }
+  }
+  return false;
 }
 
 std::pair<PodPlacementInfo, std::string> retrieveMissingPodPlacement(Group* g, int leafCellNum,
@@ -68,10 +70,10 @@
     (void)ln;
     for (auto& p : pods) {
       if (!p.present) continue;
-      for (auto& mbi : p.bindInfo.memberBindInfo) {
+      for (auto& mbi : p.bindInfo->memberBindInfo) {
         if (!mbi.empty() && static_cast<int>(mbi[0].leafIndices.size()) == leafCellNum &&
             podIndex < static_cast<int>(mbi.size())) {
-          return {mbi[podIndex], p.bindInfo.chain};
+          return {mbi[podIndex], p.bindInfo->chain};
         }
       }
     }
@@ -94,7 +96,7 @@
   return nullptr;
 }
 
-int getNewPodIndex(const std::vector<AllocatedPod>& pods) {
+int getNewPodIndex(const PodSlots& pods) {
   for (size_t i = 0; i < pods.size(); i++) {
     if (!pods[i].present) return static_cast<int>(i);
   }
@@ -116,7 +118,7 @@
   return -1;
 }
 
-bool allPodsReleased(const std::map<int, std::vector<AllocatedPod>>& allocatedPods) {
+bool allPodsReleased(const FlatLeafMap<PodSlots>& allocatedPods) {
   for (auto& [ln, pods] : allocatedPods) {
     (void)ln;
     for (auto& p : pods) {
@@ -134,8 +136,7 @@
   return false;
 }
 
-std::unique_ptr<Group> newGroup(const PodSpec& s, GState state) {
-  auto g = std::make_unique<Group>();
+void initGroup(Group* g, const PodSpec& s, GState state) {
   g->name = s.groupName;
   g->vc = s.vc;
   g->lazyPreemptionEnable = s.lazyPreemptionEnable;
@@ -146,14 +147,9 @@
   g->totalPodNums = s.groupPodNums;
   for (auto& [leafNum, podNum] : s.groupPodNums) {
     g->allocatedPods[leafNum].resize(podNum);
-    auto& phys = g->physPlacement[leafNum];
-    phys.resize(podNum);
-    for (auto& pod : phys) pod.assign(leafNum, nullptr);
-    auto& virt = g->virtPlacement[leafNum];
-    virt.resize(podNum);
-    for (auto& pod : virt) pod.assign(leafNum, nullptr);
-  }
-  return g;
+    g->physPlacement[leafNum].assign(podNum, leafNum);
+    g->virtPlacement[leafNum].assign(podNum, leafNum);
+  }
 }
 
 }
@@ -166,7 +162,8 @@
   Placement<PhysicalCell> phys;
   Placement<VirtualCell> virt;
   bool hasVirtual = true;
-  std::map<std::string, std::set<std::string>> victims;
+  VictimList& victims = victimScratch_;
+  victims.clear();
   std::string waitReason;
   waitReason.reserve(kWaitReasonReserve);
   int podIndex = 0;
@@ -197,7 +194,7 @@
 
 ScheduleResult HivedCore::generateResult(const Placement<PhysicalCell>& phys, bool hasVirtual,
                                          const Placement<VirtualCell>& virt,
-                                         const std::map<std::string, std::set<std::string>>& victims,
+                                         const VictimList& victims,
                                          std::string&& waitReason, int currentLeafNum,
                                          int podIndex, Group* group,
                                          const std::string& groupName) {
@@ -213,14 +210,13 @@
   }
   if (!victims.empty()) {
     r.kind = ScheduleResult::Kind::Preempt;
-    auto it = victims.begin();
-    std::advance(it, static_cast<long>(victimRng_() % victims.size()));
-    r.victimNode = it->first;
-    r.victimPodKeys.assign(it->second.begin(), it->second.end());
+    victims.nodeAt(victimRng_() % victims.nodeCount(), &r.victimNode, &r.victimPodKeys);
     return r;
   }
   r.kind = ScheduleResult::Kind::Bind;
-  BindInfo& info = r.bindInfo;
+  auto built = std::make_shared<BindInfo>();
+  BindInfo& info = *built;
+  info.memberBindInfo.reserve(phys.size());
   for (auto& [leafNum, pods] : phys) {
     std::vector<PodPlacementInfo> placements(pods.size());
     for (size_t pi = 0; pi < pods.size(); pi++) {
@@ -263,6 +259,7 @@
     }
     info.memberBindInfo.push_back(std::move(placements));
   }
+  r.bindInfo = std::move(built);
   return r;
 }
 
@@ -270,10 +267,8 @@
 bool HivedCore::schedulePodFromExistingGroup(
     Group* g, const PodSpec& s, const std::set<std::string>& suggestedNodes, Phase phase,
     const std::string& podKey, Placement<PhysicalCell>* phys, bool* hasVirtual,
-    Placement<VirtualCell>* virt, std::map<std::string, std::set<std::string>>* victims,
+    Placement<VirtualCell>* virt, VictimList* victims,
     int* podIndex) {
-  std::set<std::string> badNodes =
-      collectBadOrNonSuggestedNodes(g->physPlacement, suggestedNodes, g->ignoreK8sSuggestedNodes);
   if (g->state == GState::Allocated) {
     *phys = g->physPlacement;
     *hasVirtual = g->hasVirtualPlacement;
@@ -288,15 +283,15 @@
     *podIndex = idx;
     return true;
   }
-  if (phase == Phase::Preempting && !badNodes.empty()) {
+  if (phase == Phase::Preempting &&
+      usesBadOrNonSuggestedNode(g->physPlacement, suggestedNodes, g->ignoreK8sSuggestedNodes)) {
     deletePreemptingGroup(g, podKey);
     return false;
   }
   *phys = g->physPlacement;
   *hasVirtual = g->hasVirtualPlacement;
   *virt = g->virtPlacement;
-  Victims v = collectPreemptionVictims(g->physPlacement);
-  *victims = std::move(v.byNode);
+  collectPreemptionVictims(g->physPlacement, victims);
   g->preemptingPods.insert(podKey);
   return true;
 }
@@ -305,16 +300,15 @@
                                         const std::set<std::string>& suggestedNodes, Phase phase,
                                         const std::string& podKey, Placement<PhysicalCell>* phys,
                                         bool* hasVirtual, Placement<VirtualCell>* virt,
-                                        std::map<std::string, std::set<std::string>>* victims,
+                                        VictimList* victims,
                                         std::string* waitReason) {
   if (!scheduleNewAffinityGroup(s, suggestedNodes, podKey, phys, hasVirtual, virt, waitReason)) {
     phys->clear();
     return;
   }
-  Victims v = collectPreemptionVictims(*phys);
-  *victims = std::move(v.byNode);
+  OverlappingPreemptors overlapping = collectPreemptionVictims(*phys, victims);
   if (phase == Phase::Preempting) {
-    for (Group* preemptor : v.overlappingPreemptors) {
+    for (Group* preemptor : overlapping) {
       deletePreemptingGroup(preemptor, podKey);
     }
     if (!victims->empty()) {
@@ -516,11 +510,10 @@
     if (mapped) {
       phys->clear();
       for (auto& [leafNum, pods] : *virt) {
+        PodCells<PhysicalCell>& physPods = (*phys)[leafNum];
         for (auto& pod : pods) {
-          std::vector<PhysicalCell*> cells;
-          cells.reserve(pod.size());
-          for (VirtualCell* v : pod) cells.push_back(bindings.at(v));
-          (*phys)[leafNum].push_back(std::move(cells));
+          PhysicalCell** cells = physPods.appendPod(pod.size());
+          for (size_t i = 0; i < pod.size(); i++) cells[i] = bindings.at(pod[i]);
         }
       }
       return true;
@@ -602,20 +595,10 @@
 bool HivedCore::scheduleOpportunisticGroup(const SchedulingRequest& sr,
                                            Placement<PhysicalCell>* phys,
                                            std::string* failedReason) {
-  Placement<Cell> generic;
   if (!sr.topo->Schedule(sr.podLeafCellNums, kOpportunisticPriority, *sr.suggestedNodes,
-                         sr.ignoreSuggestedNodes, &generic, failedReason, sr.hbmBytes)) {
+                         sr.ignoreSuggestedNodes, phys, failedReason, sr.hbmBytes)) {
     failedReason->append(" when scheduling in physical cluster");
     return false;
-  }
-  phys->clear();
-  for (auto& [leafNum, pods] : generic) {
-    for (auto& pod : pods) {
-      std::vector<PhysicalCell*> cells;
-      cells.reserve(pod.size());
-      for (Cell* c : pod) cells.push_back(static_cast<PhysicalCell*>(c));
-      (*phys)[leafNum].push_back(std::move(cells));
-    }
   }
   return true;
 }
@@ -633,6 +616,17 @@
 }
 
 void HivedCore::addAllocatedPod(const PodSpec& s, const BindInfo& info, const std::string& podKey) {
+  addAllocatedPodShared(s, info, nullptr, podKey);
+}
+
+void HivedCore::addAllocatedPod(const PodSpec& s, const std::shared_ptr<const BindInfo>& info,
+                                const std::string& podKey) {
+  addAllocatedPodShared(s, *info, &info, podKey);
+}
+
+void HivedCore::addAllocatedPodShared(const PodSpec& s, const BindInfo& info,
+                                      const std::shared_ptr<const BindInfo>* shared,
+                                      const std::string& podKey) {
   OpGuard opGuard(this);
   int podIndex = 0;
   bool releasable = true;
@@ -651,7 +645,8 @@
       releasable = false;
     }
   }
-  setPodSlot(g, s.leafCellNumber, podIndex, releasable, podKey, info);
+  setPodSlot(g, s.leafCellNumber, podIndex, releasable, podKey,
+             shared != nullptr ? *shared : std::make_shared<const BindInfo>(info));
 }
 
 void HivedCore::deleteAllocatedPod(const PodSpec& s, const BindInfo& info,
@@ -683,15 +678,15 @@
 }
 
 void HivedCore::setPodSlot(Group* g, int leafCellNum, int podIndex, bool releasable,
-                           const std::string& podKey, const BindInfo& info) {
+                           const std::string& podKey, std::shared_ptr<const BindInfo> info) {
   auto& slots = g->allocatedPods[leafCellNum];
   if (podIndex >= static_cast<int>(slots.size())) slots.resize(podIndex + 1);
   AllocatedPod& slot = slots[podIndex];
   if (slot.present && slot.key != podKey) clearPodSlot(g, leafCellNum, podIndex);
   slot.present = true;
   slot.key = podKey;
-  slot.node = info.node;
-  slot.bindInfo = info;
+  slot.node = info->node;
+  slot.bindInfo = std::move(info);
   podIndex_[podKey] = PodSlotRef{g, leafCellNum, podIndex, releasable};
 }
 
@@ -715,24 +710,47 @@
       if (pods[i].present) clearPodSlot(g, leafNum, static_cast<int>(i));
     }
   }
-  groups_.erase(g->name);
+  auto it = groups_.find(g->name);
+  if (it == groups_.end()) return;
+  if (groupPool_.size() >= kGroupPoolMax) {
+    groups_.erase(it);
+    return;
+  }
+  GroupNode node = groups_.extract(it);
+  node.mapped()->reset();
+  groupPool_.push_back(std::move(node));
+}
+
+Group* HivedCore::insertNewGroup(const PodSpec& s, GState state) {
+  Group* g = nullptr;
+  if (!groupPool_.empty()) {
+    GroupNode node = std::move(groupPool_.back());
+    groupPool_.pop_back();
+    node.key() = s.groupName;
+    g = node.mapped().get();
+    auto entered = groups_.insert(std::move(node));
+    if (!entered.inserted) {
+      groupPool_.push_back(std::move(entered.node));
+      throw HivedError::Internal("group " + s.groupName + " already exists");
+    }
+  } else {
+    g = (groups_[s.groupName] = std::make_unique<Group>()).get();
+  }
+  initGroup(g, s, state);
+  return g;
 }
 
 
 Group* HivedCore::createAllocatedGroup(const PodSpec& s, const BindInfo& info,
                                        const std::string& podKey) {
-  auto group = newGroup(s, GState::Allocated);
-  Group* g = group.get();
-  groups_[s.groupName] = std::move(group);
+  Group* g = insertNewGroup(s, GState::Allocated);
   bool shouldLazyPreempt = false;
   for (auto& mbi : info.memberBindInfo) {
     if (mbi.empty()) continue;
     int leafCellNumber = static_cast<int>(mbi[0].leafIndices.size());
     if (!g->physPlacement.count(leafCellNumber)) {
-      g->physPlacement[leafCellNumber].assign(mbi.size(),
-                                              std::vector<PhysicalCell*>(leafCellNumber, nullptr));
-      g->virtPlacement[leafCellNumber].assign(mbi.size(),
-                                              std::vector<VirtualCell*>(leafCellNumber, nullptr));
+      g->physPlacement[leafCellNumber].assign(mbi.size(), leafCellNumber);
+      g->virtPlacement[leafCellNumber].assign(mbi.size(), leafCellNumber);
       g->allocatedPods[leafCellNumber].resize(mbi.size());
     }
     for (size_t podIndex = 0; podIndex < mbi.size(); podIndex++) {
@@ -798,8 +816,7 @@
 void HivedCore::createPreemptingGroup(const PodSpec& s, const Placement<PhysicalCell>& phys,
                                       const Placement<VirtualCell>& virt,
                                       const std::string& podKey) {
-  auto group = newGroup(s, GState::Preempting);
-  Group* g = group.get();
+  Group* g = insertNewGroup(s, GState::Preempting);
   g->physPlacement = phys;
   g->virtPlacement = virt;
   for (auto& [leafNum, pods] : phys) {
@@ -824,7 +841,6 @@
     }
   }
   g->preemptingPods.insert(podKey);
-  groups_[s.groupName] = std::move(group);
 }
 
 void HivedCore::deletePreemptingGroup(Group* g, const std::string& podKey) {
diff --git a/hivedscheduler_amd/core/bindings.cpp b/hivedscheduler_amd/core/bindings.cpp
--- a/hivedscheduler_amd/core/bindings.cpp
+++ b/hivedscheduler_amd/core/bindings.cpp
@@ -456,11 +456,53 @@
   if (PyDict_SetItem(d.ptr(), key, value.ptr()) != 0) throw py::error_already_set();
 }
 
-py::dict bindInfoToDict(const BindInfo& info) {
+class NameStrs {
+ public:
+  NameStrs() { add(std::string()); }
+  NameStrs(const NameStrs&) = delete;
+  NameStrs& operator=(const NameStrs&) = delete;
+  ~NameStrs() {
+    for (auto& [name, o] : strs_) {
+      (void)name;
+      Py_DECREF(o);
+    }
+  }
+  void add(const std::string& name) {
+    if (strs_.count(name)) return;
+    PyObject* o = PyUnicode_FromStringAndSize(name.data(), static_cast<Py_ssize_t>(name.size()));
+    if (o == nullptr) throw py::error_already_set();
+    strs_.emplace(name, o);
+  }
+  PyObject* get(const std::string& name) const {
+    auto it = strs_.find(name);
+    if (it == strs_.end()) {
+      PyObject* o = PyUnicode_FromStringAndSize(name.data(), static_cast<Py_ssize_t>(name.size()));
+      if (o == nullptr) throw py::error_already_set();
+      return o;
+    }
+    Py_INCREF(it->second);
+    return it->second;
+  }
+  py::object str(const std::string& name) const {
+    return py::reinterpret_steal<py::object>(get(name));
+  }
+  py::object strList(const std::vector<std::string>& v) const {
+    py::list l(v.size());
+    for (size_t i = 0; i < v.size(); i++) {
+      PyList_SET_ITEM(l.ptr(), static_cast<Py_ssize_t>(i), get(v[i]));
+    }
+    return std::move(l);
+  }
+
+ private:
+  std::unordered_map<std::string, PyObject*> strs_;
+};
+
+py::dict bindInfoToDict(const BindInfo& info, const NameStrs& names) {
   py::dict d;
-  setItem(d, N.node, pyStr(info.node));
+  setItem(d, N.node, names.str(info.node));
   setItem(d, N.leafCellIsolation, pyIntList(info.isolation));
-  setItem(d, N.cellChain, pyStr(info.chain));
+  setItem(d, N.cellChain, names.str(info.chain));
   py::list mbis(info.memberBindInfo.size());
   for (size_t m = 0; m < info.memberBindInfo.size(); m++) {
     auto& mbi = info.memberBindInfo[m];
@@ -468,9 +510,9 @@
     for (size_t p = 0; p < mbi.size(); p++) {
       auto& pl = mbi[p];
       py::dict pd;
-      setItem(pd, N.physicalNode, pyStr(pl.node));
+      setItem(pd, N.physicalNode, names.str(pl.node));
       setItem(pd, N.physicalLeafCellIndices, pyIntList(pl.leafIndices));
-      setItem(pd, N.preassignedCellTypes, pyStrList(pl.preassignedTypes));
+      setItem(pd, N.preassignedCellTypes, names.strList(pl.preassignedTypes));
       PyList_SET_ITEM(placements.ptr(), static_cast<Py_ssize_t>(p), pd.release().ptr());
     }
     py::dict md;
@@ -599,7 +641,7 @@
   return s;
 }
 
-py::object bindInfoToObject(const BindInfo& info) {
+py::object bindInfoToObject(const BindInfo& info, const NameStrs& names) {
   py::list mbis(info.memberBindInfo.size());
   for (size_t m = 0; m < info.memberBindInfo.size(); m++) {
     auto& mbi = info.memberBindInfo[m];
@@ -607,9 +649,9 @@
     for (size_t p = 0; p < mbi.size(); p++) {
       auto& pl = mbi[p];
       py::object po = newInstance(T.PodPlacementInfo);
-      setAttr(po, N.physicalNode, pyStr(pl.node));
+      setAttr(po, N.physicalNode, names.str(pl.node));
       setAttr(po, N.physicalLeafCellIndices, pyIntList(pl.leafIndices));
-      setAttr(po, N.preassignedCellTypes, pyStrList(pl.preassignedTypes));
+      setAttr(po, N.preassignedCellTypes, names.strList(pl.preassignedTypes));
       PyList_SET_ITEM(placements.ptr(), static_cast<Py_ssize_t>(p), po.release().ptr());
     }
     py::object mo = newInstance(T.AffinityGroupMemberBindInfo);
@@ -617,9 +659,9 @@
     PyList_SET_ITEM(mbis.ptr(), static_cast<Py_ssize_t>(m), mo.release().ptr());
   }
   py::object o = newInstance(T.PodBindInfo);
-  setAttr(o, N.node, pyStr(info.node));
+  setAttr(o, N.node, names.str(info.node));
   setAttr(o, N.leafCellIsolation, pyIntList(info.isolation));
-  setAttr(o, N.cellChain, pyStr(info.chain));
+  setAttr(o, N.cellChain, names.str(info.chain));
   setAttr(o, N.affinityGroupBindInfo, mbis);
   return o;
 }
@@ -631,6 +673,7 @@
   PyObject* victimPodKeys;
   PyObject* waitReason;
   hived::ScheduleResult r;
+  std::shared_ptr<const NameStrs> names;
 };
 
 void resultDealloc(PyObject* self) {
@@ -640,6 +683,7 @@
   Py_XDECREF(o->victimPodKeys);
   Py_XDECREF(o->waitReason);
   o->r.~ScheduleResult();
+  o->names.~shared_ptr();
   Py_TYPE(self)->tp_free(self);
 }
 
@@ -673,7 +717,7 @@
 PyObject* resultBindInfo(PyObject* self, void*) {
   auto* o = reinterpret_cast<PyScheduleResult*>(self);
   if (o->r.kind != hived::ScheduleResult::Kind::Bind) Py_RETURN_NONE;
-  return cachedAttr(&o->bindInfo, [o] { return bindInfoToObject(o->r.bindInfo); });
+  return cachedAttr(&o->bindInfo, [o] { return bindInfoToObject(*o->r.bindInfo, *o->names); });
 }
 PyObject* resultVictimNode(PyObject* self, void*) {
   auto* o = reinterpret_cast<PyScheduleResult*>(self);
@@ -744,11 +788,12 @@
   m.add_object("ScheduleResult", reinterpret_cast<PyObject*>(&ResultType));
 }
 
-py::object makeResult(hived::ScheduleResult&& r) {
+py::object makeResult(hived::ScheduleResult&& r, const std::shared_ptr<const NameStrs>& names) {
   PyScheduleResult* o = PyObject_New(PyScheduleResult, &ResultType);
   if (o == nullptr) throw py::error_already_set();
   o->bindInfo = o->victimNode = o->victimPodKeys = o->waitReason = nullptr;
   new (&o->r) hived::ScheduleResult(std::move(r));
+  new (&o->names) std::shared_ptr<const NameStrs>(names);
   return py::reinterpret_steal<py::object>(reinterpret_cast<PyObject*>(o));
 }
 
@@ -871,10 +916,20 @@
 class PyHivedCore {
  public:
   explicit PyHivedCore(const py::dict& spec) : core_(parseClusterSpec(spec)) {
+    auto names = std::make_shared<NameStrs>();
     for (auto& node : core_.allNodes()) {
-      nodeNames_.push_back(pyStr(node));
+      names->add(node);
+      nodeNames_.push_back(names->str(node));
       allNodeSet_.insert(node);
     }
+    for (auto& chain : core_.chains()) {
+      names->add(chain);
+      for (auto& [level, type] : core_.chainLevelTypes(chain)) {
+        (void)level;
+        names->add(type);
+      }
+    }
+    nameStrs_ = std::move(names);
   }
 
   void setNodeHealthy(const std::string& node, bool healthy) {
@@ -937,7 +992,7 @@
     switch (r.kind) {
       case ScheduleResult::Kind::Bind:
         setItem(d, N.kind, N.bind);
-        setItem(d, N.bindInfo, bindInfoToDict(r.bindInfo));
+        setItem(d, N.bindInfo, bindInfoToDict(*r.bindInfo, *nameStrs_));
         break;
       case ScheduleResult::Kind::Preempt:
         setItem(d, N.kind, N.preempt);
@@ -992,7 +1047,7 @@
       }
       return decided;
     }();
-    return makeResult(std::move(r));
+    return makeResult(std::move(r), nameStrs_);
   }
 
   void deleteUnallocatedPod(py::handle spec, const std::string& podKey) {
@@ -1158,6 +1213,7 @@
  private:
   HivedCore core_;
   std::vector<py::object> nodeNames_;
+  std::shared_ptr<const NameStrs> nameStrs_;
   std::set<std::string> allNodeSet_;
   CoreMutex coreMutex_;
   std::string releaseKey_;
diff --git a/hivedscheduler_amd/core/config4_alloc_main.cpp b/hivedscheduler_amd/core/config4_alloc_main.cpp
--- a/hivedscheduler_amd/core/config4_alloc_main.cpp
+++ b/hivedscheduler_amd/core/config4_alloc_main.cpp
@@ -72,7 +72,7 @@
 
   std::map<std::string, Tally> tallies;
   for (int step = 0; step < warmup + steps; step++) {
-    std::vector<std::pair<int, BindInfo>> bound;
+    std::vector<std::pair<int, std::shared_ptr<const BindInfo>>> bound;
     for (int i = 0; i < kNumRequests; i++) {
       long before = gAllocations;
       ScheduleResult r = core.schedule(specs[i], keys[i], suggested, Phase::Filtering);
@@ -119,7 +119,7 @@
         }
       } else
 #endif
-        core.deleteAllocatedPod(specs[i], info, keys[i]);
+        core.deleteAllocatedPod(specs[i], *info, keys[i]);
       if (step >= warmup) {
         tallies[byKey ? "release (deleteAllocatedPodByKey)" : "release (deleteAllocatedPod)"].add(
             gAllocations - before);
diff --git a/hivedscheduler_amd/core/config4_bench_main.cpp b/hivedscheduler_amd/core/config4_bench_main.cpp
--- a/hivedscheduler_amd/core/config4_bench_main.cpp
+++ b/hivedscheduler_amd/core/config4_bench_main.cpp
@@ -58,7 +58,7 @@
   long binds = 0, waits = 0, preempts = 0;
   for (int step = 0; step < warmup + steps; step++) {
     bool timed = step >= warmup;
-    std::vector<std::pair<int, BindInfo>> bound;
+    std::vector<std::pair<int, std::shared_ptr<const BindInfo>>> bound;
     auto ts = Clock::now();
     for (int i = 0; i < kNumRequests; i++) {
       auto t0 = Clock::now();
@@ -104,7 +104,7 @@
         }
       } else
 #endif
-        core.deleteAllocatedPod(specs[i], info, keys[i]);
+        core.deleteAllocatedPod(specs[i], *info, keys[i]);
       double us = usSince(t0);
       if (timed) (byKey ? delKeyS : delS).us.push_back(us);
     }
diff --git a/hivedscheduler_amd/core/core.hpp b/hivedscheduler_amd/core/core.hpp
--- a/hivedscheduler_amd/core/core.hpp
+++ b/hivedscheduler_amd/core/core.hpp
@@ -4,6 +4,7 @@
 #include <cstddef>
 #include <map>
 #include <memory>
+#include <new>
 #include <optional>
 #include <random>
 #include <set>
@@ -175,6 +176,263 @@
     *j = moving;
   }
 }
+
+
+template <class V, size_t N = 4>
+class FlatIntMap {
+ public:
+  using value_type = std::pair<int, V>;
+  using iterator = value_type*;
+  using const_iterator = const value_type*;
+
+  FlatIntMap() {}
+  FlatIntMap(const FlatIntMap& o) : spill_(o.spill_) {
+    for (; n_ < o.n_; n_++) new (inl() + n_) value_type(o.inl()[n_]);
+  }
+  FlatIntMap(FlatIntMap&& o) noexcept : spill_(std::move(o.spill_)) {
+    for (; n_ < o.n_; n_++) new (inl() + n_) value_type(std::move(o.inl()[n_]));
+    o.clear();
+  }
+  FlatIntMap& operator=(const FlatIntMap& o) {
+    if (this == &o) return *this;
+    clear();
+    for (; n_ < o.n_; n_++) new (inl() + n_) value_type(o.inl()[n_]);
+    spill_ = o.spill_;
+    return *this;
+  }
+  FlatIntMap& operator=(FlatIntMap&& o) noexcept {
+    if (this == &o) return *this;
+    clear();
+    for (; n_ < o.n_; n_++) new (inl() + n_) value_type(std::move(o.inl()[n_]));
+    spill_ = std::move(o.spill_);
+    o.clear();
+    return *this;
+  }
+  ~FlatIntMap() { clear(); }
+
+  bool empty() const { return size() == 0; }
+  size_t size() const { return spill_.empty() ? n_ : spill_.size(); }
+  iterator begin() { return spill_.empty() ? inl() : spill_.data(); }
+  iterator end() { return begin() + size(); }
+  const_iterator begin() const { return spill_.empty() ? inl() : spill_.data(); }
+  const_iterator end() const { return begin() + size(); }
+
+  iterator find(int k) {
+    iterator it = lowerBound(k);
+    return it != end() && it->first == k ? it : end();
+  }
+  const_iterator find(int k) const { return const_cast<FlatIntMap*>(this)->find(k); }
+  size_t count(int k) const { return find(k) != end() ? 1 : 0; }
+  V& at(int k) {
+    iterator it = find(k);
+    if (it == end()) throw std::out_of_range("FlatIntMap::at");
+    return it->second;
+  }
+  const V& at(int k) const { return const_cast<FlatIntMap*>(this)->at(k); }
+  V& operator[](int k) {
+    iterator it = lowerBound(k);
+    if (it != end() && it->first == k) return it->second;
+    const size_t pos = static_cast<size_t>(it - begin());
+    if (spill_.empty() && n_ < N) {
+      if (pos == n_) {
+        new (inl() + n_) value_type(k, V{});
+      } else {
+        new (inl() + n_) value_type(std::move(inl()[n_ - 1]));
+        for (size_t i = n_ - 1; i > pos; i--) inl()[i] = std::move(inl()[i - 1]);
+        inl()[pos] = value_type(k, V{});
+      }
+      n_++;
+      return inl()[pos].second;
+    }
+    if (spill_.empty()) {
+      spill_.reserve(2 * N);
+      for (size_t i = 0; i < n_; i++) spill_.push_back(std::move(inl()[i]));
+      destroyInline();
+    }
+    return spill_.insert(spill_.begin() + static_cast<std::ptrdiff_t>(pos), value_type(k, V{}))
+        ->second;
+  }
+  size_t erase(int k) {
+    iterator it = find(k);
+    if (it == end()) return 0;
+    if (!spill_.empty()) {
+      spill_.erase(spill_.begin() + (it - spill_.data()));
+      return 1;
+    }
+    for (iterator j = it; j + 1 != end(); ++j) *j = std::move(*(j + 1));
+    inl()[--n_].~value_type();
+    return 1;
+  }
+  void clear() {
+    destroyInline();
+    spill_.clear();
+  }
+
+ private:
+  iterator lowerBound(int k) {
+    iterator it = begin();
+    for (iterator e = end(); it != e && it->first < k; ++it) {
+    }
+    return it;
+  }
+  value_type* inl() { return reinterpret_cast<value_type*>(raw_); }
+  const value_type* inl() const { return reinterpret_cast<const value_type*>(raw_); }
+  void destroyInline() {
+    while (n_ > 0) inl()[--n_].~value_type();
+  }
+  alignas(value_type) unsigned char raw_[N * sizeof(value_type)];
+  size_t n_ = 0;
+  std::vector<value_type> spill_;
+};
+
+template <class V, size_t N = 4>
+using FlatLeafMap = FlatIntMap<V, N>;
+
+template <class P>
+struct CellRow {
+  P* p = nullptr;
+  size_t n = 0;
+  P* begin() const { return p; }
+  P* end() const { return p + n; }
+  size_t size() const { return n; }
+  bool empty() const { return n == 0; }
+  P& operator[](size_t i) const { return p[i]; }
+};
+
+template <class T, size_t N = 8>
+class PodCells {
+ public:
+  using Row = CellRow<T*>;
+  using ConstRow = CellRow<T* const>;
+  template <class P>
+  class RowIter {
+   public:
+    RowIter(P* base, size_t cols, size_t i) : base_(base), cols_(cols), i_(i) {}
+    CellRow<P>& operator*() const {
+      row_ = CellRow<P>{base_ + i_ * cols_, cols_};
+      return row_;
+    }
+    RowIter& operator++() {
+      i_++;
+      return *this;
+    }
+    bool operator!=(const RowIter& o) const { return i_ != o.i_; }
+    bool operator==(const RowIter& o) const { return i_ == o.i_; }
+
+   private:
+    P* base_;
+    size_t cols_;
+    size_t i_;
+    mutable CellRow<P> row_;
+  };
+
+  PodCells() {}
+  PodCells(const PodCells& o) : heap_(o.heap_), rows_(o.rows_), cols_(o.cols_) { copyInline(o); }
+  PodCells& operator=(const PodCells& o) {
+    if (this == &o) return *this;
+    heap_ = o.heap_;
+    rows_ = o.rows_;
+    cols_ = o.cols_;
+    copyInline(o);
+    return *this;
+  }
+  PodCells(PodCells&& o) noexcept : heap_(std::move(o.heap_)), rows_(o.rows_), cols_(o.cols_) {
+    copyInline(o);
+    o.clear();
+  }
+  PodCells& operator=(PodCells&& o) noexcept {
+    if (this == &o) return *this;
+    heap_ = std::move(o.heap_);
+    rows_ = o.rows_;
+    cols_ = o.cols_;
+    copyInline(o);
+    o.clear();
+    return *this;
+  }
+
+  size_t size() const { return rows_; }
+  bool empty() const { return rows_ == 0; }
+  Row operator[](size_t pod) { return Row{data() + pod * cols_, cols_}; }
+  ConstRow operator[](size_t pod) const { return ConstRow{data() + pod * cols_, cols_}; }
+  RowIter<T*> begin() { return {data(), cols_, 0}; }
+  RowIter<T*> end() { return {data(), cols_, rows_}; }
+  RowIter<T* const> begin() const { return {data(), cols_, 0}; }
+  RowIter<T* const> end() const { return {data(), cols_, rows_}; }
+
+  void clear() {
+    heap_.clear();
+    rows_ = cols_ = 0;
+  }
+  void assign(size_t pods, size_t leaves) {
+    clear();
+    rows_ = pods;
+    cols_ = leaves;
+    if (pods * leaves > N) {
+      heap_.assign(pods * leaves, nullptr);
+    } else {
+      std::fill(inl_, inl_ + pods * leaves, nullptr);
+    }
+  }
+  T** appendPod(size_t leaves) {
+    if (rows_ == 0) cols_ = leaves;
+    if (leaves != cols_) throw std::logic_error("PodCells: pods of one block differ in size");
+    const size_t have = rows_ * cols_;
+    if (!heap_.empty() || have + cols_ > N) {
+      if (heap_.empty()) heap_.assign(inl_, inl_ + have);
+      heap_.resize(have + cols_, nullptr);
+    } else {
+      std::fill(inl_ + have, inl_ + have + cols_, nullptr);
+    }
+    rows_++;
+    return data() + have;
+  }
+
+ private:
+  T** data() { return heap_.empty() ? inl_ : heap_.data(); }
+  T* const* data() const { return heap_.empty() ? inl_ : heap_.data(); }
+  void copyInline(const PodCells& o) {
+    if (heap_.empty()) std::copy(o.inl_, o.inl_ + rows_ * cols_, inl_);
+  }
+  T* inl_[N];
+  std::vector<T*> heap_;
+  size_t rows_ = 0;
+  size_t cols_ = 0;
+};
+
+template <class T, size_t N = 1>
+class InlineVec {
+ public:
+  size_t size() const { return heap_.empty() ? n_ : heap_.size(); }
+  bool empty() const { return size() == 0; }
+  T* begin() { return heap_.empty() ? inl_ : heap_.data(); }
+  T* end() { return begin() + size(); }
+  const T* begin() const { return heap_.empty() ? inl_ : heap_.data(); }
+  const T* end() const { return begin() + size(); }
+  T& operator[](size_t i) { return begin()[i]; }
+  const T& operator[](size_t i) const { return begin()[i]; }
+  void resize(size_t n) {
+    if (heap_.empty() && n <= N) {
+      for (size_t i = n; i < n_; i++) inl_[i] = T{};
+      n_ = n;
+      return;
+    }
+    if (heap_.empty()) {
+      heap_.reserve(n);
+      for (size_t i = 0; i < n_; i++) {
+        heap_.push_back(std::move(inl_[i]));
+        inl_[i] = T{};
+      }
+      n_ = 0;
+    }
+    heap_.resize(n);
+  }
+  void clear() { resize(0); }
+
+ private:
+  T inl_[N];
+  size_t n_ = 0;
+  std::vector<T> heap_;
+};
 
 struct Group;
 struct PhysicalCell;
@@ -192,7 +450,7 @@
   std::vector<Cell*> children;
   int priority = kFreePriority;
   bool healthy = true;
-  std::map<int, int> usedLeafAtPriority;
+  FlatIntMap<int> usedLeafAtPriority;
   int freeLeavesUnder = 0;
 
   virtual ~Cell() = default;
@@ -273,8 +531,12 @@
   bool present = false;
   std::string key;
   std::string node;
-  BindInfo bindInfo;
-};
+  std::shared_ptr<const BindInfo> bindInfo;
+};
+using PodSlots = InlineVec<AllocatedPod, 1>;
+
+template <class CellT>
+using Placement = FlatLeafMap<PodCells<CellT>>;
 
 struct LazyPreemptionStatus {
   std::string preemptor;
@@ -289,13 +551,29 @@
   bool gangReleaseEnable = false;
   int priority = 0;
   GState state = GState::Allocated;
-  std::map<int, int> totalPodNums;
-  std::map<int, std::vector<AllocatedPod>> allocatedPods;
-  std::map<int, std::vector<std::vector<PhysicalCell*>>> physPlacement;
+  FlatLeafMap<int> totalPodNums;
+  FlatLeafMap<PodSlots> allocatedPods;
+  Placement<PhysicalCell> physPlacement;
   bool hasVirtualPlacement = true;
-  std::map<int, std::vector<std::vector<VirtualCell*>>> virtPlacement;
+  Placement<VirtualCell> virtPlacement;
   std::set<std::string> preemptingPods;
   std::optional<LazyPreemptionStatus> lazyStatus;
+  void reset() {
+    name.clear();
+    vc.clear();
+    lazyPreemptionEnable = false;
+    ignoreK8sSuggestedNodes = true;
+    gangReleaseEnable = false;
+    priority = 0;
+    state = GState::Allocated;
+    totalPodNums.clear();
+    allocatedPods.clear();
+    physPlacement.clear();
+    hasVirtualPlacement = true;
+    virtPlacement.clear();
+    preemptingPods.clear();
+    lazyStatus.reset();
+  }
 };
 
 struct CellTypeSpec {
@@ -335,7 +613,7 @@
   bool lazyPreemptionEnable = false;
   bool ignoreK8sSuggestedNodes = true;
   std::string groupName;
-  std::map<int, int> groupPodNums;
+  FlatLeafMap<int> groupPodNums;
   long long hbmBytesPerCell = 0;
 };
 
@@ -343,14 +621,11 @@
 
 struct ScheduleResult {
   enum class Kind { Bind, Preempt, Wait } kind = Kind::Wait;
-  BindInfo bindInfo;
+  std::shared_ptr<const BindInfo> bindInfo;
   std::string victimNode;
   std::vector<std::string> victimPodKeys;
   std::string waitReason;
 };
-
-template <class CellT>
-using Placement = std::map<int, std::vector<std::vector<CellT*>>>;
 
 struct CleanShapeWorld {
   int priority = kOpportunisticPriority;
@@ -372,7 +647,7 @@
   const std::string& vc;
   const std::string& pinnedCellId;
   const std::string& groupName;
-  const std::map<int, int>& podLeafCellNums;
+  const FlatLeafMap<int>& podLeafCellNums;
   const std::string* chain = nullptr;
   IntraVCScheduler* vcScheduler = nullptr;
   const TopoScheduler* topo = nullptr;
@@ -389,11 +664,22 @@
   TopoScheduler() = default;
   TopoScheduler(const ChainCellList& ccl, std::map<int, int> levelLeafNum, bool crossPriorityPack);
 
-  bool Schedule(const std::map<int, int>& podLeafCellNums, int priority,
+  template <class CellT>
+  bool Schedule(const FlatLeafMap<int>& podLeafCellNums, int priority,
                 const std::set<std::string>& suggestedNodes, bool ignoreSuggestedNodes,
-                Placement<Cell>* out, std::string* failedReason,
-                long long minHbmBytes = 0,
-                const CleanShapeWorld* cleanWorld = nullptr, bool honorOnly = false) const;
+                Placement<CellT>* out, std::string* failedReason, long long minHbmBytes = 0,
+                const CleanShapeWorld* cleanWorld = nullptr, bool honorOnly = false) const {
+    PlacementSink sink{out, [](void* to) { static_cast<Placement<CellT>*>(to)->clear(); },
+                       [](void* to, int leafNum, const std::vector<Cell*>& leaves) {
+                         CellT** row = (*static_cast<Placement<CellT>*>(to))[leafNum].appendPod(
+                             leaves.size());
+                         for (size_t i = 0; i < leaves.size(); i++) {
+                           row[i] = static_cast<CellT*>(leaves[i]);
+                         }
+                       }};
+    return scheduleInto(podLeafCellNums, priority, suggestedNodes, ignoreSuggestedNodes, sink,
+                        failedReason, minHbmBytes, cleanWorld, honorOnly);
+  }
 
  private:
   struct NodeView {
@@ -404,10 +690,19 @@
     bool healthy = true;
     bool suggested = true;
   };
+  struct PlacementSink {
+    void* to;
+    void (*clear)(void* to);
+    void (*addPod)(void* to, int leafNum, const std::vector<Cell*>& leaves);
+  };
+  bool scheduleInto(const FlatLeafMap<int>& podLeafCellNums, int priority,
+                    const std::set<std::string>& suggestedNodes, bool ignoreSuggestedNodes,
+                    const PlacementSink& out, std::string* failedReason, long long minHbmBytes,
+                    const CleanShapeWorld* cleanWorld, bool honorOnly) const;
   bool tryScheduleAtPriority(const std::vector<int>& sortedLeafNums, int priority,
                              const std::set<std::string>& suggestedNodes, bool ignoreSuggestedNodes,
                              long long minHbmBytes, bool honorLinks,
-                             const CleanShapeWorld* cleanWorld, Placement<Cell>* out,
+                             const CleanShapeWorld* cleanWorld, const PlacementSink& out,
                              std::string* failedReason) const;
 
   std::vector<Cell*> viewCells_;
@@ -417,6 +712,7 @@
     std::vector<NodeView> view;
     std::vector<int> sortedLeafNums;
     std::vector<int> pickedNodeIndices;
+    std::vector<Cell*> leaves;
   };
   mutable Scratch scratch_;
 };
@@ -434,6 +730,48 @@
 struct BindingVertex {
   VirtualCell* cell = nullptr;
   std::vector<BindingVertex*> children;
+};
+
+class VictimList {
+ public:
+  bool empty() const { return pods_.empty(); }
+  void clear() {
+    pods_.clear();
+    nodes_ = 0;
+  }
+  void add(const std::string& node, const std::string& key) { pods_.push_back({&node, &key}); }
+  void seal() {
+    auto less = [](const Entry& a, const Entry& b) {
+      const int c = a.first->compare(*b.first);
+      return c != 0 ? c < 0 : *a.second < *b.second;
+    };
+    auto same = [](const Entry& a, const Entry& b) {
+      return *a.first == *b.first && *a.second == *b.second;
+    };
+    std::sort(pods_.begin(), pods_.end(), less);
+    pods_.erase(std::unique(pods_.begin(), pods_.end(), same), pods_.end());
+    nodes_ = 0;
+    for (size_t i = 0; i < pods_.size(); i++) {
+      if (i == 0 || *pods_[i].first != *pods_[i - 1].first) nodes_++;
+    }
+  }
+  size_t nodeCount() const { return nodes_; }
+  void nodeAt(size_t index, std::string* node, std::vector<std::string>* keys) const {
+    size_t at = 0;
+    size_t i = 0;
+    for (; i < pods_.size(); i++) {
+      if (i > 0 && *pods_[i].first != *pods_[i - 1].first) at++;
+      if (at == index) break;
+    }
+    *node = *pods_[i].first;
+    keys->clear();
+    for (; i < pods_.size() && *pods_[i].first == *node; i++) keys->push_back(*pods_[i].second);
+  }
+
+ private:
+  using Entry = std::pair<const std::string*, const std::string*>;
+  std::vector<Entry> pods_;
+  size_t nodes_ = 0;
 };
 
 using CellBindings = SmallPtrMap<VirtualCell, PhysicalCell*, 32>;
@@ -455,6 +793,8 @@
                           const std::set<std::string>& suggestedNodes, Phase phase);
   void deleteUnallocatedPod(const PodSpec& s, const std::string& podKey);
   void addAllocatedPod(const PodSpec& s, const BindInfo& info, const std::string& podKey);
+  void addAllocatedPod(const PodSpec& s, const std::shared_ptr<const BindInfo>& info,
+                       const std::string& podKey);
   void deleteAllocatedPod(const PodSpec& s, const BindInfo& info, const std::string& podKey);
   bool deleteAllocatedPodByKey(const std::string& podKey);
 
@@ -504,20 +844,20 @@
 
   ScheduleResult generateResult(const Placement<PhysicalCell>& phys, bool hasVirtual,
                                 const Placement<VirtualCell>& virt,
-                                const std::map<std::string, std::set<std::string>>& victims,
+                                const VictimList& victims,
                                 std::string&& waitReason, int currentLeafNum, int podIndex,
                                 Group* group, const std::string& groupName);
   bool schedulePodFromExistingGroup(Group* g, const PodSpec& s,
                                     const std::set<std::string>& suggestedNodes, Phase phase,
                                     const std::string& podKey, Placement<PhysicalCell>* phys,
                                     bool* hasVirtual, Placement<VirtualCell>* virt,
-                                    std::map<std::string, std::set<std::string>>* victims,
+                                    VictimList* victims,
                                     int* podIndex);
   void schedulePodFromNewGroup(const PodSpec& s, const std::set<std::string>& suggestedNodes,
                                Phase phase, const std::string& podKey,
                                Placement<PhysicalCell>* phys, bool* hasVirtual,
                                Placement<VirtualCell>* virt,
-                               std::map<std::string, std::set<std::string>>* victims,
+                               VictimList* victims,
                                std::string* waitReason);
   bool scheduleNewAffinityGroup(const PodSpec& s, const std::set<std::string>& suggestedNodes,
                                 const std::string& podKey, Placement<PhysicalCell>* phys,
@@ -541,10 +881,14 @@
   std::map<std::string, Placement<VirtualCell>> tryLazyPreempt(const Placement<VirtualCell>& p,
                                                                const std::string& groupName);
 
+  void addAllocatedPodShared(const PodSpec& s, const BindInfo& info,
+                             const std::shared_ptr<const BindInfo>* shared,
+                             const std::string& podKey);
   void setPodSlot(Group* g, int leafCellNum, int podIndex, bool releasable,
-                  const std::string& podKey, const BindInfo& info);
+                  const std::string& podKey, std::shared_ptr<const BindInfo> info);
   void clearPodSlot(Group* g, int leafCellNum, int podIndex);
   void eraseGroup(Group* g);
+  Group* insertNewGroup(const PodSpec& s, GState state);
 
   Group* createAllocatedGroup(const PodSpec& s, const BindInfo& info, const std::string& podKey);
   void deleteAllocatedGroup(Group* g, const std::string& podKey);
@@ -608,6 +952,14 @@
     }
   };
   MapScratch mapScratch_;
+  VictimList victimScratch_;
+
+  using GroupNode = std::map<std::string, std::unique_ptr<Group>>::node_type;
+#ifndef HIVED_GROUP_POOL_MAX
+#define HIVED_GROUP_POOL_MAX 64
+#endif
+  static constexpr size_t kGroupPoolMax = HIVED_GROUP_POOL_MAX;
+  std::vector<GroupNode> groupPool_;
 
  public:
   std::map<std::string, ChainCellList> fullCellList_;
diff --git a/hivedscheduler_amd/core/debug.cpp b/hivedscheduler_amd/core/debug.cpp
--- a/hivedscheduler_amd/core/debug.cpp
+++ b/hivedscheduler_amd/core/debug.cpp
@@ -58,7 +58,13 @@
           }
           if (c->healthy != allHealthy) fail("healthiness roll-up at " + c->address);
           if (anyUsed && c->state != CState::Used) fail("state roll-up (Used) at " + c->address);
-          if (usedSum != c->usedLeafAtPriority) fail("usedLeafAtPriority roll-up at " + c->address);
+          const bool sameCounts =
+              usedSum.size() == c->usedLeafAtPriority.size() &&
+              std::equal(usedSum.begin(), usedSum.end(), c->usedLeafAtPriority.begin(),
+                         [](const auto& a, const auto& b) {
+                           return a.first == b.first && a.second == b.second;
+                         });
+          if (!sameCounts) fail("usedLeafAtPriority roll-up at " + c->address);
         } else if (c->freeLeavesUnder != (c->priority == kFreePriority ? 1 : 0)) {
           fail("leaf freeLeavesUnder at " + c->address);
         }
diff --git a/hivedscheduler_amd/core/flat_containers_test_main.cpp b/hivedscheduler_amd/core/flat_containers_test_main.cpp
--- /dev/null
+++ b/hivedscheduler_amd/core/flat_containers_test_main.cpp
@@ -0,0 +1,263 @@
+#include <cstdio>
+#include <cstdlib>
+#include <map>
+#include <memory>
+#include <random>
+#include <string>
+#include <vector>
+
+#include "core.hpp"
+
+using namespace hived;
+
+namespace {
+
+long gChecks = 0;
+
+#define CHECK(cond)                                                        \
+  do {                                                                     \
+    gChecks++;                                                             \
+    if (!(cond)) {                                                         \
+      fprintf(stderr, "%s:%d: check failed: %s\n", __FILE__, __LINE__, #cond); \
+      exit(1);                                                             \
+    }                                                                      \
+  } while (0)
+
+struct Owner {
+  std::unique_ptr<std::string> text;
+  std::vector<int> numbers;
+  Owner() = default;
+  explicit Owner(int v) : text(std::make_unique<std::string>(40, static_cast<char>('a' + v % 26))),
+                          numbers(static_cast<size_t>(v % 5 + 1), v) {}
+  Owner(const Owner& o)
+      : text(o.text ? std::make_unique<std::string>(*o.text) : nullptr), numbers(o.numbers) {}
+  Owner(Owner&&) = default;
+  Owner& operator=(const Owner& o) {
+    text = o.text ? std::make_unique<std::string>(*o.text) : nullptr;
+    numbers = o.numbers;
+    return *this;
+  }
+  Owner& operator=(Owner&&) = default;
+  bool operator==(const Owner& o) const {
+    if (static_cast<bool>(text) != static_cast<bool>(o.text)) return false;
+    return (!text || *text == *o.text) && numbers == o.numbers;
+  }
+};
+
+template <class V>
+void expectSame(const FlatLeafMap<V>& flat, const std::map<int, V>& ref) {
+  CHECK(flat.size() == ref.size());
+  CHECK(flat.empty() == ref.empty());
+  auto it = flat.begin();
+  int last = 0;
+  for (auto& [k, v] : ref) {
+    CHECK(it != flat.end());
+    CHECK(it->first == k);
+    CHECK(it->first > last);
+    CHECK(it->second == v);
+    last = it->first;
+    ++it;
+  }
+  CHECK(it == flat.end());
+  for (int k = 0; k <= 13; k++) {
+    CHECK(flat.count(k) == ref.count(k));
+    auto found = flat.find(k);
+    CHECK((found == flat.end()) == (ref.find(k) == ref.end()));
+    if (found != flat.end()) CHECK(found->second == ref.at(k) && flat.at(k) == ref.at(k));
+  }
+}
+
+template <class V, class Make>
+void randomOperations(unsigned seed, int operations, Make make) {
+  std::mt19937 rng(seed);
+  FlatLeafMap<V> flat;
+  std::map<int, V> ref;
+  expectSame(flat, ref);
+  for (int op = 0; op < operations; op++) {
+    const int k = 1 + static_cast<int>(rng() % 12);
+    switch (rng() % 10) {
+      case 0:
+      case 1:
+      case 2:
+      case 3: {
+        V v = make(static_cast<int>(rng() % 1000));
+        flat[k] = v;
+        ref[k] = v;
+        break;
+      }
+      case 4:
+        CHECK(flat[k] == ref[k]);
+        break;
+      case 5:
+      case 6:
+        CHECK(flat.erase(k) == ref.erase(k));
+        break;
+      case 7: {
+        FlatLeafMap<V> copy(flat);
+        expectSame(copy, ref);
+        FlatLeafMap<V> target;
+        target[3] = make(3);
+        target[9] = make(9);
+        target = copy;
+        expectSame(target, ref);
+        copy[k] = make(k);
+        expectSame(flat, ref);
+        flat = target;
+        break;
+      }
+      case 8: {
+        FlatLeafMap<V> moved(std::move(flat));
+        expectSame(moved, ref);
+        CHECK(flat.empty() && flat.begin() == flat.end());
+        flat[5] = make(5);
+        flat = std::move(moved);
+        CHECK(moved.empty());
+        break;
+      }
+      case 9:
+        if (rng() % 4 == 0) {
+          flat.clear();
+          ref.clear();
+        }
+        try {
+          flat.at(13);
+          CHECK(false);
+        } catch (const std::out_of_range&) {
+        }
+        break;
+    }
+    expectSame(flat, ref);
+  }
+}
+
+template <class V, class Make>
+void capacityEdges(Make make) {
+  const std::vector<std::vector<int>> orders = {
+      {}, {4, 3, 2, 1}, {1, 2, 3, 4}, {4, 1, 5, 2, 3}, {5, 4, 3, 2, 1}, {2, 9, 1, 12, 7, 3, 11}};
+  for (auto& order : orders) {
+    FlatLeafMap<V> flat;
+    std::map<int, V> ref;
+    for (int k : order) {
+      flat[k] = make(k);
+      ref[k] = make(k);
+      expectSame(flat, ref);
+    }
+    FlatLeafMap<V> copy = flat;
+    expectSame(copy, ref);
+    for (int k : order) {
+      CHECK(flat.erase(k) == 1);
+      ref.erase(k);
+      expectSame(flat, ref);
+    }
+    CHECK(flat.erase(1) == 0);
+    for (int k : order) flat[k] = make(k + 1);
+    for (int k : order) ref[k] = make(k + 1);
+    expectSame(flat, ref);
+    expectSame(copy, [&] {
+      std::map<int, V> m;
+      for (int k : order) m[k] = make(k);
+      return m;
+    }());
+  }
+}
+
+void podCells() {
+  int cellsStore[64];
+  std::mt19937 rng(3);
+  for (size_t leaves : {0, 1, 2, 4, 5, 8}) {
+    PodCells<int> block;
+    std::vector<std::vector<int*>> ref;
+    CHECK(block.empty() && block.begin() == block.end());
+    for (size_t pod = 0; pod < 5; pod++) {
+      int** row = block.appendPod(leaves);
+      ref.emplace_back();
+      for (size_t i = 0; i < leaves; i++) {
+        CHECK(row[i] == nullptr);
+        row[i] = &cellsStore[rng() % 64];
+        ref.back().push_back(row[i]);
+      }
+      CHECK(block.size() == ref.size());
+      size_t pi = 0;
+      for (auto& podCellsRow : block) {
+        CHECK(podCellsRow.size() == leaves && podCellsRow.empty() == (leaves == 0));
+        size_t li = 0;
+        for (int* c : podCellsRow) CHECK(c == ref[pi][li++]);
+        CHECK(li == leaves);
+        pi++;
+      }
+      CHECK(pi == ref.size());
+      const PodCells<int>& constBlock = block;
+      for (size_t p = 0; p < ref.size(); p++) {
+        for (size_t i = 0; i < leaves; i++) CHECK(constBlock[p][i] == ref[p][i]);
+      }
+      PodCells<int> copy = block;
+      PodCells<int> assigned;
+      assigned.assign(3, 7);
+      assigned = copy;
+      PodCells<int> moved = std::move(copy);
+      CHECK(copy.empty());
+      for (size_t p = 0; p < ref.size(); p++) {
+        for (size_t i = 0; i < leaves; i++) {
+          CHECK(moved[p][i] == ref[p][i] && assigned[p][i] == ref[p][i]);
+        }
+      }
+      if (leaves > 0) {
+        moved[0][0] = nullptr;
+        CHECK(block[0][0] == ref[0][0]);
+      }
+    }
+    if (leaves > 0) {
+      try {
+        block.appendPod(leaves + 1);
+        CHECK(false);
+      } catch (const std::logic_error&) {
+      }
+    }
+    block.assign(2, 3);
+    CHECK(block.size() == 2 && block[1].size() == 3 && block[1][2] == nullptr);
+    block.assign(4, 6);
+    CHECK(block.size() == 4 && block[3].size() == 6 && block[3][5] == nullptr);
+    block.clear();
+    CHECK(block.empty());
+  }
+}
+
+void inlineVec() {
+  std::mt19937 rng(4);
+  InlineVec<Owner, 1> vec;
+  std::vector<Owner> ref;
+  for (int op = 0; op < 400; op++) {
+    if (rng() % 3 == 0) {
+      const size_t n = rng() % 5;
+      vec.resize(n);
+      ref.resize(n);
+    } else if (!ref.empty()) {
+      const size_t i = rng() % ref.size();
+      vec[i] = Owner(op);
+      ref[i] = Owner(op);
+    }
+    CHECK(vec.size() == ref.size() && vec.empty() == ref.empty());
+    size_t i = 0;
+    for (auto& v : vec) CHECK(v == ref[i++]);
+    CHECK(i == ref.size());
+    InlineVec<Owner, 1> copy = vec;
+    InlineVec<Owner, 1> moved = std::move(copy);
+    CHECK(moved.size() == ref.size());
+    for (size_t j = 0; j < ref.size(); j++) CHECK(moved[j] == ref[j]);
+  }
+}
+
+}
+
+int main() {
+  for (unsigned seed = 1; seed <= 4; seed++) {
+    randomOperations<int>(seed, 1500, [](int v) { return v; });
+    randomOperations<Owner>(seed + 10, 1500, [](int v) { return Owner(v); });
+  }
+  capacityEdges<int>([](int v) { return v; });
+  capacityEdges<Owner>([](int v) { return Owner(v); });
+  podCells();
+  inlineVec();
+  printf("flat containers OK (%ld checks)\n", gChecks);
+  return 0;
+}
diff --git a/hivedscheduler_amd/core/sched_bench_main.cpp b/hivedscheduler_amd/core/sched_bench_main.cpp
--- a/hivedscheduler_amd/core/sched_bench_main.cpp
+++ b/hivedscheduler_amd/core/sched_bench_main.cpp
@@ -75,7 +75,7 @@
   lat.reserve(nreq);
   struct LivePod {
     PodSpec spec;
-    BindInfo info;
+    std::shared_ptr<const BindInfo> info;
     std::string key;
   };
   std::vector<LivePod> live;
@@ -99,7 +99,7 @@
       live.push_back({s, r.bindInfo, key});
     }
     if ((int)live.size() > nodes * 4) {
-      core.deleteAllocatedPod(live.front().spec, live.front().info, live.front().key);
+      core.deleteAllocatedPod(live.front().spec, *live.front().info, live.front().key);
       live.erase(live.begin());
     }
   }
diff --git a/hivedscheduler_amd/core/topo_sched.cpp b/hivedscheduler_amd/core/topo_sched.cpp
--- a/hivedscheduler_amd/core/topo_sched.cpp
+++ b/hivedscheduler_amd/core/topo_sched.cpp
@@ -587,7 +587,7 @@
                                           const std::set<std::string>& suggestedNodes,
                                           bool ignoreSuggestedNodes, long long minHbmBytes,
                                           bool honorLinks, const CleanShapeWorld* cleanWorld,
-                                          Placement<Cell>* out,
+                                          const PlacementSink& out,
                                           std::string* failedReason) const {
   std::vector<NodeView>& cv = scratch_.view;
   cv.clear();
@@ -694,11 +694,12 @@
       }
     }
   }
-  out->clear();
+  out.clear(out.to);
+  std::vector<Cell*>& leaves = scratch_.leaves;
   for (size_t i = 0; i < sortedLeafNums.size(); i++) {
     int q = sortedLeafNums[i];
     Cell* node = cv[pickedNodeIndices[i]].c;
-    std::vector<Cell*> leaves;
+    leaves.clear();
     leaves.reserve(q);
     if (session.world != nullptr && !node->isPhysical()) {
       bool placed = false;
@@ -715,16 +716,16 @@
     } else {
       pickLeaves(node, q, priority, session, leaves);
     }
-    (*out)[q].push_back(std::move(leaves));
+    out.addPod(out.to, q, leaves);
   }
   return true;
 }
 
-bool TopoScheduler::Schedule(const std::map<int, int>& podLeafCellNums, int priority,
-                             const std::set<std::string>& suggestedNodes,
-                             bool ignoreSuggestedNodes, Placement<Cell>* out,
-                             std::string* failedReason, long long minHbmBytes,
-                             const CleanShapeWorld* cleanWorld, bool honorOnly) const {
+bool TopoScheduler::scheduleInto(const FlatLeafMap<int>& podLeafCellNums, int priority,
+                                 const std::set<std::string>& suggestedNodes,
+                                 bool ignoreSuggestedNodes, const PlacementSink& out,
+                                 std::string* failedReason, long long minHbmBytes,
+                                 const CleanShapeWorld* cleanWorld, bool honorOnly) const {
   std::vector<int>& sortedLeafNums = scratch_.sortedLeafNums;
   sortedLeafNums.clear();
   for (auto& [leafNum, podNum] : podLeafCellNums) {
@@ -754,24 +755,14 @@
 bool IntraVCScheduler::schedule(const SchedulingRequest& sr, Placement<VirtualCell>* out,
                                 std::string* failedReason) const {
   const TopoScheduler* scheduler = sr.topo;
-  Placement<Cell> generic;
   if (scheduler == nullptr ||
       !scheduler->Schedule(sr.podLeafCellNums, sr.priority, *sr.suggestedNodes,
-                           sr.ignoreSuggestedNodes, &generic, failedReason, sr.hbmBytes,
+                           sr.ignoreSuggestedNodes, out, failedReason, sr.hbmBytes,
                            sr.cleanWorld, sr.honorLinksOnly)) {
     if (failedReason->empty()) *failedReason = "no scheduler for request";
     failedReason->append(" when scheduling in VC ").append(sr.vc);
     return false;
   }
-  out->clear();
-  for (auto& [leafNum, pods] : generic) {
-    for (auto& pod : pods) {
-      std::vector<VirtualCell*> cells;
-      cells.reserve(pod.size());
-      for (Cell* c : pod) cells.push_back(static_cast<VirtualCell*>(c));
-      (*out)[leafNum].push_back(std::move(cells));
-    }
-  }
   return true;
 }
 
```

New measurement: 751.0 ns (median of 6 runs). 1.05x faster.
